# ucsdmanorlab/bootstrapper

Hardware: AMD Instinct MI355X
Metric: Mvoxels/s predict+segment, 1024^3 vol in 128^3 blocks (higher is better)
Workload: dtype bf16x3

## Files before the change

bootstrapper_amd/_lib.py:

```python
import ctypes as C
import os

import torch

_HERE = os.path.dirname(os.path.abspath(__file__))
LIB_PATH = os.environ.get("BSMI_LIB") or os.path.join(_HERE, "libbsmi.so")

MAX_LEVELS, MAX_CONVS, MAX_HEADS, NAME_LEN = 8, 4, 4, 32
PREC_F32, PREC_BF16, PREC_BF16X3 = 0, 1, 2
RAW_U8, RAW_F32, RAW_U8_UNIT = 0, 1, 2
ERR_INVALID, ERR_HIP, ERR_STATE, ERR_MISSING, ERR_OVERFLOW = -1, -2, -3, -4, -5


class UNetConfig(C.Structure):
    _fields_ = [
        ("in_channels", C.c_int32),
        ("num_fmaps", C.c_int32),
        ("fmap_inc_factor", C.c_int32),
        ("num_levels", C.c_int32),
        ("downsample_factors", (C.c_int32 * 3) * MAX_LEVELS),
        ("n_convs_down", C.c_int32 * MAX_LEVELS),
        ("kernel_size_down", ((C.c_int32 * 3) * MAX_CONVS) * MAX_LEVELS),
        ("n_convs_up", C.c_int32 * MAX_LEVELS),
        ("kernel_size_up", ((C.c_int32 * 3) * MAX_CONVS) * MAX_LEVELS),
        ("num_heads", C.c_int32),
        ("head_name", (C.c_char * NAME_LEN) * MAX_HEADS),
        ("head_dims", C.c_int32 * MAX_HEADS),
        ("num_fmaps_out", C.c_int32),
    ]


class StepInfo(C.Structure):
    _fields_ = [("type", C.c_int32), ("materialised", C.c_int32), ("shape", C.c_int32 * 4), ("conv_index", C.c_int32),
                ("form", C.c_int32), ("flags", C.c_int32), ("bn", C.c_int32), ("ksteps", C.c_int32), ("head", C.c_int32),
                ("factor", C.c_int32 * 3), ("offset", C.c_int32 * 3), ("prefix", C.c_char * 64)]


class TrainWgradInfo(C.Structure):
    _fields_ = [(n, C.c_int32) for n in ("family", "residual", "n", "c", "cbase", "kx", "tile_n", "tile_c", "ranges", "lines_per_range",
                                         "det_workspace")]


class TrainStepInfo(C.Structure):
    _fields_ = [("type", C.c_int32), ("n_wgrad", C.c_int32), ("wgrad", TrainWgradInfo * 4), ("dgrad", C.c_int32), ("dgrad_raw", C.c_int32),
                ("dgrad_converted", C.c_int32), ("dgrad_bn", C.c_int32), ("dgrad_ksteps", C.c_int32), ("dgrad_split_k", C.c_int32),
                ("dgrad_scatter", C.c_int32), ("dgrad_residual", C.c_int32), ("border", C.c_int32 * 3), ("has_split", C.c_int32),
                ("bias", C.c_int32), ("up", C.c_int32), ("fwd_split", C.c_int32), ("deterministic", C.c_int32)]


WGRAD_FAMILIES = ("none", "wave-f32", "tiled-f32", "split-bf16")
TRAIN_TENSORS = {"dout": 0, "gmask": 1, "gsplit": 2, "gsplit_hi": 3, "gsplit_lo": 4, "dcat": 5, "head_dp": 6, "pad_count": 7}
STEP_TYPES = ("input", "conv", "pool", "up", "head")
CONV_FORMS = ("gather", "raster-halo", "box-halo", "halo-resident", "first-pass", "winograd F(2x2)", "winograd F(4x4)")
STEP_FLAGS = {1: "fused-up", 2: "res-low", 4: "split-k"}
STEP_BELOW_UP = 8
STEP_WINO_Z = 16


class Codec(C.Structure):
    _fields_ = [("id", C.c_int32), ("level", C.c_int32), ("cname", C.c_int32), ("shuffle", C.c_int32),
                ("typesize", C.c_int32), ("blocksize", C.c_int32)]


class ChunkCopy(C.Structure):
    _fields_ = [("path", C.c_char_p), ("base", C.c_void_p), ("start", C.c_int64 * 4), ("extent", C.c_int64 * 4),
                ("stride", C.c_int64 * 4), ("read_modify_write", C.c_int32), ("reserved", C.c_int32)]


class BatchFragArgs(C.Structure):
    _fields_ = [("affs_dev", C.c_void_p), ("frags_dev", C.c_void_p), ("max_id_dev", C.c_void_p), ("labels_dev", C.c_void_p),
                ("num_labels_dev", C.c_void_p), ("id_offset", C.c_uint64), ("size_dev", C.c_void_p), ("sums_dev", C.c_void_p)]


class BatchGraphArgs(C.Structure):
    _fields_ = [("affs_dev", C.c_void_p), ("frags_dev", C.c_void_p), ("edges_dev", C.c_void_p), ("sums_dev", C.c_void_p),
                ("pair_counts_dev", C.c_void_p), ("counts_dev", C.c_void_p), ("edge_capacity", C.c_uint64)]


class Aug2dDraw(C.Structure):
    _fields_ = [("a", C.c_float * 4), ("src", C.c_float * 2), ("inv_spacing", C.c_float * 2), ("flags", C.c_int32), ("n", C.c_int32 * 2),
                ("lattice_offset", C.c_int32), ("crop", C.c_int32 * 2), ("crop_offset", C.c_int32), ("reserved", C.c_int32)]


class Aug2dIDraw(C.Structure):
    _fields_ = [("seed", C.c_uint64), ("impulse_threshold", C.c_uint64), ("noise_sigma", C.c_float), ("contrast_scale", C.c_float),
                ("nodes", C.c_int32), ("radius", C.c_int32), ("taps_offset", C.c_int32), ("reserved", C.c_int32 * 3)]


CODEC_RAW, CODEC_ZLIB, CODEC_GZIP, CODEC_ZSTD, CODEC_LZ4, CODEC_BLOSC = range(6)
BLOSC_LZ4, BLOSC_ZLIB, BLOSC_ZSTD = 1, 3, 4
CHUNK_MISSING = 1
MORPH_DILATE, MORPH_ERODE = 0, 1
RESCALE_DOWN, RESCALE_UP = 0, 1


class BsmiError(RuntimeError):
    def __init__(self, code, msg):
        super().__init__(f"libbsmi error {code}: {msg}")
        self.code = code
        self.msg = msg


def _load():
    if not os.path.exists(LIB_PATH):
        raise ImportError(
            f"{LIB_PATH} not found: build it with `python -c 'import __graft_entry__ as g; g.build()'` "
            "(or `make -C bootstrapper_amd/csrc`).  There is no CPU fallback.")
    lib = C.CDLL(LIB_PATH)
    p, i32, i64p, vp = C.c_void_p, C.c_int, C.POINTER(C.c_int64), C.c_void_p
# ... 184 lines not shown
```

bootstrapper_amd/csrc/conv_h16.h:

```cpp
#pragma once
#include "conv_igemm.h"

namespace bsmi {

struct H16Phase {
  int32_t tensor;
  int32_t delta;
  int32_t rows;
  int32_t nsteps;
};
static_assert(sizeof(H16Phase) == 16, "H16Phase layout");

struct H16Step {
  int32_t offa, offb, pad0, pad1;
};
static_assert(sizeof(H16Step) == 16, "H16Step layout");

struct H16Args {
  ConvSrc t[kMaxConvTensors];
  const H16Phase* phases;
  const H16Step* steps;
  int nphases, nsteps;
  const void* w;
  const void* w_lo;
  const float* bias;
  void* out;
  int Do, Ho, Wo, Co;
  int Hin, Win;
  int Q;
  int Npad;
  int relu;
  int ntiles, n_big, r_small;
};

constexpr int kH16TileRows = 512;
int h16_halo_rows(int Win, int ky, int kx, int npad, int* max_r);
void h16_tiling(int64_t Q, int npad, int halo_rows, int max_r, int n_cus, int* ntiles, int* n_big, int* r_small);
int launch_conv_h16(const H16Args& a, int halo_rows, hipStream_t stream);

}
```

bootstrapper_amd/csrc/conv_h16.hip:

```cpp
#include "conv_h16.h"

#include <algorithm>

#include "conv_dev.h"

namespace bsmi {

#ifdef BSMI_STAMP
__device__ unsigned long long g_h16_stamp[8];
extern "C" int bsmi_debug_stamps_h16(unsigned long long* out, int reset) {
  if (hipMemcpyFromSymbol(out, HIP_SYMBOL(g_h16_stamp), sizeof(unsigned long long) * 8) != hipSuccess) return -1;
  if (reset) {
    unsigned long long z[8] = {0, 0, 0, 0, 0, 0, 0, 0};
    if (hipMemcpyToSymbol(HIP_SYMBOL(g_h16_stamp), z, sizeof z) != hipSuccess) return -1;
  }
  return 0;
}
#define H16_STAMP(var_) const unsigned long long var_ = wall_clock64()
#else
#define H16_STAMP(var_)
#endif

namespace {

constexpr int kNW = 4;
constexpr int kR = 8;

template <int FNB, int HR>
__global__ __launch_bounds__(64 * kNW, 2) void conv_h16_kernel(const H16Args a) {
  using T = bf16f_elem;
  constexpr int BN = 16 * FNB, BM = kH16TileRows;
  static_assert(BM == kNW * kR * 16, "tile rows");
  constexpr int HALO = HR * 64;
  constexpr int OFF_B = HALO;
  constexpr int EB = BN * 64;
  constexpr int SLOT = 2 * EB;
  constexpr int JW = HR / 16 / kNW;
  static_assert(HR % (16 * kNW) == 0, "the waves share the halo rows evenly");
  constexpr int G = FNB >= 4 ? 1 : (FNB == 2 ? 2 : 8);
  extern __shared__ __attribute__((aligned(16))) char smem[];
  const int tid = threadIdx.x, lane = tid & 63;
  const int wave = __builtin_amdgcn_readfirstlane(tid >> 6);
  const int ntiles = a.ntiles;
  const int qn = ntiles >> 3, rn = ntiles & 7;
  const int xcd = blockIdx.x & 7, jn = blockIdx.x >> 3;
  const int tile = (xcd < rn ? xcd * (qn + 1) : rn * (qn + 1) + (xcd - rn) * qn) + jn;
  const int R = tile < a.n_big ? kR : a.r_small;
  const int q0 = tile < a.n_big ? tile * BM : a.n_big * BM + (tile - a.n_big) * a.r_small * (kNW * 16);
  const int cut = (kR - R) * (kNW * 16);
  H16_STAMP(st_begin);
#ifdef BSMI_STAMP
  unsigned long long acc_halo = 0, acc_k = 0, acc_w = 0;
#endif
  const cint_ptr_t phases = (cint_ptr_t)a.phases;
  const cint_ptr_t steps = (cint_ptr_t)a.steps;
  const int nsteps = a.nsteps, nphases = a.nphases;
// ... 84 lines not shown
      const uint32_t ar = arow0 + (uint32_t)(tap_b ? offb : offa);
      const char* ap = smem + ar * 64 + ((aslot ^ ((ar >> 2) & 1)) << 4);
      const char* apl = smem + ar * 64 + ((aslot ^ ((ar >> 2) & 1) ^ 1) << 4);
#pragma unroll
      for (int i0 = 0; i0 < kR; i0 += G) {
        if (i0 >= R) break;
        u32x4_t AH[G], AL[G];
#pragma unroll
        for (int g = 0; g < G; ++g) {
          AH[g] = *(const u32x4_t*)(ap + (i0 + g) * 1024);
          AL[g] = *(const u32x4_t*)(apl + (i0 + g) * 1024);
        }
#pragma unroll
        for (int g = 0; g < G; ++g)
#pragma unroll
          for (int j = 0; j < FNB; ++j)
            acc[i0 + g][j] = __builtin_amdgcn_mfma_f32_16x16x32_bf16(__builtin_bit_cast(bf16x8_t, AL[g]), __builtin_bit_cast(bf16x8_t, BH[j]), acc[i0 + g][j], 0, 0, 0);
#pragma unroll
        for (int g = 0; g < G; ++g)
#pragma unroll
          for (int j = 0; j < FNB; ++j)
            acc[i0 + g][j] = __builtin_amdgcn_mfma_f32_16x16x32_bf16(__builtin_bit_cast(bf16x8_t, AH[g]), __builtin_bit_cast(bf16x8_t, BH[j]), acc[i0 + g][j], 0, 0, 0);
#pragma unroll
        for (int g = 0; g < G; ++g)
#pragma unroll
          for (int j = 0; j < FNB; ++j)
            acc[i0 + g][j] = __builtin_amdgcn_mfma_f32_16x16x32_bf16(__builtin_bit_cast(bf16x8_t, AH[g]), __builtin_bit_cast(bf16x8_t, BL[j]), acc[i0 + g][j], 0, 0, 0);
      }
      H16_STAMP(st_k1);
      asm volatile("s_waitcnt vmcnt(0) lgkmcnt(0)" ::: "memory");
      __builtin_amdgcn_s_barrier();
#ifdef BSMI_STAMP
      {
        const unsigned long long st_k2 = wall_clock64();
        acc_k += st_k1 - st_k0;
        acc_w += st_k2 - st_k1;
      }
#endif
    }
  }
#undef H16_ISSUE_B
  H16_STAMP(st_epi);

  constexpr int PITCH = BN * 2 + 16;
  constexpr int CPR = BN * 2 / 16;
  constexpr int NCH = 16 * CPR;
  constexpr int LO_STRIPS = kNW * 16 * PITCH;
  static_assert(2 * LO_STRIPS <= HALO, "strips fit in the halo area");
  char* strip = smem + wave * (16 * PITCH);
  T* out = (T*)a.out;
  float bv[FNB];
#pragma unroll
  for (int j = 0; j < FNB; ++j) bv[j] = a.bias[j * 16 + lr];
#pragma unroll
  for (int i = 0; i < kR; ++i) {
    if (i >= R) break;
#pragma unroll
    for (int j = 0; j < FNB; ++j)
#pragma unroll
      for (int r = 0; r < 4; ++r) {
        float v = acc[i][j][r] + bv[j];
        if (a.relu) v = v > 0.f ? v : 0.f;
        Elem<T>::store((T*)(strip + (4 * lq + r) * PITCH) + j * 16 + lr, v);
        Elem<T>::store((T*)(strip + LO_STRIPS + (4 * lq + r) * PITCH) + j * 16 + lr, split_lo(v));
      }
    asm volatile("s_waitcnt lgkmcnt(0)" ::: "memory");
#pragma unroll
    for (int k = 0; k < (NCH + 63) / 64; ++k) {
      const int c = lane + 64 * k;
      if (c >= NCH) break;
      const int row = c / CPR, cc = c - row * CPR;
      const int q = q0 + wave * (R * 16) + i * 16 + row;
      const int n = cc * 8;
      if (q < a.Q && n < a.Co) {
        const int xx = q % a.Win;
        const int zy = q / a.Win;
        const int yy = zy % a.Hin, z = zy / a.Hin;
        if (xx < a.Wo && yy < a.Ho) {
          T* dst = out + act_index<T>(((size_t)(z * a.Ho + yy) * a.Wo + xx) * a.Co, n);
          store_stream16(dst, *(const u32x4_t*)(strip + row * PITCH + cc * 16));
          store_stream16(dst + kSplitLoElems, *(const u32x4_t*)(strip + LO_STRIPS + row * PITCH + cc * 16));
        }
      }
    }
    asm volatile("s_waitcnt lgkmcnt(0)" ::: "memory");
  }
#ifdef BSMI_STAMP
  if (tid == 0) {
    const unsigned long long st_end = wall_clock64();
    atomicAdd(&g_h16_stamp[0], acc_halo);
    atomicAdd(&g_h16_stamp[1], acc_k);
    atomicAdd(&g_h16_stamp[2], acc_w);
    atomicAdd(&g_h16_stamp[3], 1ull);
    atomicAdd(&g_h16_stamp[4], (unsigned long long)nphases);
    atomicAdd(&g_h16_stamp[5], (unsigned long long)nsteps);
    atomicAdd(&g_h16_stamp[6], st_loop - st_begin);
    atomicAdd(&g_h16_stamp[7], st_end - st_epi);
  }
#endif
}

template <int FNB, int HR>
int launch_t(const H16Args& a, hipStream_t stream) {
  constexpr int smem = HR * 64 + 4 * 16 * FNB * 64;
  static_assert(2 * smem <= 160 * 1024, "two workgroups per CU (three at 16 columns and 768 rows)");
  auto kern = conv_h16_kernel<FNB, HR>;
  static DeviceOnce once;
  const int rc_once = once.run([&]() -> int {
    BSMI_HIP(hipFuncSetAttribute((const void*)kern, hipFuncAttributeMaxDynamicSharedMemorySize, smem));
    hipFuncAttributes fa;
    BSMI_HIP(hipFuncGetAttributes(&fa, (const void*)kern));
    if (fa.localSizeBytes != 0) BSMI_FAIL(BSMI_ERR_STATE, "halo conv kernel (%d columns) was compiled with %zu bytes of scratch", 16 * FNB, (size_t)fa.localSizeBytes);
    return BSMI_OK;
  });
  if (rc_once) return rc_once;
  hipLaunchKernelGGL(kern, dim3(a.ntiles), dim3(64 * kNW), smem, stream, a);
  BSMI_HIP(hipGetLastError());
  return BSMI_OK;
}

}

int h16_halo_rows(int Win, int ky, int kx, int npad, int* max_r) {
  if (npad != 16 && npad != 64) return 0;
  const int reach = (ky - 1) * Win + (kx - 1);
  *max_r = kR;
  if (kH16TileRows + reach <= 768) return 768;
  if (npad == 16 && (kR - 1) * kNW * 16 + reach <= 768) {
    *max_r = kR - 1;
    return 768;
  }
  if (kH16TileRows + reach <= 1024 && npad == 16) return 1024;
  return 0;
}

void h16_tiling(int64_t Q, int npad, int halo_rows, int max_r, int n_cus, int* ntiles, int* n_big, int* r_small) {
  const int64_t big = kH16TileRows, unit = kNW * 16;
  if (max_r < kR) {
    *ntiles = (int)((Q + max_r * unit - 1) / (max_r * unit));
    *n_big = 0;
    *r_small = max_r;
    return;
  }
  const int64_t nt = (Q + big - 1) / big;
  *ntiles = (int)nt;
  *n_big = (int)nt;
  *r_small = kR;
  const int64_t lds = (int64_t)halo_rows * 64 + 4 * npad * 64;
  const int64_t per_cu = std::min<int64_t>(npad == 64 ? 2 : 3, (160 * 1024) / lds);
  const int64_t slots = per_cu * n_cus;
  if (slots <= 0 || nt % slots == 0) return;
  const int64_t rounds = (nt + slots - 1) / slots, total = rounds * slots;
  if (rounds > 4) return;
  const int64_t r = (Q + total * unit - 1) / (total * unit);
  if (r < 6 || r > kR) return;
  if (r < kR) {
    const int64_t rows = r * unit;
    *ntiles = (int)((Q + rows - 1) / rows);
    *n_big = 0;
    *r_small = (int)r;
    return;
  }
  const int64_t small = big - unit;
  int64_t nb = (Q - total * small + unit - 1) / unit;
  if (nb < 0) nb = 0;
  *ntiles = (int)total;
  *n_big = (int)nb;
  *r_small = kR - 1;
}

int launch_conv_h16(const H16Args& a, int halo_rows, hipStream_t stream) {
  if (a.Q <= 0 || a.nsteps <= 0 || a.nphases <= 0 || a.Hin <= 0 || a.Win <= 0 || a.Hin > 2047 || a.Win > 2047 || a.Do > 1023)
    BSMI_FAIL(BSMI_ERR_INVALID, "halo conv: bad geometry Q=%d steps=%d phases=%d raster %d x %d", a.Q, a.nsteps, a.nphases, a.Hin, a.Win);
// ... 12 lines not shown
```

bootstrapper_amd/csrc/unet_debug.hip:

```cpp
#include <cstring>

#include "unet_internal.h"

extern "C" {

int bsmi_debug_wino_pack_host(const float* w, int cout, int cin, int wz, uint16_t* out, uint64_t capacity, uint64_t* image_elems, uint64_t* batch_elems,
                              int* npad, int* ksteps) {
  if (!w || cout < 1 || cin < 1) BSMI_FAIL(BSMI_ERR_INVALID, "bad argument");
  std::vector<int> cin_of_v;
  for (int c = 0; c < round_up(cin, kChanPad); ++c) cin_of_v.push_back(c < cin ? c : -1);
  const int Npad = round_up(cout, tile_bn(choose_tile(cout)));
  std::vector<WinoUnit> units;
  wino_units((int)cin_of_v.size(), units, wz ? 1 : 3);
  if (image_elems || batch_elems || out) {
    std::vector<uint16_t> packed;
    size_t ie = 0, be = 0;
    wino_pack_weights(w, cout, cin, cin_of_v, Npad, units, packed, ie, be, 4, wz != 0);
    if (image_elems) *image_elems = ie;
    if (batch_elems) *batch_elems = be;
    if (out) {
      if (capacity < packed.size()) BSMI_FAIL(BSMI_ERR_INVALID, "buffer of %llu values too small", (unsigned long long)capacity);
      memcpy(out, packed.data(), packed.size() * sizeof(uint16_t));
    }
  }
  if (npad) *npad = Npad;
  if (ksteps) *ksteps = (int)(units.size() / kUnitsPerStep);
  return BSMI_OK;
}

int bsmi_unet_debug_activation(bsmi_unet* h, int step, int what, int64_t shape_out[4], float* host_out, uint64_t capacity) {
  if (!h || !shape_out) BSMI_FAIL(BSMI_ERR_INVALID, "null argument");
  Plan* plan = h->last_plan;
  if (!plan) BSMI_FAIL(BSMI_ERR_STATE, "no forward has run");
  if (step < 0 || step >= (int)plan->steps.size()) BSMI_FAIL(BSMI_ERR_INVALID, "step %d out of range (%zu steps)", step, plan->steps.size());
  const PlanStep& st = plan->steps[step];
  if (st.type == PlanStep::HEAD) BSMI_FAIL(BSMI_ERR_INVALID, "head steps write into the caller's buffers");
  if (plan->fused_first && step < 2)
    BSMI_FAIL(BSMI_ERR_STATE, "step %d is not materialised: the first ConvPass ran as one launch (first_pass), which writes step 2 only", step);
  if (st.type == PlanStep::UP && st.skip)
    BSMI_FAIL(BSMI_ERR_STATE, "step %d is not materialised: the upsampling is fused into the Winograd stages that read it", step);
  const TDesc& t = st.out;
  shape_out[0] = t.D; shape_out[1] = t.H; shape_out[2] = t.W; shape_out[3] = t.C;
  if (!host_out) return BSMI_OK;
  const size_t nvox = (size_t)t.D * t.H * t.W;
  if (capacity < nvox * t.C) BSMI_FAIL(BSMI_ERR_INVALID, "buffer of %llu floats too small", (unsigned long long)capacity);
  BSMI_HIP(hipSetDevice(h->device));
  BSMI_HIP(hipDeviceSynchronize());
  const int es = esize(plan->prec);
  const bool split = t.lo_off != 0;
  const size_t bytes = nvox * t.Cpad * es * (split ? 2 : 1);
  std::vector<uint8_t> raw(bytes);
  BSMI_HIP(hipMemcpy(raw.data(), t.ptr, raw.size(), hipMemcpyDeviceToHost));
  for (size_t v = 0; v < nvox; ++v)
    for (int c = 0; c < t.C; ++c) {
      float x;
      if (plan->prec == BSMI_PREC_F32) {
        x = ((const float*)raw.data())[v * t.Cpad + c];
      } else if (!split) {
        x = host_bf16_to_f32(((const uint16_t*)raw.data())[v * t.Cpad + c]);
      } else {
        const size_t i = 2 * v * t.Cpad + (size_t)((c >> 3) << 4) + (c & 7);
        const float hi = host_bf16_to_f32(((const uint16_t*)raw.data())[i]);
        const float lo = host_bf16_to_f32(((const uint16_t*)raw.data())[i + 8]);
        x = what == 1 ? hi : (what == 2 ? lo : hi + lo);
      }
      host_out[v * t.C + c] = x;
    }
  return BSMI_OK;
}

int bsmi_unet_debug_step_info(bsmi_unet* h, int step, bsmi_unet_step_info* info, int* n_steps) {
  if (!h) BSMI_FAIL(BSMI_ERR_INVALID, "null handle");
  Plan* plan = h->last_plan;
  if (!plan) BSMI_FAIL(BSMI_ERR_STATE, "no forward has run");
  if (n_steps) *n_steps = (int)plan->steps.size();
  if (!info) return BSMI_OK;
  if (step < 0 || step >= (int)plan->steps.size()) BSMI_FAIL(BSMI_ERR_INVALID, "step %d out of range (%zu steps)", step, plan->steps.size());
  const PlanStep& st = plan->steps[step];
  memset(info, 0, sizeof *info);
  info->type = (int32_t)st.type;
  const bool in_first = plan->fused_first && step < 3;
  info->materialised = !((plan->fused_first && step < 2) || (st.type == PlanStep::UP && st.skip));
  const TDesc& t = st.type == PlanStep::HEAD ? st.in : st.out;
  info->shape[0] = t.D; info->shape[1] = t.H; info->shape[2] = t.W;
  info->shape[3] = st.type == PlanStep::HEAD ? h->heads[st.head].cout : t.C;
  const std::string* prefix = nullptr;
  if (st.type == PlanStep::HEAD) {
    info->head = st.head;
    prefix = &h->heads[st.head].prefix;
  } else if (st.type == PlanStep::POOL || st.type == PlanStep::UP) {
    for (int d = 0; d < 3; ++d) { info->factor[d] = st.f[d]; info->offset[d] = st.type == PlanStep::UP ? st.o[d] : 0; }
  } else if (st.type == PlanStep::CONV) {
    prefix = &st.site->prefix;
    info->conv_index = st.ci;
    const int sk_grid = h->sk_grid > 0 ? h->sk_grid : 0;
    if (in_first) {
      info->form = BSMI_FORM_FIRST_PASS;
    } else if (st.use_wino) {
      info->form = st.wino_in.m == 4 ? BSMI_FORM_WINO4 : BSMI_FORM_WINO2;
      info->bn = tile_bn(st.tile);
      info->ksteps = st.wino_gemm.nsteps;
      bool up = false;
      for (int q = 0; q < st.wino_in.nsrc; ++q) up = up || st.wino_in.upf[q] > 0;
      if (up || st.wino_out.low || st.wino_has_below) info->flags |= BSMI_STEP_FUSED_UP;
      if (st.wino_has_below) info->flags |= BSMI_STEP_BELOW_UP;
      if (st.wino_has_res_low) info->flags |= BSMI_STEP_RES_LOW;
      if (st.wino_in.wz) info->flags |= BSMI_STEP_WINO_Z;
      if (conv_igemm_split_k(st.wino_gemm, plan->prec, st.tile, sk_grid) ||
          (st.wino_has_res && conv_igemm_split_k(st.wino_res, plan->prec, st.tile, sk_grid)) ||
          (st.wino_has_res_low && conv_igemm_split_k(st.wino_res_low, plan->prec, st.tile, sk_grid)) ||
          (st.wino_has_below && conv_igemm_split_k(st.wino_below, plan->prec, st.below_tile, sk_grid)))
        info->flags |= BSMI_STEP_SPLIT_K;
    } else if (st.use_h16) {
      info->form = BSMI_FORM_HALO_RESIDENT;
      info->bn = st.h16.Npad;
      info->ksteps = st.h16.nsteps;
    } else if (st.use_box) {
      info->form = BSMI_FORM_BOX_HALO;
    } else if (st.use_rh) {
      info->form = BSMI_FORM_RASTER_HALO;
      info->bn = tile_bn(st.tile);
      info->ksteps = st.rh.nsteps;
      if (conv_rh_split_k(st.rh, st.tile, sk_grid)) info->flags |= BSMI_STEP_SPLIT_K;
    } else {
      info->form = BSMI_FORM_GATHER;
      info->bn = tile_bn(st.tile);
      info->ksteps = st.conv.nsteps;
      if (conv_igemm_split_k(st.conv, plan->prec, st.tile, sk_grid)) info->flags |= BSMI_STEP_SPLIT_K;
    }
  }
  if (prefix) snprintf(info->prefix, sizeof info->prefix, "%s", prefix->c_str());
  return BSMI_OK;
}

}
```

bootstrapper_amd/csrc/unet_forward.hip:

```cpp
#include <algorithm>
#include <cstdlib>
#include <mutex>

#include "unet_internal.h"
#include "unet_ops.h"

#include "dev_guard.h"

namespace bsmi {

static int harvest(bsmi_unet* h, Plan* plan) {
  if (!plan || plan->inflight.empty()) return BSMI_OK;
  const size_t n = plan->steps.size();
  for (auto& set : plan->inflight) {
    plan->last_ms.assign(n, 0.f);
    BSMI_HIP(hipEventSynchronize(set[2 * n - 1]));
    for (size_t i = 0; i < n; ++i) {
      float t = 0.f;
      BSMI_HIP(hipEventElapsedTime(&t, set[2 * i], set[2 * i + 1]));
      plan->last_ms[i] = t;
      const int ty = (plan->fused_first && i < 2) ? (int)PlanStep::CONV : (int)plan->steps[i].type;
      h->prof_ms[ty] += t;
      h->prof_flops[ty] += plan->steps[i].flops;
      if (ty == 1) h->prof_exec += plan->steps[i].exec_flops > 0 ? plan->steps[i].exec_flops : plan->steps[i].flops * (plan->prec == BSMI_PREC_BF16X3 ? 3.0 : 1.0);
// ... 71 lines not shown
    } else {
      plan.events.assign(n_ev, nullptr);
      for (auto& e : plan.events) BSMI_HIP(hipEventCreate(&e));
    }
  }
  if (!h->sk_grid) {
    const char* e = getenv("BSMI_STREAMK");
    if ((e && e[0] == '0') || h->sk_request == 0) {
      h->sk_grid = -1;
    } else {
      hipDeviceProp_t prop;
      BSMI_HIP(hipGetDeviceProperties(&prop, h->device));
      h->sk_grid = h->sk_request >= 0 ? h->sk_request : prop.multiProcessorCount / 8 * 8;
      if (const char* g = getenv("BSMI_SK_GRID")) h->sk_grid = std::max(8, atoi(g) / 8 * 8);
      BSMI_HIP(hipMalloc((void**)&h->sk_ws, stream_k_ws_bytes(h->sk_grid)));
      BSMI_HIP(hipMemsetAsync((char*)h->sk_ws + stream_k_ws_bytes(h->sk_grid) - 64, 0, 64, s));
    }
  }
  if (h->train && precision == BSMI_PREC_F32 && !h->train_forward && (rc = train_refresh_f32_images(h, s))) return rc;
  size_t step_idx = 0;
  for (const PlanStep& st : plan.steps) {
    if (prof) BSMI_HIP(hipEventRecord(plan.events[2 * step_idx], s));
    if (plan.fused_first && step_idx < 3) {
      if (step_idx == 2) {
        FirstPassArgs fa;
        fa.raw = raw_dev; fa.raw_dtype = raw_dtype;
        fa.D = plan.steps[0].out.D; fa.H = plan.steps[0].out.H; fa.W = plan.steps[0].out.W;
        fa.out = (uint16_t*)st.out.ptr;
        const FirstPassWeights& fw = precision == BSMI_PREC_BF16X3 ? h->first_pass_x3 : h->first_pass;
        fa.w1a = fw.w1a; fa.w2a = fw.w2a; fa.vec = fw.vec;
        fa.split = fw.split;
        rc = launch_first_pass(fa, h->sk_grid > 0 ? h->sk_grid : 256, s);
        if (rc) return rc;
      }
      if (prof) BSMI_HIP(hipEventRecord(plan.events[2 * step_idx + 1], s));
      ++step_idx;
      continue;
    }
    switch (st.type) {
      case PlanStep::INPUT:
        rc = launch_input_prep(precision, raw_dev, raw_dtype, st.out.ptr, st.out.C, st.out.Cpad,
                               (size_t)st.out.D * st.out.H * st.out.W, s);
        break;
      case PlanStep::CONV:
        if (st.use_wino && !(st.tx3 && h->train_forward)) {
          if ((rc = launch_wino_in(st.wino_in, s))) break;
          if ((rc = launch_conv_igemm(st.wino_gemm, precision, st.tile, s, h->sk_ws, h->sk_grid))) break;
          if (st.wino_has_res && (rc = launch_conv_igemm(st.wino_res, precision, st.tile, s, h->sk_ws, h->sk_grid))) break;
          if (st.wino_has_res_low && (rc = launch_conv_igemm(st.wino_res_low, precision, st.tile, s, h->sk_ws, h->sk_grid))) break;
          if (st.wino_has_below && (rc = launch_conv_igemm(st.wino_below, precision, st.below_tile, s, h->sk_ws, h->sk_grid))) break;
          rc = launch_wino_out(st.wino_out, s);
          break;
        }
        rc = (st.tx3 && h->train_forward) ? train_forward_conv_x3(h, st, s)
             : st.use_h16 ? launch_conv_h16(st.h16, st.h16_rows, s)
             : st.use_box ? launch_conv_box(st.box, s)
             : st.use_rh ? launch_conv_rh(st.rh, precision, st.tile, s, h->sk_ws, h->sk_grid)
                         : launch_conv_igemm(st.conv, precision, st.tile, s, h->sk_ws, h->sk_grid);
        break;
      case PlanStep::POOL:
        if (st.pool_fused) break;
        rc = launch_maxpool(precision, st.in.ptr, st.out.ptr, st.in.D, st.in.H, st.in.W, st.in.Cpad,
                            st.f[0], st.f[1], st.f[2], s);
        break;
      case PlanStep::UP:
        if (st.skip) break;
        rc = launch_upsample_crop(precision, st.in.ptr, st.out.ptr, st.in.D, st.in.H, st.in.W, st.in.Cpad,
                                  st.out.D, st.out.H, st.out.W, st.f[0], st.f[1], st.f[2], st.o[0], st.o[1], st.o[2], s);
        break;
      case PlanStep::HEAD: {
        const HeadSite& hd = h->heads[st.head];
        float* of = out_f32_dev ? out_f32_dev[st.head] : nullptr;
        uint8_t* ou = out_u8_dev ? out_u8_dev[st.head] : nullptr;
        if (of || ou)
          rc = launch_head(precision, st.in.ptr, st.in.Cpad, hd.cin, hd.cout, hd.hw, hd.hb, of, ou,
                           (size_t)st.in.D * st.in.H * st.in.W, s);
        break;
      }
    }
    if (rc) return rc;
    if (prof) BSMI_HIP(hipEventRecord(plan.events[2 * step_idx + 1], s));
    ++step_idx;
  }
  if (prof) plan.inflight.push_back(std::move(plan.events));
  return forward_chain_leave(h->device, s);
}

int bsmi_unet_profile_enable(bsmi_unet* h, int on) {
  if (!h) BSMI_FAIL(BSMI_ERR_INVALID, "null handle");
  h->profile_period = on > 0 ? on : 0;
  h->profile_count = 0;
  return BSMI_OK;
}

int bsmi_unet_profile_read(bsmi_unet* h, int max_n, int* n, int32_t* types, double* ms, double* flops) {
  if (!h || !n) BSMI_FAIL(BSMI_ERR_INVALID, "null argument");
  Plan* plan = h->last_plan;
  if (!plan || !plan->profiled) BSMI_FAIL(BSMI_ERR_STATE, "no profiled forward to read");
  int rc = harvest(h, plan);
  if (rc) return rc;
  const int cnt = (int)plan->steps.size();
  *n = cnt;
  for (int i = 0; i < cnt && i < max_n; ++i) {
    if (types) types[i] = (int32_t)plan->steps[i].type;
    if (ms) ms[i] = plan->last_ms[i];
    if (flops) flops[i] = plan->steps[i].flops;
// ... 27 lines not shown
```

bootstrapper_amd/csrc/unet_internal.h:

```cpp
#pragma once
#include <cstring>
#include <map>
#include <memory>
#include <string>
#include <vector>

#include "conv_igemm.h"
#include "conv_rh.h"
#include "conv_h16.h"
#include "conv_box.h"
#include "first_pass.h"
#include "wino.h"

namespace bsmi {

struct HostWeight {
  std::vector<int64_t> shape;
  std::vector<float> data;
  bool loaded = false;
};

struct PackEntry {
  int slot;
  int dz, dy, dx;
  int c0;
  int wsrc;
  int tap;
  int cin_base;
  int creal;
  bool dummy;
  int phase;
};

struct PackPhase {
  int slot, c0, kind, first_unit, nunits;
};

struct PackedConv {
  bool ready = false;
  std::vector<PackEntry> entries;
  std::vector<PackPhase> phases;
  void* w = nullptr;
  int ks = 1;
  size_t lo_image_bytes = 0;
  float* bias = nullptr;
  int Npad = 0;
  TileCfg tile = TILE_256x32;
};

struct PackedWino {
  bool ready = false;
  int m = 2;
  bool fused_only = false;
  bool wz = false;
  std::vector<WinoUnit> units;
  std::vector<int> cin_of_v;
  int Cv = 0;
  void* w = nullptr;
  size_t lo_image_bytes = 0, batch_bytes = 0;
  int Npad = 0;
  TileCfg tile = TILE_256x32;
  std::vector<PackEntry> res_entries;
  void* res_w = nullptr;
  size_t res_lo_image_bytes = 0;
  std::vector<PackEntry> res_part[2];
  void* res_part_w[2] = {nullptr, nullptr};
  size_t res_part_lo[2] = {0, 0};
  bool below_ready = false;
  std::vector<WinoUnit> skip_units, below_units;
  std::vector<int> skip_cin_of_v;
  int skip_Cv = 0;
  void* skip_w = nullptr;
  size_t skip_lo_image_bytes = 0, skip_batch_bytes = 0;
  void* below_w = nullptr;
  size_t below_lo_image_bytes = 0, below_batch_bytes = 0;
  int below_Npad = 0;
  bool below_dense = false;
  TileCfg below_tile = TILE_256x320;
};

struct H16PhaseHost {
  int slot, c0, dz, kind;
  int first_step, nsteps;
};
struct PackedH16 {
  bool ready = false;
  std::vector<PackEntry> entries;
  std::vector<H16PhaseHost> phases;
  void* w = nullptr;
  size_t lo_image_bytes = 0;
  int Npad = 0;
};

struct PassSite {
  std::string prefix;
  int nslots = 1;
  int cin[2] = {0, 0};
  int cout = 0;
  int nconv = 0;
  int k[BSMI_MAX_CONVS][3];
  PackedConv packed[BSMI_NUM_PREC][BSMI_MAX_CONVS];
  PackedWino wino[BSMI_MAX_CONVS];
  PackedH16 h16[BSMI_MAX_CONVS];
};

struct HeadSite {
  std::string prefix;
  int cin = 0, cout = 0;
  float* hw = nullptr;
  float* hb = nullptr;
};

struct TDesc {
  void* ptr = nullptr;
  int C = 0, Cpad = 0, D = 0, H = 0, W = 0;
  size_t lo_off = 0;
};

struct PlanStep {
  enum Type { INPUT, CONV, POOL, UP, HEAD } type;
  ConvArgs conv;
  RhArgs rh;
  bool use_rh = false;
  H16Args h16;
  bool use_h16 = false;
  int h16_rows = 0;
  BoxArgs box;
  bool use_box = false;
  bool use_wino = false;
  WinoInArgs wino_in;
  ConvArgs wino_gemm, wino_res, wino_res_low;
  bool wino_has_res = false, wino_has_res_low = false;
  ConvArgs wino_below;
  bool wino_has_below = false;
  TileCfg below_tile = TILE_256x320;
  WinoOutArgs wino_out;
  TileCfg tile;
  TDesc in, out;
  int f[3], o[3];
  bool skip = false;
  bool pool_fused = false;
  int head = 0;
  double flops = 0;
  double exec_flops = 0;
  struct PassSite* site = nullptr;
  int ci = 0;
  TDesc slots[kMaxConvTensors];
  int so[kMaxConvTensors][3] = {{0, 0, 0}, {0, 0, 0}, {0, 0, 0}};
  int nsl = 0;
  struct TrainFwdX3* tx3 = nullptr;
};

struct Plan {
  std::vector<float> last_ms;
  bool pending = false;
  std::vector<void*> allocs;
  std::vector<PlanStep> steps;
  int64_t out_shape[3] = {0, 0, 0};
  double flops = 0;
  size_t bytes = 0;
  std::vector<hipEvent_t> events;
  std::vector<std::vector<hipEvent_t>> inflight, spare;
  bool profiled = false;
  bool fused_first = false;
  int prec = 0;
};

struct TrainState;

static inline uint16_t host_f32_to_bf16(float f) {
  uint32_t u;
  memcpy(&u, &f, 4);
  if ((u & 0x7fffffffu) > 0x7f800000u) return (uint16_t)((u >> 16) | 0x40);
  u += 0x7fffu + ((u >> 16) & 1u);
  return (uint16_t)(u >> 16);
}
static inline float host_bf16_to_f32(uint16_t b) {
  const uint32_t u = (uint32_t)b << 16;
  float f;
// ... 4 lines not shown
int esize(int prec);
int ksplit(int prec);
int bke(int prec);
int sube(int prec);
void build_entries(const PassSite& p, int ci, int prec, std::vector<PackEntry>& out, std::vector<PackPhase>* phases_out = nullptr);

}

using namespace bsmi;

struct bsmi_unet {
  bsmi_unet_config cfg;
  int device = 0;
  int nl = 0;
  std::vector<PassSite> l_conv, r_conv;
  std::vector<HeadSite> heads;
  int crop_factor[BSMI_MAX_LEVELS][3];
  std::map<std::string, HostWeight> weights;
  bool finalized[BSMI_NUM_PREC] = {false, false, false};
  int profile_period = 0;
  uint64_t profile_count = 0;
  Plan* last_plan = nullptr;
  double prof_ms[5] = {0, 0, 0, 0, 0}, prof_flops[5] = {0, 0, 0, 0, 0};
  double prof_exec = 0;
  int64_t prof_launches[5] = {0, 0, 0, 0, 0};
  std::map<std::vector<int64_t>, std::unique_ptr<Plan>> plans;
  float* sk_ws = nullptr;
  int sk_grid = 0;
  int sk_request = -1;
  bsmi::TrainState* train = nullptr;
  bool train_forward = false;
  int train_split = 1;
  int train_det = 0;
  bsmi::FirstPassWeights first_pass;
  bsmi::FirstPassWeights first_pass_x3;
};

namespace bsmi {
int pack_conv(bsmi_unet* h, PassSite& p, int ci, int prec);
int pack_wino(bsmi_unet* h, PassSite& p, int ci);
int pack_h16(bsmi_unet* h, PassSite& p, int ci);
void release(PackedConv& pc);
void release(PackedWino& pw);
void release(PackedH16& ph);

bool x3_fused_for(TileCfg tile);
bool wino_eligible(const PassSite& p, int ci);
int wino_tile_edge();
bool wino_narrow_last(const bsmi_unet* h, const PassSite& p, int ci);
bool below_up_site(const bsmi_unet* h, const PassSite& p, int ci);
bool wino_z_site(const bsmi_unet* h, const PassSite& p, int ci);
bool fuse_up_enabled();
bool pool_fuse_enabled();
int h16_mode();
int h16_only_npad();
bool h16_balanced();
bool rh_enabled(int prec, TileCfg tile, size_t nsteps);
bool box_enabled();
bool first_pass_eligible(const bsmi_unet* h);

int check_shape_arg(const int64_t s[3]);
int get_plan(bsmi_unet* h, int precision, const int64_t in_shape[3], Plan** out);
int dry_plan(bsmi_unet* h, const int64_t in_shape[3], Plan& plan);
void free_plan(Plan* p);
void free_train_state(bsmi_unet* h);
int train_forward_conv_x3(bsmi_unet* h, const PlanStep& st, hipStream_t s);
int train_refresh_f32_images(bsmi_unet* h, hipStream_t s);
}
```

bootstrapper_amd/csrc/unet_pack.hip:

```cpp
#include <cstdlib>
#include <cstring>

#include "unet_internal.h"

#include "dev_guard.h"

namespace bsmi {

int esize(int prec) { return prec == BSMI_PREC_F32 ? 4 : 2; }
int ksplit(int prec) { return prec == BSMI_PREC_BF16X3 ? 3 : 1; }
int bke(int prec) { return kStepRowBytes / esize(prec); }
int sube(int prec) { return 32 / esize(prec); }

static inline void split_bf16(float v, uint16_t& hi, uint16_t& lo) {
  hi = host_f32_to_bf16(v);
  lo = host_f32_to_bf16(v - host_bf16_to_f32(hi));
}

template <class T>
static void release_image(T*& w) {
  if (w) (void)hipFree(w);
  w = nullptr;
}
void release(PackedConv& pc) {
  release_image(pc.w);
  release_image(pc.bias);
  pc.ready = false;
}
void release(PackedWino& pw) {
  release_image(pw.w);
  release_image(pw.res_w);
  for (int part = 0; part < 2; ++part) release_image(pw.res_part_w[part]);
  release_image(pw.skip_w);
  release_image(pw.below_w);
  pw.below_ready = false;
  pw.ready = false;
}
void release(PackedH16& ph) {
  release_image(ph.w);
  ph.ready = false;
}

void build_entries(const PassSite& p, int ci, int prec, std::vector<PackEntry>& out, std::vector<PackPhase>* phases_out) {
  const int SUB = sube(prec);
  const bool last = ci == p.nconv - 1;
  std::vector<PackPhase> phases;
  auto close_phase = [&](PackPhase ph) {
    while ((out.size() - ph.first_unit) % kUnitsPerStep) out.push_back(PackEntry{ph.slot, 0, 0, 0, 0, 0, 0, 0, 0, true, (int)phases.size()});
    ph.nunits = (int)out.size() - ph.first_unit;
    phases.push_back(ph);
  };
  auto add_taps = [&](int slot, const int* k, int cin_base, int creal) {
    const int cpad = round_up(creal, kChanPad);
    if (cpad == SUB) {
      PackPhase ph{slot, 0, 0, (int)out.size(), 0};
      for (int z = 0; z < k[0]; ++z)
        for (int y = 0; y < k[1]; ++y)
          for (int x = 0; x < k[2]; x += kUnitsPerStep)
            for (int j = 0; j < kUnitsPerStep; ++j) {
              if (x + j < k[2])
                out.push_back(PackEntry{slot, z, y, x + j, 0, 0, (z * k[1] + y) * k[2] + x + j, cin_base, creal, false, (int)phases.size()});
              else
                out.push_back(PackEntry{slot, 0, 0, 0, 0, 0, 0, 0, 0, true, (int)phases.size()});
            }
      close_phase(ph);
      return;
    }
    for (int c32 = 0; c32 < cpad; c32 += kUnitsPerStep * SUB) {
      PackPhase ph{slot, c32, 0, (int)out.size(), 0};
      for (int z = 0; z < k[0]; ++z)
        for (int y = 0; y < k[1]; ++y)
          for (int x = 0; x < k[2]; ++x) {
            for (int c0 = c32; c0 < std::min(cpad, c32 + kUnitsPerStep * SUB); c0 += SUB)
              out.push_back(PackEntry{slot, z, y, x, c0, 0, (z * k[1] + y) * k[2] + x, cin_base, creal, false, (int)phases.size()});
            while ((out.size() - ph.first_unit) % kUnitsPerStep)
              out.push_back(PackEntry{slot, 0, 0, 0, 0, 0, 0, 0, 0, true, (int)phases.size()});
          }
      close_phase(ph);
    }
  };
  auto add_residual = [&](int slot, const int* crop, int cin_base, int creal) {
    const int cpad = round_up(creal, kChanPad);
    for (int c32 = 0; c32 < cpad; c32 += kUnitsPerStep * SUB) {
      PackPhase ph{slot, c32, 1, (int)out.size(), 0};
      for (int c0 = c32; c0 < std::min(cpad, c32 + kUnitsPerStep * SUB); c0 += SUB)
        out.push_back(PackEntry{slot, crop[0] / 2, crop[1] / 2, crop[2] / 2, c0, 1, 0, cin_base, creal, false, (int)phases.size()});
      close_phase(ph);
    }
  };
  const int* k = p.k[ci];
  if (ci == 0) {
    int base = 0;
// ... 37 lines not shown
  const int64_t cin_r = wr.shape[1];
  const int SUB = sube(prec);
  const bool fused = prec == BSMI_PREC_BF16X3 && x3_fused_for(pc.tile);
  const int KS = pc.ks = fused ? 1 : ksplit(prec);
  const size_t nsteps = pc.entries.size() / kUnitsPerStep * KS;
  const size_t nelem = (nsteps * (size_t)pc.Npad + kWeightRowSlack) * BKE;
  std::vector<float> bias(pc.Npad, 0.f);
  for (int n = 0; n < p.cout; ++n) bias[n] = bm.data[n] + (last ? br.data[n] : 0.f);

  pc.lo_image_bytes = fused ? nelem * esize(prec) : 0;
  std::vector<uint8_t> packed(nelem * esize(prec) * (fused ? 2 : 1), 0);
  host_parallel_for((size_t)p.cout, [&](size_t n_) {
    const int n = (int)n_;
    for (size_t u = 0; u < pc.entries.size(); ++u) {
      const PackEntry& e = pc.entries[u];
      if (e.dummy) continue;
      const size_t s = u / kUnitsPerStep, j = u % kUnitsPerStep;
      for (int kk = 0; kk < SUB; ++kk) {
        const int c = e.c0 + kk;
        if (c >= e.creal) break;
        float v;
        if (e.wsrc == 0) v = wm.data[((size_t)n * cin_m + (e.cin_base + c)) * ntap_m + e.tap];
        else v = wr.data[(size_t)n * cin_r + (e.cin_base + c)];
        const size_t idx = (s * KS * pc.Npad + n) * BKE + j * SUB + kk;
        if (prec == BSMI_PREC_F32) {
          ((float*)packed.data())[idx] = v;
        } else if (prec == BSMI_PREC_BF16) {
          ((uint16_t*)packed.data())[idx] = host_f32_to_bf16(v);
        } else {
          uint16_t hi, lo;
          split_bf16(v, hi, lo);
          uint16_t* w16 = (uint16_t*)packed.data();
          if (fused) {
            w16[idx] = hi;
            w16[idx + nelem] = lo;
          } else {
            const size_t blk = (size_t)pc.Npad * BKE;
            w16[idx] = hi;
            w16[idx + blk] = hi;
            w16[idx + 2 * blk] = lo;
          }
        }
      }
    }
  });
  BSMI_HIP(hipMalloc(&pc.w, packed.size()));
  BSMI_HIP(hipMemcpy(pc.w, packed.data(), packed.size(), hipMemcpyHostToDevice));
  BSMI_HIP(hipMalloc((void**)&pc.bias, bias.size() * sizeof(float)));
  BSMI_HIP(hipMemcpy(pc.bias, bias.data(), bias.size() * sizeof(float), hipMemcpyHostToDevice));
  pc.ready = true;
  return BSMI_OK;
}

int pack_wino(bsmi_unet* h, PassSite& p, int ci) {
  PackedWino& pw = p.wino[ci];
  release(pw);
  pw.fused_only = wino_narrow_last(h, p, ci);
  if (!wino_eligible(p, ci) && !pw.fused_only) return BSMI_OK;
  const HostWeight& wm = h->weights[p.prefix + ".conv_pass." + std::to_string(2 * ci) + ".weight"];
  const HostWeight& wr = h->weights[p.prefix + ".residual.0.weight"];
  const int cin_m = (int)wm.shape[1];
  pw.cin_of_v.clear();
  if (ci == 0) {
    int base = 0;
    for (int s = 0; s < p.nslots; ++s) {
      for (int c = 0; c < round_up(p.cin[s], kChanPad); ++c) pw.cin_of_v.push_back(c < p.cin[s] ? base + c : -1);
      base += p.cin[s];
    }
  } else {
    for (int c = 0; c < round_up(p.cout, kChanPad); ++c) pw.cin_of_v.push_back(c < p.cout ? c : -1);
  }
  pw.Cv = (int)pw.cin_of_v.size();
  pw.m = wino_tile_edge();
  pw.tile = choose_tile(p.cout);
  pw.Npad = round_up(p.cout, tile_bn(pw.tile));
  pw.wz = !pw.fused_only && pw.m == 4 && wino_z_site(h, p, ci);
  wino_units(pw.Cv, pw.units, pw.wz ? 1 : 3);
  {
    size_t image_elems = 0, batch_elems = 0;
    static const bool on_host = [] { const char* e = getenv("BSMI_WINO_PACK_HOST"); return e && e[0] == '1'; }();
    if (on_host) {
      std::vector<uint16_t> packed;
      wino_pack_weights(wm.data.data(), p.cout, cin_m, pw.cin_of_v, pw.Npad, pw.units, packed, image_elems, batch_elems, pw.m, pw.wz);
      BSMI_HIP(hipMalloc(&pw.w, packed.size() * 2));
      BSMI_HIP(hipMemcpy(pw.w, packed.data(), packed.size() * 2, hipMemcpyHostToDevice));
    } else {
      const int rc = wino_pack_weights_dev(wm.data.data(), p.cout, cin_m, pw.cin_of_v, pw.Npad, pw.units, pw.m, &pw.w, image_elems, batch_elems, pw.wz);
      if (rc) return rc;
    }
    pw.lo_image_bytes = image_elems * 2;
    pw.batch_bytes = batch_elems * 2;
  }
  pw.res_entries.clear();
  if (ci == p.nconv - 1) {
    std::vector<PackEntry> all;
    build_entries(p, ci, BSMI_PREC_BF16X3, all);
    for (size_t u = 0; u + 1 < all.size(); u += kUnitsPerStep) {
      bool res = false;
      for (int j = 0; j < kUnitsPerStep; ++j) res |= !all[u + j].dummy && all[u + j].wsrc == 1;
      if (res)
        for (int j = 0; j < kUnitsPerStep; ++j) pw.res_entries.push_back(all[u + j]);
    }
    if ((pw.res_entries.size() / kUnitsPerStep) % 2)
      for (int j = 0; j < kUnitsPerStep; ++j) pw.res_entries.push_back(PackEntry{0, 0, 0, 0, 0, 0, 0, 0, 0, true, 0});
    const int64_t cin_r = wr.shape[1];
    auto pack_res = [&](const std::vector<PackEntry>& ents, void** w_out, size_t* lo_out) -> int {
      const size_t nsteps = ents.size() / kUnitsPerStep;
      const size_t nelem = (nsteps * (size_t)pw.Npad + kWeightRowSlack) * 32;
      std::vector<uint16_t> packed(2 * nelem, 0);
      for (size_t u = 0; u < ents.size(); ++u) {
        const PackEntry& e = ents[u];
        if (e.dummy) continue;
        const size_t s = u / kUnitsPerStep, j = u % kUnitsPerStep;
        for (int n = 0; n < p.cout; ++n)
          for (int kk = 0; kk < 16; ++kk) {
            const int c = e.c0 + kk;
            if (c >= e.creal) break;
            const float v = wr.data[(size_t)n * cin_r + (e.cin_base + c)];
            const size_t idx = (s * pw.Npad + n) * 32 + j * 16 + kk;
            split_bf16(v, packed[idx], packed[nelem + idx]);
          }
      }
      *lo_out = nelem * 2;
      BSMI_HIP(hipMalloc(w_out, packed.size() * 2));
      BSMI_HIP(hipMemcpy(*w_out, packed.data(), packed.size() * 2, hipMemcpyHostToDevice));
      return BSMI_OK;
    };
    int rc = pack_res(pw.res_entries, &pw.res_w, &pw.res_lo_image_bytes);
    if (rc) return rc;
    for (int part = 0; part < 2; ++part) pw.res_part[part].clear();
    if (p.nslots == 2) {
      const int up_slot = (ci == 0 ? 0 : 1) + 1;
      for (size_t u = 0; u + 1 < pw.res_entries.size(); u += kUnitsPerStep) {
        int slot = -1;
        for (int j = 0; j < kUnitsPerStep; ++j)
          if (!pw.res_entries[u + j].dummy) slot = pw.res_entries[u + j].slot;
        if (slot < 0) continue;
        for (int j = 0; j < kUnitsPerStep; ++j) pw.res_part[slot == up_slot ? 1 : 0].push_back(pw.res_entries[u + j]);
      }
      for (int part = 0; part < 2; ++part) {
        if ((pw.res_part[part].size() / kUnitsPerStep) % 2)
          for (int j = 0; j < kUnitsPerStep; ++j) pw.res_part[part].push_back(PackEntry{0, 0, 0, 0, 0, 0, 0, 0, 0, true, 0});
        if ((rc = pack_res(pw.res_part[part], &pw.res_part_w[part], &pw.res_part_lo[part]))) return rc;
      }
    }
  }
  if (below_up_site(h, p, ci) && pw.m == 4) {
    pw.skip_cin_of_v.assign(pw.cin_of_v.begin(), pw.cin_of_v.begin() + round_up(p.cin[0], kChanPad));
    pw.skip_Cv = (int)pw.skip_cin_of_v.size();
    wino_units(pw.skip_Cv, pw.skip_units);
    size_t image_elems = 0, batch_elems = 0;
    int rc = wino_pack_weights_dev(wm.data.data(), p.cout, cin_m, pw.skip_cin_of_v, pw.Npad, pw.skip_units, pw.m, &pw.skip_w, image_elems, batch_elems);
    if (rc) return rc;
    pw.skip_lo_image_bytes = image_elems * 2;
    pw.skip_batch_bytes = batch_elems * 2;
    const int cpad_low = round_up(p.cin[1], kChanPad), cpad_out = round_up(p.cout, kChanPad);
    wino_units(cpad_low, pw.below_units);
    pw.below_dense = p.cout <= 64;
    pw.below_tile = pw.below_dense ? TILE_256x320 : pw.tile;
    pw.below_Npad = pw.below_dense ? round_up(9 * cpad_out, tile_bn(pw.below_tile)) : pw.Npad;
    const size_t nsteps = pw.below_units.size() / kUnitsPerStep;
    const size_t tap_elems = nsteps * (size_t)pw.below_Npad * 32;
    const size_t nelem = (pw.below_dense ? 1 : 9) * tap_elems + (size_t)kWeightRowSlack * 32;
    std::vector<uint16_t> packed(2 * nelem, 0);
    const bool dense = pw.below_dense;
    const int cin1 = p.cin[1], cbase = p.cin[0];
    host_parallel_for((size_t)p.cout, [&](size_t n_) {
      const int n = (int)n_;
      for (size_t u = 0; u < pw.below_units.size(); ++u) {
        const WinoUnit& un = pw.below_units[u];
        if (un.dummy) continue;
        const size_t s = u / kUnitsPerStep, j = u % kUnitsPerStep;
        for (int kk = 0; kk < 16; ++kk) {
          const int c = un.vc0 + kk;
          if (c >= cin1) break;
          const float* g = wm.data.data() + (((size_t)n * cin_m + (cbase + c)) * 3 + un.kz) * 9;
          for (int tap = 0; tap < 9; ++tap) {
            const size_t idx = dense ? (s * pw.below_Npad + (size_t)tap * cpad_out + n) * 32 + j * 16 + kk
                                     : (size_t)tap * tap_elems + (s * pw.below_Npad + n) * 32 + j * 16 + kk;
            split_bf16(g[tap], packed[idx], packed[nelem + idx]);
          }
        }
      }
    });
    pw.below_lo_image_bytes = nelem * 2;
    pw.below_batch_bytes = dense ? 0 : tap_elems * 2;
    BSMI_HIP(hipMalloc(&pw.below_w, packed.size() * 2));
    BSMI_HIP(hipMemcpy(pw.below_w, packed.data(), packed.size() * 2, hipMemcpyHostToDevice));
    pw.below_ready = true;
  }
  pw.ready = true;
  return BSMI_OK;
}

static void build_entries_h16(const PassSite& p, int ci, std::vector<PackEntry>& out, std::vector<H16PhaseHost>& phases) {
  const bool last = ci == p.nconv - 1;
  const int* k = p.k[ci];
  const PackEntry dummy{0, 0, 0, 0, 0, 0, 0, 0, 0, true, 0};
  auto add_taps = [&](int slot, int cin_base, int creal) {
    const int cpad = round_up(creal, kChanPad);
    for (int z = 0; z < k[0]; ++z)
      for (int c0 = 0; c0 < cpad; c0 += 16) {
        H16PhaseHost ph{slot, c0, z, 0, (int)(out.size() / kUnitsPerStep), 0};
        const int ntap = k[1] * k[2];
        for (int i = 0; i < ntap; i += 2) {
          for (int j = 0; j < 2; ++j) {
            if (i + j < ntap) {
              const int y = (i + j) / k[2], x = (i + j) % k[2];
              out.push_back(PackEntry{slot, z, y, x, c0, 0, (z * k[1] + y) * k[2] + x, cin_base, creal, false, (int)phases.size()});
            } else {
              out.push_back(dummy);
            }
          }
          ++ph.nsteps;
        }
        phases.push_back(ph);
      }
  };
  if (ci == 0) {
    int base = 0;
    for (int s = 0; s < p.nslots; ++s) {
      add_taps(s, base, p.cin[s]);
      base += p.cin[s];
    }
  } else {
    add_taps(0, 0, p.cout);
  }
  if (last) {
    int crop[3] = {0, 0, 0};
    for (int i = 0; i < p.nconv; ++i)
      for (int d = 0; d < 3; ++d) crop[d] += p.k[i][d] - 1;
    const int first_slot = ci == 0 ? 0 : 1;
    int base = 0;
    for (int s = 0; s < p.nslots; ++s) {
      const int cpad = round_up(p.cin[s], kChanPad);
      for (int c0 = 0; c0 < cpad; c0 += 16) {
        phases.push_back(H16PhaseHost{first_slot + s, c0, crop[0] / 2, 1, (int)(out.size() / kUnitsPerStep), 1});
        out.push_back(PackEntry{first_slot + s, crop[0] / 2, crop[1] / 2, crop[2] / 2, c0, 1, 0, base, p.cin[s], false, (int)phases.size() - 1});
        out.push_back(dummy);
      }
      base += p.cin[s];
    }
  }
}

int pack_h16(bsmi_unet* h, PassSite& p, int ci) {
  PackedH16& ph = p.h16[ci];
  release(ph);
  if (h16_mode() == 0 || p.cout > 64) return BSMI_OK;
  ph.entries.clear();
  ph.phases.clear();
  build_entries_h16(p, ci, ph.entries, ph.phases);
  ph.Npad = p.cout <= 16 ? 16 : 64;
  const HostWeight& wm = h->weights[p.prefix + ".conv_pass." + std::to_string(2 * ci) + ".weight"];
  const HostWeight& wr = h->weights[p.prefix + ".residual.0.weight"];
  const int64_t cin_m = wm.shape[1], ntap_m = wm.shape[2] * wm.shape[3] * wm.shape[4], cin_r = wr.shape[1];
  const size_t nsteps = ph.entries.size() / kUnitsPerStep;
  const size_t nelem = (nsteps * (size_t)ph.Npad + kWeightRowSlack) * 32;
  std::vector<uint16_t> packed(2 * nelem, 0);
  host_parallel_for((size_t)p.cout, [&](size_t n_) {
    const int n = (int)n_;
    for (size_t u = 0; u < ph.entries.size(); ++u) {
      const PackEntry& e = ph.entries[u];
      if (e.dummy) continue;
      const size_t s = u / kUnitsPerStep, j = u % kUnitsPerStep;
      for (int kk = 0; kk < 16; ++kk) {
        const int c = e.c0 + kk;
        if (c >= e.creal) break;
        const float v = e.wsrc == 0 ? wm.data[((size_t)n * cin_m + (e.cin_base + c)) * ntap_m + e.tap] : wr.data[(size_t)n * cin_r + (e.cin_base + c)];
        const size_t idx = (s * ph.Npad + n) * 32 + j * 16 + kk;
        split_bf16(v, packed[idx], packed[nelem + idx]);
      }
    }
  });
  ph.lo_image_bytes = nelem * 2;
  BSMI_HIP(hipMalloc(&ph.w, packed.size() * 2));
  BSMI_HIP(hipMemcpy(ph.w, packed.data(), packed.size() * 2, hipMemcpyHostToDevice));
  ph.ready = true;
  return BSMI_OK;
}

}
```

bootstrapper_amd/csrc/unet_plan.h:

```cpp
#pragma once
#include "unet_internal.h"

namespace bsmi {

struct UpFuse {
  TDesc low;
  int f[3];
  int o[3];
};

struct Planner {
  bsmi_unet* h;
  int prec;
  Plan* plan;
  bool dry;
  const UpFuse* fuse_up = nullptr;

  int alloc(TDesc& t);
  int plan_rh(const PassSite& p, int ci, const PackedConv& pc, const TDesc* slots, const int (*so)[3], const TDesc& o, PlanStep& st);
  int plan_h16(PassSite& p, int ci, const PackedConv& pc, const TDesc* slots, const int (*so)[3], const TDesc& o, PlanStep& st);
  int plan_box(const PassSite& p, int ci, const TDesc* slots, const int (*so)[3], const TDesc& o, PlanStep& st);
  int plan_wino(PassSite& p, int ci, const PackedConv& pc, const TDesc* slots, const int (*so)[3], int nsl, const TDesc& o, PlanStep& st);
  int pass(PassSite& p, const TDesc* in, const int (*org)[3], const int sp_in[3], TDesc& out);
  int rec(int level, const TDesc& f_in, TDesc& f_out);
  int run(const int64_t in_shape[3]);
};

int upload_ksteps(Plan* plan, const std::vector<KStep>& ks, ConvArgs& a);
void set_strides(ConvArgs& a, const void* base, int H, int W, int C, int bytes_per_channel);

}
```

bootstrapper_amd/csrc/unet_plan.hip:

```cpp
#include <algorithm>
#include <cmath>
#include <cstdlib>
#include <cstring>
#include <memory>

#include "unet_plan.h"

#include "dev_guard.h"

namespace bsmi {

int upload_ksteps(Plan* plan, const std::vector<KStep>& ks, ConvArgs& a) {
  KStep* dks = nullptr;
  BSMI_HIP(hipMalloc((void**)&dks, ks.size() * sizeof(KStep)));
  plan->allocs.push_back(dks);
  BSMI_HIP(hipMemcpy(dks, ks.data(), ks.size() * sizeof(KStep), hipMemcpyHostToDevice));
  a.steps = dks;
  a.nsteps = (int)ks.size();
  return BSMI_OK;
}

void set_strides(ConvArgs& a, const void* base, int H, int W, int C, int bytes_per_channel) {
  for (int sl = 0; sl < kMaxConvTensors; ++sl) {
    a.t[sl].base = (uint64_t)(uintptr_t)base;
// ... 74 lines not shown
  for (int q = 2; q < np; ++q) {
    const int is = first_step[q - 1] - 1;
    phases[q].issue_step = is;
    if (steps[is].issue >= 0) BSMI_FAIL(BSMI_ERR_STATE, "raster-halo plan: two halos on one staging slot");
    steps[is].issue = q;
  }
  std::vector<int> posW(nlisted + 8, 0), posH(np, 0);
  std::vector<char> isH;
  auto push = [&](bool halo) { isH.push_back(halo ? 1 : 0); return (int)isH.size() - 1; };
  posH[0] = push(true);
  if (np > 1) posH[1] = push(true);
  for (int w = 0; w < 4; ++w) posW[w] = push(false);
  for (size_t hh = 0; hh < nlisted; ++hh) {
    if (steps[hh].issue >= 0) posH[steps[hh].issue] = push(true);
    posW[hh + 4] = push(false);
  }
  for (size_t hh = 0; hh < nlisted; ++hh) {
    const int upto = posW[hh + 3];
    int need = posW[hh + 1];
    if (hh + 1 < nlisted) need = std::max(need, posH[steps[hh + 1].buf_phase >> 8]);
    if (need > upto) BSMI_FAIL(BSMI_ERR_STATE, "raster-halo plan: halo of K-step %zu staged too late", hh + 1);
    int aw = 0, bh = 0;
    for (int q = need + 1; q <= upto; ++q) (isH[q] ? bh : aw)++;
    if (aw > 2 || bh > 2) BSMI_FAIL(BSMI_ERR_STATE, "raster-halo plan: wait code out of range");
    steps[hh].wait = aw * 3 + bh;
  }
  RhArgs& a = st.rh;
  memset(&a, 0, sizeof a);
  for (int sl = 0; sl < kMaxConvTensors; ++sl) a.t[sl] = st.conv.t[sl];
  RhStep* dsteps = nullptr;
  RhPhase* dphases = nullptr;
  BSMI_HIP(hipMalloc((void**)&dsteps, steps.size() * sizeof(RhStep)));
  plan->allocs.push_back(dsteps);
  BSMI_HIP(hipMalloc((void**)&dphases, phases.size() * sizeof(RhPhase)));
  plan->allocs.push_back(dphases);
  BSMI_HIP(hipMemcpy(dsteps, steps.data(), steps.size() * sizeof(RhStep), hipMemcpyHostToDevice));
  BSMI_HIP(hipMemcpy(dphases, phases.data(), phases.size() * sizeof(RhPhase), hipMemcpyHostToDevice));
  a.steps = dsteps;
  a.phases = dphases;
  a.nsteps = (int)nlisted;
  a.nphases = np;
  a.w = pc.w;
  a.bias = pc.bias;
  a.out = o.ptr;
  a.Do = o.D; a.Ho = o.H; a.Wo = o.W; a.Co = o.Cpad;
  a.Hin = Hin; a.Win = Win;
  a.Q = o.D * Hin * Win;
  a.Npad = pc.Npad;
  a.relu = 1;
  st.use_rh = true;
  return BSMI_OK;
}

int Planner::plan_h16(PassSite& p, int ci, const PackedConv& pc, const TDesc* slots, const int (*so)[3], const TDesc& o, PlanStep& st) {
  st.use_h16 = false;
  const PackedH16& ph = p.h16[ci];
  const int* k = p.k[ci];
  const int Hin = o.H + k[1] - 1, Win = o.W + k[2] - 1;
  if (prec != BSMI_PREC_BF16X3 || !ph.ready || h16_mode() == 0 || pc.bias == nullptr) return BSMI_OK;
  if (h16_only_npad() && h16_only_npad() != ph.Npad) return BSMI_OK;
  int max_r = 0;
  const int rows = h16_halo_rows(Win, k[1], k[2], ph.Npad, &max_r);
  if (!rows || Hin > 2047 || Win > 2047 || o.D > 1023) return BSMI_OK;
  const int64_t Q = (int64_t)o.D * Hin * Win;
  if (Q >= ((int64_t)1 << 31)) return BSMI_OK;
  if (h16_mode() == 1 && Q < (int64_t)2 * 256 * kH16TileRows) return BSMI_OK;
  if (h16_mode() == 1 && ph.Npad == 64) {
    int main_steps = 0, res_steps = 0;
    for (const H16PhaseHost& hp : ph.phases) (hp.kind ? res_steps : main_steps) += hp.nsteps;
    if (3 * res_steps > main_steps) return BSMI_OK;
  }
  const int64_t es = 4;
  std::vector<H16Phase> phases(ph.phases.size());
  std::vector<H16Step> steps(ph.entries.size() / kUnitsPerStep);
  for (size_t q = 0; q < ph.phases.size(); ++q) {
    const H16PhaseHost& hp = ph.phases[q];
    const TDesc& t = slots[hp.slot];
    const PackEntry& e0 = ph.entries[(size_t)kUnitsPerStep * hp.first_step];
    const int oz = so[hp.slot][0] + hp.dz;
    const int oy = so[hp.slot][1] + (hp.kind ? e0.dy : 0);
    const int ox = so[hp.slot][2] + (hp.kind ? e0.dx : 0);
    const int64_t delta = ((((int64_t)oz * t.H + oy) * t.W + ox) * t.Cpad + hp.c0) * es;
    if (delta >= ((int64_t)1 << 31)) return BSMI_OK;
    phases[q] = H16Phase{hp.slot, (int32_t)delta, hp.kind ? kH16TileRows : kH16TileRows + (k[1] - 1) * Win + (k[2] - 1), hp.nsteps};
    for (int s = hp.first_step; s < hp.first_step + hp.nsteps; ++s) {
      const PackEntry& ea = ph.entries[(size_t)kUnitsPerStep * s];
      const PackEntry& eb = ph.entries[(size_t)kUnitsPerStep * s + 1];
      const int offa = hp.kind ? 0 : ea.dy * Win + ea.dx;
      const int offb = (hp.kind || eb.dummy) ? offa : eb.dy * Win + eb.dx;
      steps[s] = H16Step{offa, offb, 0, 0};
    }
  }
  H16Args& a = st.h16;
  memset(&a, 0, sizeof a);
  for (int sl = 0; sl < kMaxConvTensors; ++sl) a.t[sl] = st.conv.t[sl];
  H16Phase* dphases = nullptr;
  H16Step* dsteps = nullptr;
  BSMI_HIP(hipMalloc((void**)&dphases, phases.size() * sizeof(H16Phase)));
  plan->allocs.push_back(dphases);
  BSMI_HIP(hipMalloc((void**)&dsteps, steps.size() * sizeof(H16Step)));
  plan->allocs.push_back(dsteps);
  BSMI_HIP(hipMemcpy(dphases, phases.data(), phases.size() * sizeof(H16Phase), hipMemcpyHostToDevice));
  BSMI_HIP(hipMemcpy(dsteps, steps.data(), steps.size() * sizeof(H16Step), hipMemcpyHostToDevice));
  a.phases = dphases;
  a.steps = dsteps;
  a.nphases = (int)phases.size();
  a.nsteps = (int)steps.size();
  a.w = ph.w;
  a.w_lo = (const char*)ph.w + ph.lo_image_bytes;
  a.bias = pc.bias;
  a.out = o.ptr;
  a.Do = o.D; a.Ho = o.H; a.Wo = o.W; a.Co = o.Cpad;
  a.Hin = Hin; a.Win = Win;
  a.Q = (int)Q;
  a.Npad = ph.Npad;
  a.relu = 1;
  {
    int n_cus = 256;
    hipDeviceProp_t prop;
    if (hipGetDeviceProperties(&prop, h->device) == hipSuccess && prop.multiProcessorCount > 0) n_cus = prop.multiProcessorCount;
    h16_tiling(Q, ph.Npad, rows, max_r, h16_balanced() ? n_cus : 0, &a.ntiles, &a.n_big, &a.r_small);
  }
  st.h16_rows = rows;
  st.use_h16 = true;
  return BSMI_OK;
}

int Planner::plan_box(const PassSite& p, int ci, const TDesc* slots, const int (*so)[3], const TDesc& o, PlanStep& st) {
  st.use_box = false;
  const int* k = p.k[ci];
  if (!box_enabled() || prec != BSMI_PREC_BF16 || k[0] != 3 || k[1] != 3 || k[2] != 3 || !box_supported(p.cout)) return BSMI_OK;
  const bool last = ci == p.nconv - 1;
  const int NB = 1;
  const HostWeight& wm = h->weights[p.prefix + ".conv_pass." + std::to_string(2 * ci) + ".weight"];
  const HostWeight& bm = h->weights[p.prefix + ".conv_pass." + std::to_string(2 * ci) + ".bias"];
  const HostWeight& wr = h->weights[p.prefix + ".residual.0.weight"];
  const HostWeight& br = h->weights[p.prefix + ".residual.0.bias"];
  const int64_t cin_m = wm.shape[1], cin_r = wr.shape[1];
  int crop[3] = {0, 0, 0};
  for (int i = 0; i < p.nconv; ++i)
    for (int d = 0; d < 3; ++d) crop[d] += p.k[i][d] - 1;

  struct Src { int slot, cin_base, creal; };
  std::vector<Src> full, center;
  if (ci == 0) {
    int base = 0;
    for (int s = 0; s < p.nslots; ++s) { full.push_back({s, base, p.cin[s]}); base += p.cin[s]; }
  } else {
    full.push_back({0, 0, p.cout});
  }
  if (last) {
    const int first_slot = ci == 0 ? 0 : 1;
    int base = 0;
    for (int s = 0; s < p.nslots; ++s) { center.push_back({first_slot + s, base, p.cin[s]}); base += p.cin[s]; }
  }
  std::vector<BoxChunk> chunks;
  std::vector<uint32_t> wimg;
  auto chunk_of = [&](const TDesc& t, const int* org, int c0) {
    BoxChunk ck;
    ck.sx = t.Cpad * 2; ck.sy = t.W * ck.sx; ck.sz = t.H * ck.sy;
    ck.base = (uint64_t)(uintptr_t)t.ptr + (uint64_t)org[0] * ck.sz + (uint64_t)org[1] * ck.sy + (uint64_t)org[2] * ck.sx + (uint64_t)c0 * 2;
    ck.D = t.D - org[0]; ck.H = t.H - org[1]; ck.W = t.W - org[2];
    return ck;
  };
  auto put = [&](size_t lane_base, int j, float v) { wimg[lane_base + j / 2] |= (uint32_t)host_f32_to_bf16(v) << (16 * (j & 1)); };
  for (const Src& sr : full) {
    const TDesc& t = slots[sr.slot];
    for (int c0 = 0; c0 < t.Cpad; c0 += 16) {
      chunks.push_back(chunk_of(t, so[sr.slot], c0));
      const size_t w0 = wimg.size();
      wimg.resize(w0 + (size_t)14 * NB * 64 * 4, 0u);
      for (int s = 0; s < 14; ++s)
        for (int b = 0; b < NB; ++b)
          for (int l = 0; l < 64; ++l) {
// ... 210 lines not shown
    for (int d = 0; d < 3; ++d) st.f[d] = f[d];
    PlanStep& prod = plan->steps.back();
    if (pool_fuse_enabled() && prec == BSMI_PREC_BF16X3 && f[0] == 1 && f[1] == 2 && f[2] == 2 && prod.type == PlanStep::CONV && prod.use_wino &&
        prod.wino_out.m == 4 && !prod.wino_out.low && !prod.wino_out.wz && prod.wino_out.out == f_left.ptr && !(f_left.H & 1) && !(f_left.W & 1)) {
      prod.wino_out.pool = g_in.ptr;
      st.pool_fused = true;
    }
    plan->steps.push_back(st);
  }
  TDesc g_out;
  rc = rec(level - 1, g_in, g_out);
  if (rc) return rc;

  PassSite& rp = h->r_conv[i];
  const int up[3] = {g_out.D * f[0], g_out.H * f[1], g_out.W * f[2]};
  int conv_crop[3] = {0, 0, 0};
  for (int c = 0; c < rp.nconv; ++c)
    for (int d = 0; d < 3; ++d) conv_crop[d] += rp.k[c][d] - 1;
  int target[3];
  for (int d = 0; d < 3; ++d) {
    const int cf = h->crop_factor[i][d];
    const int n = (int)std::floor((double)(up[d] - conv_crop[d]) / cf);
    target[d] = n * cf + conv_crop[d];
    if (target[d] != up[d] && target[d] <= conv_crop[d])
      BSMI_FAIL(BSMI_ERR_INVALID,
                "Feature map with shape (%d, %d, %d) is too small to ensure translation equivariance",
                up[0], up[1], up[2]);
  }
  TDesc g_c;
  g_c.C = g_out.C; g_c.D = target[0]; g_c.H = target[1]; g_c.W = target[2];
  rc = alloc(g_c);
  if (rc) return rc;
  int so[2][3];
  for (int d = 0; d < 3; ++d) {
    so[0][d] = (dims[d] - target[d]) / 2;
    so[1][d] = 0;
    if (dims[d] < target[d])
      BSMI_FAIL(BSMI_ERR_INVALID, "skip connection (%d,%d,%d) smaller than upsampled map (%d,%d,%d)",
                dims[0], dims[1], dims[2], target[0], target[1], target[2]);
  }
  UpFuse uf;
  bool fuse = false;
  if (!dry && prec == BSMI_PREC_BF16X3 && f[0] == 1 && f[1] == 2 && f[2] == 2 && rp.nslots == 2 && rp.wino[0].ready &&
      rp.wino[rp.nconv - 1].ready && !rp.wino[rp.nconv - 1].res_part[1].empty() && g_out.ptr) {
    fuse = fuse_up_enabled();
    int sp[3] = {target[0], target[1], target[2]};
    for (int c = 0; c < rp.nconv && fuse; ++c) {
      for (int d = 0; d < 3; ++d) sp[d] -= rp.k[c][d] - 1;
      const int wm = rp.wino[c].m;
      if ((c == 0 || c == rp.nconv - 1) && ((wm == 2 && ((sp[1] & 1) || (sp[2] & 1))) || sp[0] <= 0 || sp[1] <= 0 || sp[2] <= 0)) fuse = false;
      if ((c == 0 || c == rp.nconv - 1) && (size_t)(sp[0] + 2) * ((sp[1] + wm - 1) / wm) * ((sp[2] + wm - 1) / wm) * rp.wino[c].Cv * 4 >= ((size_t)1 << 31)) fuse = false;
    }
  }
  if (!dry) {
    PlanStep st;
    st.type = PlanStep::UP;
    st.in = g_out; st.out = g_c;
    for (int d = 0; d < 3; ++d) { st.f[d] = f[d]; st.o[d] = (up[d] - target[d]) / 2; }
    st.skip = fuse;
    plan->steps.push_back(st);
  }
  if (fuse) {
    uf.low = g_out;
    for (int d = 0; d < 3; ++d) { uf.f[d] = f[d]; uf.o[d] = (up[d] - target[d]) / 2; }
    fuse_up = &uf;
    if (getenv("BSMI_PLAN_DEBUG")) fprintf(stderr, "[bsmi plan] %s: upsampling fused into the Winograd stages\n", rp.prefix.c_str());
  }
  const TDesc ins[2] = {f_left, g_c};
  rc = pass(rp, ins, so, target, f_out);
  fuse_up = nullptr;
  return rc;
}

int Planner::run(const int64_t in_shape[3]) {
  TDesc x;
  x.C = h->cfg.in_channels; x.D = (int)in_shape[0]; x.H = (int)in_shape[1]; x.W = (int)in_shape[2];
  int rc = alloc(x);
  if (rc) return rc;
  if (!dry) {
    PlanStep st;
    st.type = PlanStep::INPUT;
    st.out = x;
    plan->steps.push_back(st);
  }
  TDesc z;
  rc = rec(h->nl - 1, x, z);
  if (rc) return rc;
  plan->out_shape[0] = z.D; plan->out_shape[1] = z.H; plan->out_shape[2] = z.W;
  for (size_t hd = 0; hd < h->heads.size(); ++hd) {
    plan->flops += 2.0 * 2.0 * (double)z.D * z.H * z.W * h->heads[hd].cin * h->heads[hd].cout;
    if (!dry) {
      PlanStep st;
      st.type = PlanStep::HEAD;
      st.in = z;
      st.head = (int)hd;
      st.flops = 2.0 * 2.0 * (double)z.D * z.H * z.W * h->heads[hd].cin * h->heads[hd].cout;
      plan->steps.push_back(st);
    }
  }
  return BSMI_OK;
}

void free_plan(Plan* p) {
for (void* a : p->allocs) (void)hipFree(a);
p->allocs.clear();
for (auto* sets : {&p->inflight, &p->spare})
  for (auto& set : *sets)
    for (hipEvent_t e : set) (void)hipEventDestroy(e);
p->inflight.clear();
p->spare.clear();
p->events.clear();
}

int get_plan(bsmi_unet* h, int precision, const int64_t in_shape[3], Plan** out) {
  const std::vector<int64_t> key = {precision, in_shape[0], in_shape[1], in_shape[2]};
  auto it = h->plans.find(key);
  if (it == h->plans.end()) {
    std::unique_ptr<Plan> plan(new Plan);
    plan->prec = precision;
// ... 37 lines not shown
```

bootstrapper_amd/csrc/unet_plan_wino.hip:

```cpp
#include <cstring>

#include "unet_plan.h"

#include "dev_guard.h"

namespace bsmi {

namespace {

void raw_gemm(ConvArgs& a, const void* w, size_t lo_image_bytes, int Npad) {
  a.w = w;
  a.w_lo = (const char*)w + lo_image_bytes;
  a.Npad = Npad;
  a.relu = 0;
  a.raw = 1;
  a.nbatch = 0;
  a.a_batch = a.w_batch = 0;
}

struct WinoStage {
  Plan* plan;
  const UpFuse* fuse_up;
  const PassSite& p;
  int ci;
  const PackedConv& pc;
  const PackedWino& pw;
  const TDesc* slots;
  const int (*so)[3];
  const TDesc& o;
  PlanStep& st;
  bool below;
  bool cut;
  bool wz;
  int wm, nbatch, Dv, Ty, Tx, Cv;
  size_t vbatch, Mrows;
  void *V = nullptr, *Mbuf = nullptr, *addend = nullptr, *low = nullptr, *Ybuf = nullptr;
  size_t Mbelow = 0;
  int low_off[3] = {0, 0, 0}, below_off[3] = {0, 0, 0};

  int input_transform() {
    WinoInArgs& wi = st.wino_in;
    memset(&wi, 0, sizeof wi);
    const int nsrc = below ? 1 : ci == 0 ? p.nslots : 1;
    int cv0 = 0;
    for (int q = 0; q < nsrc; ++q) {
      const TDesc& t = slots[q];
      wi.src[q] = t.ptr;
      wi.H[q] = t.H; wi.W[q] = t.W; wi.Cpad[q] = t.Cpad;
      wi.oz[q] = so[q][0]; wi.oy[q] = so[q][1]; wi.ox[q] = so[q][2];
      wi.cv0[q] = cv0;
      cv0 += t.Cpad;
      if (fuse_up && ci == 0 && q == 1) {
        if (fuse_up->low.Cpad != t.Cpad) BSMI_FAIL(BSMI_ERR_STATE, "%s: fused upsampling with a different channel padding", p.prefix.c_str());
        wi.src[q] = fuse_up->low.ptr;
        wi.H[q] = fuse_up->low.H; wi.W[q] = fuse_up->low.W;
        wi.oz[q] += fuse_up->o[0]; wi.oy[q] += fuse_up->o[1]; wi.ox[q] += fuse_up->o[2];
        wi.upf[q] = fuse_up->f[1];
      }
    }
    if (cv0 != Cv) BSMI_FAIL(BSMI_ERR_STATE, "%s conv %d: winograd channel layout %d != %d", p.prefix.c_str(), ci, cv0, Cv);
    wi.nsrc = nsrc;
    wi.V = V;
    wi.Dv = Dv; wi.Ty = Ty; wi.Tx = Tx; wi.Cv = Cv;
    wi.m = wm;
    wi.wz = wz ? 1 : 0;
    wi.Dz = o.D + 2;
    return BSMI_OK;
  }

  int batched_gemm() {
    const std::vector<WinoUnit>& units = below ? pw.skip_units : pw.units;
    ConvArgs& g = st.wino_gemm;
    memset(&g, 0, sizeof g);
    set_strides(g, V, Ty, Tx, Cv, 4);
    std::vector<KStep> ks(units.size() / kUnitsPerStep);
    for (size_t s = 0; s < ks.size(); ++s) {
      KStep k;
      memset(&k, 0, sizeof k);
      for (int j = 0; j < kUnitsPerStep; ++j) {
        const WinoUnit& u = units[kUnitsPerStep * s + j];
        if (!u.dummy) k.delta[j] = (int32_t)(((int64_t)u.kz * Ty * Tx * Cv + u.vc0) * 4);
      }
      ks[s] = k;
    }
    const int rc = upload_ksteps(plan, ks, g);
    if (rc) return rc;
    raw_gemm(g, below ? pw.skip_w : pw.w, below ? pw.skip_lo_image_bytes : pw.lo_image_bytes, pw.Npad);
    g.bias = pc.bias;
    g.out = Mbuf;
    g.Do = wz ? Dv : o.D; g.Ho = Ty; g.Wo = Tx; g.Co = o.Cpad;
    g.M = (int)Mrows;
    g.nbatch = nbatch;
    g.a_batch = (int64_t)vbatch;
    g.w_batch = (int64_t)(below ? pw.skip_batch_bytes : pw.batch_bytes);
    return BSMI_OK;
  }

  int below_up() {
    const TDesc& lt = fuse_up->low;
    for (int d = 0; d < 3; ++d) below_off[d] = so[1][d] + fuse_up->o[d];
    if (fuse_up->f[1] != 2 || fuse_up->f[2] != 2 || lt.Cpad != slots[1].Cpad || below_off[0] < 0 || below_off[0] + o.D + 2 > lt.D || below_off[1] < 0 ||
        below_off[2] < 0 || below_off[1] + o.H + 2 > 2 * lt.H || below_off[2] + o.W + 2 > 2 * lt.W)
      BSMI_FAIL(BSMI_ERR_STATE, "%s: the low-resolution tensor does not cover the stage's input", p.prefix.c_str());
    Mbelow = (size_t)o.D * lt.H * lt.W;
    const size_t ybytes = 9 * Mbelow * o.Cpad * sizeof(float);
    if (Mbelow * 9 >= ((size_t)1 << 31)) BSMI_FAIL(BSMI_ERR_STATE, "%s: too many rows of sums below the upsampling", p.prefix.c_str());
    BSMI_HIP(hipMalloc(&Ybuf, ybytes));
    plan->allocs.push_back(Ybuf);
    plan->bytes += ybytes;
    ConvArgs& r = st.wino_below;
    memset(&r, 0, sizeof r);
    set_strides(r, lt.ptr, lt.H, lt.W, lt.Cpad, 4);
    std::vector<KStep> ks(pw.below_units.size() / kUnitsPerStep);
    for (size_t s = 0; s < ks.size(); ++s) {
      KStep k;
      memset(&k, 0, sizeof k);
      for (int j = 0; j < kUnitsPerStep; ++j) {
        const WinoUnit& u = pw.below_units[kUnitsPerStep * s + j];
        if (!u.dummy) k.delta[j] = (int32_t)(((int64_t)(u.kz + below_off[0]) * lt.H * lt.W * lt.Cpad + u.vc0) * 4);
      }
      ks[s] = k;
    }
    const int rc = upload_ksteps(plan, ks, r);
    if (rc) return rc;
    raw_gemm(r, pw.below_w, pw.below_lo_image_bytes, pw.below_Npad);
    r.bias = pc.bias;
    r.out = Ybuf;
    r.Do = o.D; r.Ho = lt.H; r.Wo = lt.W;
    r.Co = pw.below_dense ? 9 * o.Cpad : o.Cpad;
    r.M = (int)Mbelow;
    r.nbatch = pw.below_dense ? 0 : 9;
    r.w_batch = (int64_t)pw.below_batch_bytes;
    st.below_tile = pw.below_tile;
    st.wino_has_below = true;
    return BSMI_OK;
  }

  int residual_low() {
    const TDesc& g = fuse_up->low;
    const size_t Mlow = (size_t)g.D * g.H * g.W;
    BSMI_HIP(hipMalloc(&low, Mlow * o.Cpad * sizeof(float)));
    plan->allocs.push_back(low);
    plan->bytes += Mlow * o.Cpad * sizeof(float);
    ConvArgs& r = st.wino_res_low;
    memset(&r, 0, sizeof r);
    set_strides(r, g.ptr, g.H, g.W, g.Cpad, 4);
    const std::vector<PackEntry>& ents = pw.res_part[1];
    std::vector<KStep> ks(ents.size() / kUnitsPerStep);
    int up_slot = -1;
    for (size_t s = 0; s < ks.size(); ++s) {
      KStep k;
      memset(&k, 0, sizeof k);
      for (int j = 0; j < kUnitsPerStep; ++j) {
        const PackEntry& e = ents[kUnitsPerStep * s + j];
        if (e.dummy) continue;
        k.delta[j] = (int32_t)((int64_t)e.c0 * 4);
        up_slot = e.slot;
        low_off[0] = e.dz; low_off[1] = e.dy; low_off[2] = e.dx;
      }
      ks[s] = k;
    }
    if (up_slot < 0) BSMI_FAIL(BSMI_ERR_STATE, "%s: empty low-resolution residual", p.prefix.c_str());
    for (int d = 0; d < 3; ++d) low_off[d] += so[up_slot][d] + fuse_up->o[d];
    const int rc = upload_ksteps(plan, ks, r);
    if (rc) return rc;
    raw_gemm(r, pw.res_part_w[1], pw.res_part_lo[1], pw.Npad);
    r.bias = pc.bias;
    r.out = low;
    r.Do = g.D; r.Ho = g.H; r.Wo = g.W; r.Co = o.Cpad;
    r.M = (int)Mlow;
    st.wino_has_res_low = true;
    return BSMI_OK;
  }

  int residual() {
    const std::vector<PackEntry>& res_entries = cut ? pw.res_part[0] : pw.res_entries;
    BSMI_HIP(hipMalloc(&addend, (size_t)o.D * o.H * o.W * o.Cpad * sizeof(float)));
    plan->allocs.push_back(addend);
    plan->bytes += (size_t)o.D * o.H * o.W * o.Cpad * sizeof(float);
    ConvArgs& r = st.wino_res;
    r = st.conv;
    std::vector<KStep> ks(res_entries.size() / kUnitsPerStep);
    for (size_t s = 0; s < ks.size(); ++s) {
      KStep k;
      memset(&k, 0, sizeof k);
      const PackEntry& e0 = res_entries[kUnitsPerStep * s];
      k.tensor = e0.dummy ? 0 : e0.slot;
      for (int j = 0; j < kUnitsPerStep; ++j) {
        const PackEntry& e = res_entries[kUnitsPerStep * s + j];
        if (e.dummy) continue;
        const TDesc& t = slots[e.slot];
        const int64_t off = ((((int64_t)(e.dz + so[e.slot][0]) * t.H) + (e.dy + so[e.slot][1])) * t.W + (e.dx + so[e.slot][2])) * t.Cpad + e.c0;
        k.delta[j] = (int32_t)(off * 4);
      }
      ks[s] = k;
    }
    const int rc = upload_ksteps(plan, ks, r);
    if (rc) return rc;
    raw_gemm(r, cut ? pw.res_part_w[0] : pw.res_w, cut ? pw.res_part_lo[0] : pw.res_lo_image_bytes, pw.Npad);
    r.out = addend;
    return BSMI_OK;
  }

  void output_transform(int prec) {
    WinoOutArgs& wo = st.wino_out;
    memset(&wo, 0, sizeof wo);
    wo.M = (const float*)Mbuf;
    wo.addend = (const float*)addend;
    if (cut) {
      wo.low = (const float*)low;
      wo.lD = fuse_up->low.D; wo.lH = fuse_up->low.H; wo.lW = fuse_up->low.W;
      wo.lf = fuse_up->f[1];
      wo.loz = low_off[0]; wo.loy = low_off[1]; wo.lox = low_off[2];
    }
    if (below) {
      wo.below = (const float*)Ybuf;
      wo.btap = pw.below_dense ? (int64_t)o.Cpad : (int64_t)Mbelow * o.Cpad;
      wo.brow = pw.below_dense ? 9 * o.Cpad : o.Cpad;
      wo.boy = below_off[1]; wo.box = below_off[2];
      wo.lD = fuse_up->low.D; wo.lH = fuse_up->low.H; wo.lW = fuse_up->low.W;
      wo.lf = fuse_up->f[1];
    }
    wo.bias = pc.bias;
    wo.out = o.ptr;
    wo.Do = o.D; wo.Ty = Ty; wo.Tx = Tx; wo.Co = o.Cpad;
    wo.m = wm; wo.Ho = o.H; wo.Wo = o.W;
    wo.relu = 1;
    wo.wz = wz ? 1 : 0;
    const double kstep = (double)kUnitsPerStep * sube(prec);
    st.exec_flops = 2.0 * (double)round_up((int)Mrows, 256) * pw.Npad * ((double)st.wino_gemm.nsteps * kstep) * nbatch * 3.0;
    if (st.wino_has_res) st.exec_flops += 2.0 * (double)round_up(st.wino_res.M, 256) * pw.Npad * ((double)st.wino_res.nsteps * kstep) * 3.0;
    if (st.wino_has_res_low) st.exec_flops += 2.0 * (double)round_up(st.wino_res_low.M, 256) * pw.Npad * ((double)st.wino_res_low.nsteps * kstep) * 3.0;
    if (st.wino_has_below)
      st.exec_flops += 2.0 * (double)round_up(st.wino_below.M, 256) * pw.below_Npad * (pw.below_dense ? 1 : 9) * ((double)st.wino_below.nsteps * kstep) * 3.0;
  }
};

}

int Planner::plan_wino(PassSite& p, int ci, const PackedConv& pc, const TDesc* slots, const int (*so)[3], int nsl, const TDesc& o, PlanStep& st) {
  st.use_wino = false;
  const PackedWino& pw = p.wino[ci];
  const bool wants_fused = fuse_up && (ci == 0 || ci == p.nconv - 1);
  if (pw.fused_only && !fuse_up) return BSMI_OK;
  const bool wz = pw.wz;
  const int wm = pw.m, nbatch = wino_batches(wm) * (wz ? kWinoZ : 1);
  if (wz && (wm != 4 || wants_fused)) BSMI_FAIL(BSMI_ERR_STATE, "%s conv %d: packed for the z transform, but planned behind a fused upsampling", p.prefix.c_str(), ci);
  if (prec != BSMI_PREC_BF16X3 || !pw.ready || (wm == 2 && ((o.H & 1) || (o.W & 1))) || st.use_box || st.use_rh) {
    if (wants_fused) BSMI_FAIL(BSMI_ERR_STATE, "%s conv %d: the upsampling was fused into this stage, which cannot take the Winograd form", p.prefix.c_str(), ci);
    return BSMI_OK;
  }
  const bool below = fuse_up && ci == 0 && pw.below_ready && wm == 4 && nsl == 2;
  const int Dv = wz ? (o.D + 1) / 2 : o.D + 2, Ty = (o.H + wm - 1) / wm, Tx = (o.W + wm - 1) / wm, Cv = below ? pw.skip_Cv : pw.Cv;
  const size_t vbatch = (size_t)Dv * Ty * Tx * Cv * 4;
  if (vbatch >= ((size_t)1 << 31)) {
    if (wants_fused) BSMI_FAIL(BSMI_ERR_STATE, "%s conv %d: fused upsampling, but the transformed input is too large", p.prefix.c_str(), ci);
    return BSMI_OK;
  }
  const size_t Mrows = (size_t)(wz ? Dv : o.D) * Ty * Tx;
  if (Mrows >= ((size_t)1 << 31)) BSMI_FAIL(BSMI_ERR_STATE, "%s conv %d: too many rows in a batch of the transform-domain GEMM", p.prefix.c_str(), ci);
  const bool cut = fuse_up && ci == p.nconv - 1;
  WinoStage w{plan, fuse_up, p, ci, pc, pw, slots, so, o, st, below, cut, wz, wm, nbatch, Dv, Ty, Tx, Cv, vbatch, Mrows};
  BSMI_HIP(hipMalloc(&w.V, (size_t)nbatch * vbatch + 4096));
  plan->allocs.push_back(w.V);
  BSMI_HIP(hipMalloc(&w.Mbuf, (size_t)nbatch * Mrows * o.Cpad * sizeof(float)));
  plan->allocs.push_back(w.Mbuf);
  plan->bytes += nbatch * (vbatch + Mrows * o.Cpad * sizeof(float));
  int rc = w.input_transform();
  if (rc || (rc = w.batched_gemm())) return rc;
  st.wino_has_below = false;
  if (below && (rc = w.below_up())) return rc;
  if (cut && (pw.res_part[0].empty() || pw.res_part[1].empty())) BSMI_FAIL(BSMI_ERR_STATE, "%s: fused upsampling without a cut residual branch", p.prefix.c_str());
  st.wino_has_res = !(cut ? pw.res_part[0] : pw.res_entries).empty();
  st.wino_has_res_low = false;
  if (cut && (rc = w.residual_low())) return rc;
  if (st.wino_has_res && (rc = w.residual())) return rc;
  w.output_transform(prec);
  st.tile = pw.tile;
  st.use_wino = true;
  return BSMI_OK;
}

}
```

bootstrapper_amd/csrc/unet_rules.hip:

```cpp
#include <cstdlib>

#include "unet_internal.h"

namespace bsmi {

static int x3_fused_mode() {
  static const int m = [] { const char* e = getenv("BSMI_X3_FUSED"); return e ? atoi(e) : 1; }();
  return m;
}
bool x3_fused_for(TileCfg tile) {
  if (!two_waves_per_simd()) return false;
  return x3_fused_mode() == 1 || x3_fused_mode() == 2 || (x3_fused_mode() == 3 && tile != TILE_256x320);
}

static int wino_mode() {
  static const int m = [] { const char* e = getenv("BSMI_WINO"); return e ? atoi(e) : 1; }();
  return m;
}

static int wino4_mode() {
  static const int m = [] { const char* e = getenv("BSMI_WINO4"); return e ? atoi(e) : 1; }();
  return m;
}
int wino_tile_edge() { return wino4_mode() == 0 ? 2 : 4; }
// ... 33 lines not shown
  if (conv_below_up_mode() == 0 || ci != 0 || p.nslots != 2 || p.nconv < 2 || !wino_eligible(p, 0)) return false;
  if (&p < h->r_conv.data() || &p >= h->r_conv.data() + h->r_conv.size()) return false;
  const int* f = h->cfg.downsample_factors[&p - h->r_conv.data()];
  if (f[0] != 1 || f[1] != 2 || f[2] != 2) return false;
  if (p.cout <= 64 && !x3_fused_for(TILE_256x320)) return false;
  return true;
}

bool fuse_up_enabled() {
  static const bool on = [] { const char* e = getenv("BSMI_FUSE_UP"); return !(e && e[0] == '0'); }();
  return on;
}
bool pool_fuse_enabled() {
  static const bool pool_fuse = [] { const char* e = getenv("BSMI_POOL_FUSE"); return !(e && e[0] == '0'); }();
  return pool_fuse;
}

static int wino_z_mode() {
  static const int m = [] { const char* e = getenv("BSMI_WINO_Z"); return e ? atoi(e) : -1; }();
  return m;
}
bool wino_z_site(const bsmi_unet* h, const PassSite& p, int ci) {
  if (wino_z_mode() == 0 || wino_tile_edge() != 4 || !wino_eligible(p, ci)) return false;
  int cin = p.cout;
  if (ci == 0) {
    cin = 0;
    for (int s = 0; s < p.nslots; ++s) cin += p.cin[s];
  }
  if (&p >= h->r_conv.data() && &p < h->r_conv.data() + h->r_conv.size()) {
    const int* f = h->cfg.downsample_factors[&p - h->r_conv.data()];
    const bool fusable = fuse_up_enabled() && p.nslots == 2 && f[0] == 1 && f[1] == 2 && f[2] == 2;
    if (fusable && (ci == 0 || ci == p.nconv - 1)) return false;
  } else if (&p >= h->l_conv.data() && &p < h->l_conv.data() + h->l_conv.size()) {
    const size_t i = &p - h->l_conv.data();
    if (i + 1 < h->l_conv.size() && ci == p.nconv - 1) {
      const int* f = h->cfg.downsample_factors[i];
      if (pool_fuse_enabled() && f[0] == 1 && f[1] == 2 && f[2] == 2) return false;
    }
  } else {
    return false;
  }
  if (wino_z_mode() >= 1) return true;
  return cin >= 1024 && p.cout >= 1024;
}

int h16_mode() {
  static const int m = [] { const char* e = getenv("BSMI_H16"); return e ? atoi(e) : 1; }();
  return m;
}
int h16_only_npad() {
  static const int only_npad = [] { const char* e = getenv("BSMI_H16_NPAD"); return e ? atoi(e) : 0; }();
  return only_npad;
}
bool h16_balanced() {
  static const bool balanced = [] { const char* e = getenv("BSMI_H16_BALANCE"); return !(e && e[0] == '0'); }();
  return balanced;
}

bool rh_enabled(int prec, TileCfg tile, size_t nsteps) {
  static const int mode = [] { const char* e = getenv("BSMI_USE_RH"); return !e ? 2 : (e[0] == '1' ? 1 : 0); }();
  return prec != BSMI_PREC_BF16X3 && (mode == 1 || (mode == 2 && tile_bn(tile) <= 64 && nsteps >= 200));
}

bool box_enabled() {
  static const bool enabled = [] { const char* e = getenv("BSMI_USE_BOX"); return !(e && e[0] == '0'); }();
  return enabled;
}

bool first_pass_eligible(const bsmi_unet* h) {
  if (h->cfg.in_channels != 1 || h->l_conv.empty()) return false;
  const PassSite& p = h->l_conv[0];
  if (p.nconv != 2 || p.cout > 16) return false;
  for (int c = 0; c < 2; ++c)
    for (int d = 0; d < 3; ++d)
      if (p.k[c][d] != 3) return false;
  const char* e = getenv("BSMI_FUSED_FIRST");
  return !(e && e[0] == '0');
}

}
```

bootstrapper_amd/csrc/wino.hip:

```cpp
#include "wino.h"

#include <cstdlib>
#include <cstring>

#include "dev_guard.h"

namespace bsmi {

typedef uint32_t u32x4_t __attribute__((ext_vector_type(4)));
typedef float f32x4_t __attribute__((ext_vector_type(4)));

namespace {

__device__ __forceinline__ uint16_t to_bf16(float f) {
  __bf16 h = (__bf16)f;
  return __builtin_bit_cast(uint16_t, h);
}
__device__ __forceinline__ void unpack8(u32x4_t v, float* f) {
  const uint32_t w[4] = {v.x, v.y, v.z, v.w};
#pragma unroll
  for (int i = 0; i < 4; ++i) {
    f[2 * i] = __uint_as_float(w[i] << 16);
    f[2 * i + 1] = __uint_as_float(w[i] & 0xffff0000u);
  }
}
__device__ __forceinline__ u32x4_t pack8(const float* f) {
  uint32_t w[4];
#pragma unroll
  for (int i = 0; i < 4; ++i) w[i] = (uint32_t)to_bf16(f[2 * i]) | ((uint32_t)to_bf16(f[2 * i + 1]) << 16);
  u32x4_t v = {w[0], w[1], w[2], w[3]};
  return v;
}
__device__ __forceinline__ void load_split8(const uint16_t* base, size_t e, float* f) {
  const uint16_t* p = base + 2 * e;
  float g[8];
  unpack8(*(const u32x4_t*)p, f);
  unpack8(*(const u32x4_t*)(p + 8), g);
#pragma unroll
  for (int k = 0; k < 8; ++k) f[k] += g[k];
}
template <bool NT>
__device__ __forceinline__ void store_split8(uint16_t* base, size_t e, const float* f) {
  uint16_t* p = base + 2 * e;
  const u32x4_t hv = pack8(f);
  float h[8], r[8];
  unpack8(hv, h);
#pragma unroll
  for (int k = 0; k < 8; ++k) r[k] = f[k] - h[k];
  const u32x4_t lv = pack8(r);
  if constexpr (NT) {
    __builtin_nontemporal_store(hv, (u32x4_t*)p);
    __builtin_nontemporal_store(lv, (u32x4_t*)(p + 8));
  } else {
    *(u32x4_t*)p = hv;
    *(u32x4_t*)(p + 8) = lv;
  }
}

__device__ __forceinline__ void lin_src(int dst, int f, int n, int& i0, int& i1, float& w0, float& w1) {
  float src = ((float)dst + 0.5f) * (1.0f / (float)f) - 0.5f;
  src = src < 0.f ? 0.f : src;
  i0 = (int)src;
  i0 = i0 < n - 1 ? i0 : n - 1;
  i1 = i0 + 1 < n ? i0 + 1 : n - 1;
  w1 = src - (float)i0;
  w1 = w1 < 0.f ? 0.f : (w1 > 1.f ? 1.f : w1);
  w0 = 1.f - w1;
}

__global__ __launch_bounds__(256) void wino_in_kernel(const WinoInArgs a, int src, size_t total) {
  const unsigned nb = gridDim.x, q = nb >> 3, r = nb & 7, xcd = blockIdx.x & 7, j = blockIdx.x >> 3;
  const unsigned blk = (xcd < r ? xcd * (q + 1) : r * (q + 1) + (xcd - r) * q) + j;
  const size_t i = (size_t)blk * blockDim.x + threadIdx.x;
  if (i >= total) return;
  const int ncv = a.Cpad[src] >> 3;
  const int cv = (int)(i % ncv);
  const size_t t = i / ncv;
  const int ty = (int)(t % a.Ty);
  const int z = (int)(t / a.Ty);
  const uint16_t* sp = (const uint16_t*)a.src[src];
  const int H = a.H[src], W = a.W[src], C = a.Cpad[src];
  const size_t e_in = (((size_t)(z + a.oz[src]) * H + (2 * ty + a.oy[src])) * W + a.ox[src]) * C + 8 * cv;
  const size_t rstride = (size_t)W * C;
  uint16_t* V = (uint16_t*)a.V;
  const size_t plane = (size_t)a.Dv * a.Ty * a.Tx * a.Cv;
  const size_t e_out = (((size_t)z * a.Ty + ty) * a.Tx) * a.Cv + a.cv0[src] + 8 * cv;
  float col[4][4][8];
  auto load_col = [&](int c, int x) __attribute__((always_inline)) {
    float d[4][8];
#pragma unroll
    for (int rr = 0; rr < 4; ++rr) load_split8(sp, e_in + rr * rstride + (size_t)x * C, d[rr]);
#pragma unroll
    for (int k = 0; k < 8; ++k) {
      col[c][0][k] = d[0][k] - d[2][k];
      col[c][1][k] = d[1][k] + d[2][k];
      col[c][2][k] = d[2][k] - d[1][k];
      col[c][3][k] = d[1][k] - d[3][k];
    }
  };
  load_col(0, 0);
  load_col(1, 1);
  for (int tx = 0; tx < a.Tx; ++tx) {
    load_col(2, 2 * tx + 2);
    load_col(3, 2 * tx + 3);
    const size_t e0 = e_out + (size_t)tx * a.Cv;
#pragma unroll
    for (int xi = 0; xi < 4; ++xi) {
      float v[4][8];
#pragma unroll
      for (int k = 0; k < 8; ++k) {
        v[0][k] = col[0][xi][k] - col[2][xi][k];
        v[1][k] = col[1][xi][k] + col[2][xi][k];
        v[2][k] = col[2][xi][k] - col[1][xi][k];
        v[3][k] = col[1][xi][k] - col[3][xi][k];
      }
#pragma unroll
      for (int nu = 0; nu < 4; ++nu) store_split8<false>(V, (size_t)(4 * xi + nu) * plane + e0, v[nu]);
    }
#pragma unroll
    for (int xi = 0; xi < 4; ++xi)
#pragma unroll
// ... 381 lines not shown
  const size_t e_out = (((size_t)z * a.Ty + ty) * a.Tx) * a.Cv + a.cv0[src] + 8 * cv;
  float ct[5][6][4];
  auto load_ct = [&](int c, int xlow) __attribute__((always_inline)) {
    const int x = xlow < 0 ? 0 : (xlow > W - 1 ? W - 1 : xlow);
    float L[5][4];
#pragma unroll
    for (int k = 0; k < 5; ++k) load_split4(sp, e_low + ((size_t)wy[k] * W + x) * C, hf, L[k]);
#pragma unroll
    for (int xi = 0; xi < 6; ++xi)
#pragma unroll
      for (int ch = 0; ch < 4; ++ch) {
        float acc = 0.f;
#pragma unroll
        for (int k = 0; k < 5; ++k)
          if (tu4(PY, xi, k) != 0.f) acc += tu4(PY, xi, k) * L[k][ch];
        ct[c][xi][ch] = acc;
      }
  };
  load_ct(0, bx + 2 * tx0);
  load_ct(1, bx + 2 * tx0 + 1);
  load_ct(2, bx + 2 * tx0 + 2);
  uint16_t* vt = (uint16_t*)a.V + 2 * (e_out + (size_t)tx0 * a.Cv) + 8 * hf;
  for (int tx = tx0; tx < tx1; ++tx) {
    load_ct(3, bx + 2 * tx + 3);
    load_ct(4, bx + 2 * tx + 4);
    uint16_t* vp = vt;
#pragma unroll
    for (int xi = 0; xi < 6; ++xi) {
#pragma unroll
      for (int nu = 0; nu < 6; ++nu) {
        float v[4];
#pragma unroll
        for (int ch = 0; ch < 4; ++ch) {
          float acc = 0.f;
#pragma unroll
          for (int c = 0; c < 5; ++c)
            if (tu4(PX, nu, c) != 0.f) acc += tu4(PX, nu, c) * ct[c][xi][ch];
          v[ch] = acc;
        }
        store_split4_pair(vp, hf, v);
        vp += 2 * plane;
      }
    }
    vt += 2 * a.Cv;
#pragma unroll
    for (int c = 0; c < 3; ++c)
#pragma unroll
      for (int xi = 0; xi < 6; ++xi)
#pragma unroll
        for (int ch = 0; ch < 4; ++ch) ct[c][xi][ch] = ct[c + 2][xi][ch];
  }
}

__device__ __forceinline__ constexpr int up2_rel(int e) { return (e >> 1) + (e & 1); }
template <bool LOW, bool POOL = false, int BELOW = -1>
__global__ __launch_bounds__(256) void wino4_out_kernel(const WinoOutArgs a, size_t total) {
  const size_t i = (size_t)blockIdx.x * blockDim.x + threadIdx.x;
  if (i >= total) return;
  const int ncg = a.Co >> 2;
  const int cg = (int)(i % ncg), cv = cg >> 1, hf = cg & 1;
  size_t t = i / ncg;
  const int tx = (int)(t % a.Tx);
  t /= a.Tx;
  const int ty = (int)(t % a.Ty);
  const int z = (int)(t / a.Ty);
  const size_t Mrows = (size_t)a.Do * a.Ty * a.Tx;
  const size_t m = ((size_t)z * a.Ty + ty) * a.Tx + tx;
  [[maybe_unused]] float bacc[4][4][4];
  if constexpr (BELOW >= 0) {
    constexpr int PY = BELOW >> 1, PX = BELOW & 1;
    const int uy = 4 * ty + a.boy, ux = 4 * tx + a.box;
    const int wy_0 = (uy >> 1) - 1, wx_0 = (ux >> 1) - 1;
    float wy0[6], wy1[6], wx0[6], wx1[6];
#pragma unroll
    for (int s = 0; s < 6; ++s) {
      int i0, i1;
      lin_src(uy + s, 2, a.lH, i0, i1, wy0[s], wy1[s]);
      lin_src(ux + s, 2, a.lW, i0, i1, wx0[s], wx1[s]);
    }
    uint32_t roff[5], coff[5];
#pragma unroll
    for (int r = 0; r < 5; ++r) {
      const int y = wy_0 + r, x = wx_0 + r;
      roff[r] = (uint32_t)(y < 0 ? 0 : (y > a.lH - 1 ? a.lH - 1 : y)) * (uint32_t)(a.lW * a.brow);
      coff[r] = (uint32_t)(x < 0 ? 0 : (x > a.lW - 1 ? a.lW - 1 : x)) * (uint32_t)a.brow;
    }
#pragma unroll
    for (int p = 0; p < 4; ++p)
#pragma unroll
      for (int q = 0; q < 4; ++q)
#pragma unroll
        for (int k = 0; k < 4; ++k) bacc[p][q][k] = 0.f;
    const float* yb = a.below + (size_t)z * a.lH * a.lW * a.brow + 4 * cg;
#pragma unroll
    for (int ky = 0; ky < 3; ++ky)
#pragma unroll
      for (int kx = 0; kx < 3; ++kx) {
        const float* yt = yb + (size_t)(3 * ky + kx) * a.btap;
        const int r_lo = up2_rel(PY + ky), nr = up2_rel(PY + ky + 3) + 2 - r_lo;
        const int c_lo = up2_rel(PX + kx), nc = up2_rel(PX + kx + 3) + 2 - c_lo;
        f32x4_t win[4][4];
#pragma unroll
        for (int r = 0; r < 4; ++r)
#pragma unroll
          for (int c = 0; c < 4; ++c)
            if (r < nr && c < nc) win[r][c] = *(const f32x4_t*)(yt + (roff[r_lo + r] + coff[c_lo + c]));
#pragma unroll
        for (int p = 0; p < 4; ++p) {
          const int ra = up2_rel(PY + ky + p) - r_lo;
          float rowb[4][4];
#pragma unroll
          for (int c = 0; c < 4; ++c)
            if (c < nc) {
#pragma unroll
              for (int k = 0; k < 4; ++k) rowb[c][k] = wy0[ky + p] * win[ra][c][k] + wy1[ky + p] * win[ra + 1][c][k];
            }
#pragma unroll
          for (int q = 0; q < 4; ++q) {
            const int ca = up2_rel(PX + kx + q) - c_lo;
#pragma unroll
            for (int k = 0; k < 4; ++k) bacc[p][q][k] += wx0[kx + q] * rowb[ca][k] + wx1[kx + q] * rowb[ca + 1][k];
          }
        }
#pragma unroll
        for (int p = 0; p < 4; ++p)
#pragma unroll
          for (int q = 0; q < 4; ++q)
#pragma unroll
            for (int k = 0; k < 4; ++k) asm volatile("" : "+v"(bacc[p][q][k]) : : "memory");
      }
  }
  float tp[6][4][4];
#pragma unroll
  for (int nu = 0; nu < 6; ++nu) {
    float mm[6][4];
#pragma unroll
    for (int xi = 0; xi < 6; ++xi) {
      const f32x4_t v = __builtin_nontemporal_load((const f32x4_t*)(a.M + ((size_t)(6 * xi + nu) * Mrows + m) * a.Co + 4 * cg));
#pragma unroll
      for (int k = 0; k < 4; ++k) mm[xi][k] = v[k];
    }
    at4_apply(mm, tp[nu]);
  }
  float bv[4];
#pragma unroll
  for (int k = 0; k < 4; ++k) bv[k] = a.bias[4 * cg + k];
  uint16_t* out = (uint16_t*)a.out;
  [[maybe_unused]] float even[4][4];
#pragma unroll
  for (int p = 0; p < 4; ++p) {
    float in[6][4], y[4][4];
#pragma unroll
    for (int nu = 0; nu < 6; ++nu)
#pragma unroll
      for (int k = 0; k < 4; ++k) in[nu][k] = tp[nu][p][k];
    at4_apply(in, y);
    const int oy = 4 * ty + p;
    if (oy >= a.Ho) continue;
    [[maybe_unused]] float left[4];
#pragma unroll
    for (int q = 0; q < 4; ++q) {
      const int ox = 4 * tx + q;
      if (ox >= a.Wo) continue;
      const size_t e8 = (((size_t)z * a.Ho + oy) * a.Wo + ox) * a.Co + 8 * cv;
      const size_t e = e8 + 4 * hf;
      float v[4];
#pragma unroll
      for (int k = 0; k < 4; ++k) v[k] = y[q][k] + bv[k];
      if constexpr (BELOW >= 0) {
#pragma unroll
        for (int k = 0; k < 4; ++k) v[k] += bacc[p][q][k];
      }
      if (a.addend) {
        const f32x4_t r0 = __builtin_nontemporal_load((const f32x4_t*)(a.addend + e));
#pragma unroll
        for (int k = 0; k < 4; ++k) v[k] += r0[k];
      }
      if constexpr (LOW) {
        int y0, y1, x0, x1;
        float wy0, wy1, wx0, wx1;
        lin_src(oy + a.loy, a.lf, a.lH, y0, y1, wy0, wy1);
        lin_src(ox + a.lox, a.lf, a.lW, x0, x1, wx0, wx1);
        const float* base = a.low + ((size_t)(z + a.loz) * a.lH * a.lW) * a.Co + 4 * cg;
        const f32x4_t r00 = *(const f32x4_t*)(base + ((size_t)y0 * a.lW + x0) * a.Co), r01 = *(const f32x4_t*)(base + ((size_t)y0 * a.lW + x1) * a.Co);
        const f32x4_t r10 = *(const f32x4_t*)(base + ((size_t)y1 * a.lW + x0) * a.Co), r11 = *(const f32x4_t*)(base + ((size_t)y1 * a.lW + x1) * a.Co);
#pragma unroll
        for (int k = 0; k < 4; ++k) {
          const float pa = wx0 * r00[k] + wx1 * r01[k];
          const float pb = wx0 * r10[k] + wx1 * r11[k];
          v[k] += wy0 * pa + wy1 * pb;
        }
      }
      if (a.relu) {
#pragma unroll
        for (int k = 0; k < 4; ++k) v[k] = v[k] > 0.f ? v[k] : 0.f;
      }
      store_split4(out, e8, hf, v);
      if constexpr (POOL) {
        float sv[4];
#pragma unroll
        for (int k = 0; k < 4; ++k) {
          const float h = __uint_as_float((uint32_t)to_bf16(v[k]) << 16);
          sv[k] = h + __uint_as_float((uint32_t)to_bf16(v[k] - h) << 16);
        }
        if ((p & 1) == 0) {
#pragma unroll
          for (int k = 0; k < 4; ++k) even[q][k] = sv[k];
        } else if ((q & 1) == 0) {
#pragma unroll
          for (int k = 0; k < 4; ++k) left[k] = sv[k];
        } else {
          float mx[4];
#pragma unroll
          for (int k = 0; k < 4; ++k) mx[k] = fmaxf(fmaxf(fmaxf(fmaxf(-INFINITY, even[q > 0 ? q - 1 : 0][k]), even[q][k]), left[k]), sv[k]);
          const size_t pe = (((size_t)z * (a.Ho >> 1) + (oy >> 1)) * (a.Wo >> 1) + (ox >> 1)) * a.Co + 8 * cv;
          store_split4((uint16_t*)a.pool, pe, hf, mx);
        }
      }
    }
  }
}

__global__ __launch_bounds__(256) void wino4z_out_kernel(const WinoOutArgs a, size_t total) {
  const size_t i = (size_t)blockIdx.x * blockDim.x + threadIdx.x;
  if (i >= total) return;
  const int ncg = a.Co >> 2;
  const int cg = (int)(i % ncg), cv = cg >> 1, hf = cg & 1;
  size_t t = i / ncg;
  const int tx = (int)(t % a.Tx);
  t /= a.Tx;
  const int ty = (int)(t % a.Ty);
  const int r = (int)(t / a.Ty);
  const size_t Mrows = (size_t)((a.Do + 1) >> 1) * a.Ty * a.Tx;
  const size_t m = ((size_t)r * a.Ty + ty) * a.Tx + tx;
  const float* mp = a.M + m * a.Co + 4 * cg;
  const size_t bstride = Mrows * a.Co;
  float o0[4][4][4], o1[4][4][4];
#pragma unroll
  for (int e = 0; e < kWinoZ; ++e) {
    float tp[6][4][4];
#pragma unroll
    for (int nu = 0; nu < 6; ++nu) {
      float mm[6][4];
#pragma unroll
// ... 338 lines not shown
```

bootstrapper_amd/unet.py:

```python
import ctypes as C
import json
import os

import numpy as np
import torch

from . import _lib
from ._lib import lib, check

HEAD_OF_OUTPUT = {"3d_affs": "affs_head", "3d_lsds": "lsds_head", "2d_affs": "aff_head", "2d_lsds": "lsd_head"}

PRECISIONS = {"f32": _lib.PREC_F32, "fp32": _lib.PREC_F32, "float32": _lib.PREC_F32,
              "bf16": _lib.PREC_BF16, "bfloat16": _lib.PREC_BF16,
              "bf16x3": _lib.PREC_BF16X3}


def _tuplify(x):
    return [[int(v) for v in ks] for ks in x]


def _lift(k):
    k = [int(v) for v in k]
    if len(k) == 2:
        return [1] + k
# ... 132 lines not shown
        out = (C.c_int64 * 3)()
        check(lib.bsmi_unet_output_shape(self._h, _lib.i64x3(in_shape), out))
        return tuple(out)

    def flops(self, in_shape):
        f = C.c_double()
        check(lib.bsmi_unet_flops(self._h, _lib.i64x3(in_shape), C.byref(f)))
        return f.value

    def profile(self, on=True):
        check(lib.bsmi_unet_profile_enable(self._h, int(on)))
        return self

    def read_profile(self):
        n = C.c_int()
        cap = 256
        types = (C.c_int32 * cap)()
        ms = (C.c_double * cap)()
        fl = (C.c_double * cap)()
        check(lib.bsmi_unet_profile_read(self._h, cap, C.byref(n), types, ms, fl))
        return [(types[i], ms[i], fl[i]) for i in range(min(n.value, cap))]

    def profile_totals(self, reset=False):
        ms = (C.c_double * 5)()
        fl = (C.c_double * 5)()
        cnt = (C.c_int64 * 5)()
        check(lib.bsmi_unet_profile_totals(self._h, ms, fl, cnt, 1 if reset else 0))
        names = ["input", "conv", "pool", "upsample", "head"]
        return {names[i]: (ms[i], fl[i], cnt[i]) for i in range(5)}

    def profile_executed(self, reset=False):
        v = C.c_double()
        check(lib.bsmi_unet_profile_executed(self._h, C.byref(v), 1 if reset else 0))
        return v.value

    def debug_activation(self, step, what=0):
        shape = (C.c_int64 * 4)()
        check(lib.bsmi_unet_debug_activation(self._h, int(step), int(what), shape, None, 0))
        out = np.empty(tuple(shape), dtype=np.float32)
        check(lib.bsmi_unet_debug_activation(self._h, int(step), int(what), shape, out.ctypes.data_as(C.c_void_p), out.size))
        return out

    def plan_steps(self):
        n = C.c_int()
        check(lib.bsmi_unet_debug_step_info(self._h, 0, None, C.byref(n)))
        out = []
        for i in range(n.value):
            si = _lib.StepInfo()
            check(lib.bsmi_unet_debug_step_info(self._h, i, C.byref(si), None))
            d = {"step": i, "type": _lib.STEP_TYPES[si.type], "materialised": bool(si.materialised), "shape": tuple(si.shape)}
            if d["type"] == "conv":
                d.update(prefix=si.prefix.decode(), conv=si.conv_index, form=_lib.CONV_FORMS[si.form],
                         flags=tuple(name for bit, name in _lib.STEP_FLAGS.items() if si.flags & bit), bn=si.bn, ksteps=si.ksteps,
                         below_up=bool(si.flags & _lib.STEP_BELOW_UP), wino_z=bool(si.flags & _lib.STEP_WINO_Z))
            elif d["type"] == "head":
                d.update(prefix=si.prefix.decode(), head=si.head)
            elif d["type"] in ("pool", "up"):
                d.update(factor=tuple(si.factor))
                if d["type"] == "up":
                    d.update(offset=tuple(si.offset))
            out.append(d)
        return out

    def _run(self, raw, raw_dtype, in_shape, want_f32, want_u8):
        dev = torch.device("cuda", self.device)
        osz = self.output_shape(in_shape)
        nh = len(self.heads)
        f32 = [torch.empty((d,) + osz, dtype=torch.float32, device=dev) if want_f32 else None
               for _, d in self.heads]
        u8 = [torch.empty((d,) + osz, dtype=torch.uint8, device=dev) if want_u8 else None
              for _, d in self.heads]
        pf = (C.c_void_p * nh)(*[t.data_ptr() if t is not None else None for t in f32])
        pu = (C.c_void_p * nh)(*[t.data_ptr() if t is not None else None for t in u8])
        stream = torch.cuda.current_stream(dev).cuda_stream
        check(lib.bsmi_unet_forward(self._h, self.precision, C.c_void_p(raw.data_ptr()), raw_dtype,
                                    _lib.i64x3(in_shape), pf, pu, C.c_void_p(stream)))
        return f32, u8

    def forward(self, *inputs):
        if not all(t.is_cuda for t in inputs):
            raise RuntimeError("bootstrapper_amd.Model runs on the GPU only; move the input to cuda")
        input = inputs[0] if len(inputs) == 1 else torch.cat(inputs, dim=1)
        if self.two_d:
            if input.dim() == 5:
                n, c, d, hh, ww = input.shape
                input = input.reshape(n, c * d, hh, ww)
            if input.dim() != 4 or input.shape[0] != 1:
                raise ValueError("expected input of shape (1, C, H, W)")
            input = input[:, :, None]
        if input.dim() != 5 or input.shape[0] != 1:
            raise ValueError("expected input of shape (1, C, D, H, W)")
        if input.shape[1] != self._cfg.in_channels:
            raise ValueError(f"expected {self._cfg.in_channels} input channels, got {input.shape[1]}")
        x = input.to(torch.float32).contiguous()
        f32, _ = self._run(x, _lib.RAW_F32, x.shape[2:], True, False)
        outs = [t[None] for t in f32]
        if self.two_d and not self.stack_infer:
            outs = [t[:, :, 0] for t in outs]
        return outs[0] if len(outs) == 1 else tuple(outs)

    __call__ = forward

    def predict_u8(self, raw_u8, want_f32=False):
        if raw_u8.dtype != torch.uint8 or not raw_u8.is_cuda:
            raise ValueError("raw_u8 must be a uint8 CUDA tensor")
        x = raw_u8.contiguous()
        shape = x.shape[-3:]
# ... 15 lines not shown
```

include/bsmi.h:

```cpp
#ifndef BSMI_H
#define BSMI_H

#include <stddef.h>
#include <stdint.h>
#include <sys/types.h>

#ifdef __cplusplus
extern "C" {
#endif

#define BSMI_MAX_LEVELS 8
#define BSMI_MAX_CONVS 4
#define BSMI_MAX_HEADS 4
#define BSMI_NAME_LEN 32

#define BSMI_OK 0
#define BSMI_ERR_INVALID (-1)
#define BSMI_ERR_HIP (-2)
#define BSMI_ERR_STATE (-3)
#define BSMI_ERR_MISSING (-4)
#define BSMI_ERR_OVERFLOW (-5)

#define BSMI_PREC_F32 0
#define BSMI_PREC_BF16 1
// ... 106 lines not shown

int bsmi_train_lsd_targets(int device, const int64_t *labels_dev, const uint8_t *unlabelled_dev, const int64_t shape[3],
                           const int64_t roi_offset[3], const int64_t roi_shape[3], const float sigma[3],
                           const float voxel_size[3], int downsample, float *lsds_dev, float *weights_dev, void *stream);

int bsmi_train_lsd2d_targets(int device, const int64_t *labels_dev, const uint8_t *unlabelled_dev, int n_sections,
                             const int64_t shape[2], const int64_t roi_offset[2], const int64_t roi_shape[2], const float sigma[2],
                             const float voxel_size[2], int downsample, float *lsds_dev, float *weights_dev, void *stream);

int bsmi_train_affinity_targets_roi(int device, int64_t *labels_dev, const uint8_t *unlabelled_dev, int n_samples,
                                    const int64_t shape[3], const int64_t roi_offset[3], const int64_t roi_shape[3],
                                    const int32_t *neighborhood, int n, int grow_steps, int only_xy, float clip_min,
                                    float clip_max, float *affs_dev, float *weights_dev, void *stream);

int bsmi_train_mask_sat(int device, const uint8_t *mask_dev, int n_sections, int height, int width, uint32_t *sat_dev,
                        void *stream);

int bsmi_unet_set_persistent_grid(bsmi_unet *h, int n_cus);

int bsmi_stream_create_cu_mask(int device, const uint32_t *cu_mask, int n_words, void **stream_out);
int bsmi_stream_destroy(int device, void *stream);

int bsmi_unet_profile_enable(bsmi_unet *h, int on);
int bsmi_unet_profile_read(bsmi_unet *h, int max_n, int *n, int32_t *types, double *ms,
                           double *flops);
int bsmi_unet_profile_totals(bsmi_unet *h, double ms_by_type[5], double flops_by_type[5],
                             int64_t launches_by_type[5], int reset);
int bsmi_unet_profile_executed(bsmi_unet *h, double *executed_flops, int reset);
int bsmi_debug_lds_canary(int lds_bytes, int blocks, int spins, unsigned long long *mismatches_dev, void *stream);
int bsmi_debug_check_guards(void);
void *bsmi_debug_torch_malloc(ssize_t size, int device, void *stream);
void bsmi_debug_torch_free(void *ptr, ssize_t size, void *stream);
int bsmi_debug_guard_selftest(void);

int bsmi_unet_debug_activation(bsmi_unet *h, int step, int what, int64_t shape_out[4], float *host_out,
                               uint64_t capacity);

enum { BSMI_STEP_INPUT = 0, BSMI_STEP_CONV = 1, BSMI_STEP_POOL = 2, BSMI_STEP_UP = 3, BSMI_STEP_HEAD = 4 };
enum {
  BSMI_FORM_GATHER = 0,
  BSMI_FORM_RASTER_HALO = 1,
  BSMI_FORM_BOX_HALO = 2,
  BSMI_FORM_HALO_RESIDENT = 3,
  BSMI_FORM_FIRST_PASS = 4,
  BSMI_FORM_WINO2 = 5,
  BSMI_FORM_WINO4 = 6,
  BSMI_FORM_COUNT = 7
};
enum {
  BSMI_STEP_FUSED_UP = 1,
  BSMI_STEP_RES_LOW = 2,
  BSMI_STEP_SPLIT_K = 4,
  BSMI_STEP_BELOW_UP = 8,
  BSMI_STEP_WINO_Z = 16
};
typedef struct {
  int32_t type;
  int32_t materialised;
  int32_t shape[4];
  int32_t conv_index;
  int32_t form;
  int32_t flags;
  int32_t bn;
  int32_t ksteps;
  int32_t head;
  int32_t factor[3];
  int32_t offset[3];
  char prefix[64];
} bsmi_unet_step_info;
int bsmi_unet_debug_step_info(bsmi_unet *h, int step, bsmi_unet_step_info *info, int *n_steps);

int bsmi_debug_wino_pack_host(const float *w, int cout, int cin, int wz, uint16_t *out, uint64_t capacity,
                              uint64_t *image_elems, uint64_t *batch_elems, int *npad, int *ksteps);

int bsmi_extract_block_reflect_u8(const uint8_t *vol_dev, const int64_t vol_shape[3],
                                  const int64_t offset[3], const int64_t block_shape[3],
                                  uint8_t *block_dev, void *stream);

typedef struct bsmi_seg bsmi_seg;
int bsmi_seg_create(int device, const int64_t max_shape[3], bsmi_seg **out);
int bsmi_seg_destroy(bsmi_seg *h);

int bsmi_ws_fragments_u8(bsmi_seg *h, const uint8_t *affs_dev, const int64_t shape[3],
                         int fragments_in_xy, int min_seed_distance, uint64_t *frags_dev,
                         uint64_t *max_id_dev, void *stream);

int bsmi_ws_fragments_seeds_u8(bsmi_seg *h, const uint8_t *affs_dev, const int64_t shape[3],
                               int fragments_in_xy, int min_seed_distance, uint64_t *frags_dev,
                               uint64_t *max_id_dev, uint64_t *seeds_dev, void *stream);

int bsmi_agglomerate_mean_u8(bsmi_seg *h, const uint8_t *affs_dev, const uint64_t *frags_dev,
                             const int64_t shape[3], const float *thresholds_host,
                             int n_thresholds, uint64_t *segs_dev, void *stream);

int bsmi_agglomerate_hist_u8(bsmi_seg *h, const uint8_t *affs_dev, const uint64_t *frags_dev,
                             const int64_t shape[3], const float *thresholds_host, int n_thresholds,
                             int quantile, int init_with_max, uint64_t *segs_dev, void *stream);

int bsmi_agglomerate_hist_graph(uint32_t n_nodes, uint32_t n_edges, const uint32_t *edge_u, const uint32_t *edge_v,
                                uint32_t *hist, int quantile, int init_with_max, const float *thresholds,
                                int n_thresholds, uint32_t *roots_out);

int bsmi_frag_postprocess_u8(bsmi_seg *h, const uint8_t *affs_dev, uint64_t *frags_dev,
                             const int64_t shape[3], double filter_value, int64_t min_size,
                             const int64_t crop_offset[3], const int64_t crop_shape[3],
                             uint64_t id_offset, uint64_t *out_dev, uint64_t *num_labels_dev,
                             void *stream);
// ... 269 lines not shown
```

Baseline: 116.2.

## Fuse upsampling into halo-resident conv stages via below-upsample sums and blend addend

Extends the below-upsample trick, previously limited to Winograd stages, to the halo-resident (h16) convolution. The conv over the upsampled input is computed at low resolution as per-tap sums through an implicit GEMM, then blended up by a new kernel into an addend buffer. The h16 epilogue adds that buffer, so the upsampled tensor is never materialised. The cost is extra launches, an fp32 addend round trip and more packing state. The shared blend helpers move into a common header.

```diff
diff --git a/bootstrapper_amd/_lib.py b/bootstrapper_amd/_lib.py
--- a/bootstrapper_amd/_lib.py
+++ b/bootstrapper_amd/_lib.py
@@ -55,6 +55,7 @@
 STEP_FLAGS = {1: "fused-up", 2: "res-low", 4: "split-k"}
 STEP_BELOW_UP = 8
 STEP_WINO_Z = 16
+STEP_BELOW_UP_H16 = 32
 
 
 class Codec(C.Structure):
diff --git a/bootstrapper_amd/csrc/below_blend.h b/bootstrapper_amd/csrc/below_blend.h
--- /dev/null
+++ b/bootstrapper_amd/csrc/below_blend.h
@@ -0,0 +1,103 @@
+#pragma once
+#include <cstdint>
+
+#include <hip/hip_runtime.h>
+
+namespace bsmi {
+
+typedef float f32x4_t __attribute__((ext_vector_type(4)));
+
+__device__ __forceinline__ void lin_src(int dst, int f, int n, int& i0, int& i1, float& w0, float& w1) {
+  float src = ((float)dst + 0.5f) * (1.0f / (float)f) - 0.5f;
+  src = src < 0.f ? 0.f : src;
+  i0 = (int)src;
+  i0 = i0 < n - 1 ? i0 : n - 1;
+  i1 = i0 + 1 < n ? i0 + 1 : n - 1;
+  w1 = src - (float)i0;
+  w1 = w1 < 0.f ? 0.f : (w1 > 1.f ? 1.f : w1);
+  w0 = 1.f - w1;
+}
+
+__device__ __forceinline__ constexpr int up2_rel(int e) { return (e >> 1) + (e & 1); }
+
+template <int PY, int PX>
+__device__ __forceinline__ void below_blend_tile(const float* below, int64_t btap, int brow, int lH, int lW, int boy, int box, int z, int ty, int tx,
+                                                 int cg, float (&bacc)[4][4][4]) {
+  const int uy = 4 * ty + boy, ux = 4 * tx + box;
+  const int wy_0 = (uy >> 1) - 1, wx_0 = (ux >> 1) - 1;
+  float wy0[6], wy1[6], wx0[6], wx1[6];
+#pragma unroll
+  for (int s = 0; s < 6; ++s) {
+    int i0, i1;
+    lin_src(uy + s, 2, lH, i0, i1, wy0[s], wy1[s]);
+    lin_src(ux + s, 2, lW, i0, i1, wx0[s], wx1[s]);
+  }
+  uint32_t roff[5], coff[5];
+#pragma unroll
+  for (int r = 0; r < 5; ++r) {
+    const int y = wy_0 + r, x = wx_0 + r;
+    roff[r] = (uint32_t)(y < 0 ? 0 : (y > lH - 1 ? lH - 1 : y)) * (uint32_t)(lW * brow);
+    coff[r] = (uint32_t)(x < 0 ? 0 : (x > lW - 1 ? lW - 1 : x)) * (uint32_t)brow;
+  }
+#pragma unroll
+  for (int p = 0; p < 4; ++p)
+#pragma unroll
+    for (int q = 0; q < 4; ++q)
+#pragma unroll
+      for (int k = 0; k < 4; ++k) bacc[p][q][k] = 0.f;
+  const float* yb = below + (size_t)z * lH * lW * brow + 4 * cg;
+#pragma unroll
+  for (int ky = 0; ky < 3; ++ky)
+#pragma unroll
+    for (int kx = 0; kx < 3; ++kx) {
+      const float* yt = yb + (size_t)(3 * ky + kx) * btap;
+      const int r_lo = up2_rel(PY + ky), nr = up2_rel(PY + ky + 3) + 2 - r_lo;
+      const int c_lo = up2_rel(PX + kx), nc = up2_rel(PX + kx + 3) + 2 - c_lo;
+      f32x4_t win[4][4];
+#pragma unroll
+      for (int r = 0; r < 4; ++r)
+#pragma unroll
+        for (int c = 0; c < 4; ++c)
+          if (r < nr && c < nc) win[r][c] = *(const f32x4_t*)(yt + (roff[r_lo + r] + coff[c_lo + c]));
+#pragma unroll
+      for (int p = 0; p < 4; ++p) {
+        const int ra = up2_rel(PY + ky + p) - r_lo;
+        float rowb[4][4];
+#pragma unroll
+        for (int c = 0; c < 4; ++c)
+          if (c < nc) {
+#pragma unroll
+            for (int k = 0; k < 4; ++k) rowb[c][k] = wy0[ky + p] * win[ra][c][k] + wy1[ky + p] * win[ra + 1][c][k];
+          }
+#pragma unroll
+        for (int q = 0; q < 4; ++q) {
+          const int ca = up2_rel(PX + kx + q) - c_lo;
+#pragma unroll
+          for (int k = 0; k < 4; ++k) bacc[p][q][k] += wx0[kx + q] * rowb[ca][k] + wx1[kx + q] * rowb[ca + 1][k];
+        }
+      }
+#pragma unroll
+      for (int p = 0; p < 4; ++p)
+#pragma unroll
+        for (int q = 0; q < 4; ++q)
+#pragma unroll
+          for (int k = 0; k < 4; ++k) asm volatile("" : "+v"(bacc[p][q][k]) : : "memory");
+    }
+}
+
+__device__ __forceinline__ void low_blend4(const float* plane, int stride, int lH, int lW, int f, int y, int x, float (&v)[4]) {
+  int y0, y1, x0, x1;
+  float wy0, wy1, wx0, wx1;
+  lin_src(y, f, lH, y0, y1, wy0, wy1);
+  lin_src(x, f, lW, x0, x1, wx0, wx1);
+  const f32x4_t r00 = *(const f32x4_t*)(plane + ((size_t)y0 * lW + x0) * stride), r01 = *(const f32x4_t*)(plane + ((size_t)y0 * lW + x1) * stride);
+  const f32x4_t r10 = *(const f32x4_t*)(plane + ((size_t)y1 * lW + x0) * stride), r11 = *(const f32x4_t*)(plane + ((size_t)y1 * lW + x1) * stride);
+#pragma unroll
+  for (int k = 0; k < 4; ++k) {
+    const float pa = wx0 * r00[k] + wx1 * r01[k];
+    const float pb = wx0 * r10[k] + wx1 * r11[k];
+    v[k] += wy0 * pa + wy1 * pb;
+  }
+}
+
+}
diff --git a/bootstrapper_amd/csrc/conv_h16.h b/bootstrapper_amd/csrc/conv_h16.h
--- a/bootstrapper_amd/csrc/conv_h16.h
+++ b/bootstrapper_amd/csrc/conv_h16.h
@@ -31,7 +31,21 @@
   int Npad;
   int relu;
   int ntiles, n_big, r_small;
+  const float* addend;
 };
+
+struct H16BlendArgs {
+  const float* y;
+  float* addend;
+  int astride;
+  int ntaps;
+  int64_t btap;
+  int brow;
+  int lD, lH, lW;
+  int oz, oy, ox;
+  int Do, Ho, Wo, Co;
+};
+int launch_h16_blend(const H16BlendArgs& a, hipStream_t stream);
 
 constexpr int kH16TileRows = 512;
 int h16_halo_rows(int Win, int ky, int kx, int npad, int* max_r);
diff --git a/bootstrapper_amd/csrc/conv_h16.hip b/bootstrapper_amd/csrc/conv_h16.hip
--- a/bootstrapper_amd/csrc/conv_h16.hip
+++ b/bootstrapper_amd/csrc/conv_h16.hip
@@ -2,6 +2,7 @@
 
 #include <algorithm>
 
+#include "below_blend.h"
 #include "conv_dev.h"
 
 namespace bsmi {
@@ -192,9 +193,31 @@
   float bv[FNB];
 #pragma unroll
   for (int j = 0; j < FNB; ++j) bv[j] = a.bias[j * 16 + lr];
+  const float* const addend = a.addend;
 #pragma unroll
   for (int i = 0; i < kR; ++i) {
     if (i >= R) break;
+    if (addend) {
+      const int qb = q0 + wave * (R * 16) + i * 16 + 4 * lq;
+      int xx = qb % a.Win;
+      const int zy = qb / a.Win;
+      int yy = zy % a.Hin, z = zy / a.Hin;
+#pragma unroll
+      for (int r = 0; r < 4; ++r) {
+        if (qb + r < a.Q && xx < a.Wo && yy < a.Ho) {
+          const float* ar = addend + ((size_t)(z * a.Ho + yy) * a.Wo + xx) * BN + lr;
+#pragma unroll
+          for (int j = 0; j < FNB; ++j) acc[i][j][r] += ar[j * 16];
+        }
+        if (++xx == a.Win) {
+          xx = 0;
+          if (++yy == a.Hin) {
+            yy = 0;
+            ++z;
+          }
+        }
+      }
+    }
 #pragma unroll
     for (int j = 0; j < FNB; ++j)
 #pragma unroll
@@ -259,6 +282,76 @@
   return BSMI_OK;
 }
 
+template <int PAR>
+__global__ __launch_bounds__(256) void h16_blend9_kernel(const H16BlendArgs a, int Ty, int Tx, size_t total) {
+  const size_t i = (size_t)blockIdx.x * blockDim.x + threadIdx.x;
+  if (i >= total) return;
+  const int ncg = a.Co >> 2;
+  const int cg = (int)(i % ncg);
+  size_t t = i / ncg;
+  const int tx = (int)(t % Tx);
+  t /= Tx;
+  const int ty = (int)(t % Ty);
+  const int z = (int)(t / Ty);
+  float bacc[4][4][4];
+  below_blend_tile<(PAR >> 1), (PAR & 1)>(a.y, a.btap, a.brow, a.lH, a.lW, a.oy, a.ox, z, ty, tx, cg, bacc);
+#pragma unroll
+  for (int p = 0; p < 4; ++p) {
+    const int oy = 4 * ty + p;
+    if (oy >= a.Ho) continue;
+#pragma unroll
+    for (int q = 0; q < 4; ++q) {
+      const int ox = 4 * tx + q;
+      if (ox >= a.Wo) continue;
+      const f32x4_t v = {bacc[p][q][0], bacc[p][q][1], bacc[p][q][2], bacc[p][q][3]};
+      *(f32x4_t*)(a.addend + (((size_t)z * a.Ho + oy) * a.Wo + ox) * a.astride + 4 * cg) = v;
+    }
+  }
+}
+
+__global__ __launch_bounds__(256) void h16_blend1_kernel(const H16BlendArgs a, size_t total) {
+  const size_t i = (size_t)blockIdx.x * blockDim.x + threadIdx.x;
+  if (i >= total) return;
+  const int ncg = a.Co >> 2;
+  const int cg = (int)(i % ncg);
+  size_t t = i / ncg;
+  const int x = (int)(t % a.Wo);
+  t /= a.Wo;
+  const int y = (int)(t % a.Ho);
+  const int z = (int)(t / a.Ho);
+  float v[4] = {0.f, 0.f, 0.f, 0.f};
+  low_blend4(a.y + ((size_t)(z + a.oz) * a.lH * a.lW) * a.brow + 4 * cg, a.brow, a.lH, a.lW, 2, y + a.oy, x + a.ox, v);
+  const f32x4_t o = {v[0], v[1], v[2], v[3]};
+  *(f32x4_t*)(a.addend + (((size_t)z * a.Ho + y) * a.Wo + x) * a.astride + 4 * cg) = o;
+}
+
+}
+
+int launch_h16_blend(const H16BlendArgs& a, hipStream_t stream) {
+  if (!a.y || !a.addend || a.Do < 1 || a.Ho < 1 || a.Wo < 1 || a.Co < 4 || a.Co % 4 || a.astride < a.Co || a.astride % 4 || a.brow < a.Co || a.lH < 1 || a.lW < 1 || a.oy < 0 || a.ox < 0 ||
+      (int64_t)a.lH * a.lW * a.brow >= ((int64_t)1 << 31))
+    BSMI_FAIL(BSMI_ERR_INVALID, "halo conv blend: bad geometry");
+  if (a.ntaps == 9) {
+    if (a.btap < a.Co || a.oy + a.Ho + 2 > 2 * a.lH || a.ox + a.Wo + 2 > 2 * a.lW)
+      BSMI_FAIL(BSMI_ERR_INVALID, "halo conv blend: the sums below the upsampling do not cover the stage's input");
+    const int Ty = (a.Ho + 3) / 4, Tx = (a.Wo + 3) / 4;
+    const size_t total = (size_t)a.Do * Ty * Tx * (a.Co / 4);
+    const dim3 grid((unsigned)((total + 255) / 256));
+    const int par = 2 * (a.oy & 1) + (a.ox & 1);
+    if (par == 0) hipLaunchKernelGGL(h16_blend9_kernel<0>, grid, dim3(256), 0, stream, a, Ty, Tx, total);
+    else if (par == 1) hipLaunchKernelGGL(h16_blend9_kernel<1>, grid, dim3(256), 0, stream, a, Ty, Tx, total);
+    else if (par == 2) hipLaunchKernelGGL(h16_blend9_kernel<2>, grid, dim3(256), 0, stream, a, Ty, Tx, total);
+    else hipLaunchKernelGGL(h16_blend9_kernel<3>, grid, dim3(256), 0, stream, a, Ty, Tx, total);
+  } else if (a.ntaps == 1) {
+    if (a.oz < 0 || a.oz + a.Do > a.lD || a.oy + a.Ho > 2 * a.lH || a.ox + a.Wo > 2 * a.lW)
+      BSMI_FAIL(BSMI_ERR_INVALID, "halo conv blend: the low-resolution residual does not cover the output");
+    const size_t total = (size_t)a.Do * a.Ho * a.Wo * (a.Co / 4);
+    hipLaunchKernelGGL(h16_blend1_kernel, dim3((unsigned)((total + 255) / 256)), dim3(256), 0, stream, a, total);
+  } else {
+    BSMI_FAIL(BSMI_ERR_INVALID, "halo conv blend: %d taps (1 or 9)", a.ntaps);
+  }
+  BSMI_HIP(hipGetLastError());
+  return BSMI_OK;
 }
 
 int h16_halo_rows(int Win, int ky, int kx, int npad, int* max_r) {
diff --git a/bootstrapper_amd/csrc/unet_debug.hip b/bootstrapper_amd/csrc/unet_debug.hip
--- a/bootstrapper_amd/csrc/unet_debug.hip
+++ b/bootstrapper_amd/csrc/unet_debug.hip
@@ -38,7 +38,7 @@
   if (plan->fused_first && step < 2)
     BSMI_FAIL(BSMI_ERR_STATE, "step %d is not materialised: the first ConvPass ran as one launch (first_pass), which writes step 2 only", step);
   if (st.type == PlanStep::UP && st.skip)
-    BSMI_FAIL(BSMI_ERR_STATE, "step %d is not materialised: the upsampling is fused into the Winograd stages that read it", step);
+    BSMI_FAIL(BSMI_ERR_STATE, "step %d is not materialised: the upsampling is fused into the stages that read it", step);
   const TDesc& t = st.out;
   shape_out[0] = t.D; shape_out[1] = t.H; shape_out[2] = t.W; shape_out[3] = t.C;
   if (!host_out) return BSMI_OK;
@@ -115,6 +115,14 @@
       info->form = BSMI_FORM_HALO_RESIDENT;
       info->bn = st.h16.Npad;
       info->ksteps = st.h16.nsteps;
+      if (st.h16_has_blend) {
+        info->flags |= BSMI_STEP_FUSED_UP;
+        if (st.wino_has_below) info->flags |= BSMI_STEP_BELOW_UP_H16;
+        if (st.wino_has_res_low) info->flags |= BSMI_STEP_RES_LOW;
+        if ((st.wino_has_below && conv_igemm_split_k(st.wino_below, plan->prec, st.below_tile, sk_grid)) ||
+            (st.wino_has_res_low && conv_igemm_split_k(st.wino_res_low, plan->prec, st.tile, sk_grid)))
+          info->flags |= BSMI_STEP_SPLIT_K;
+      }
     } else if (st.use_box) {
       info->form = BSMI_FORM_BOX_HALO;
     } else if (st.use_rh) {
diff --git a/bootstrapper_amd/csrc/unet_forward.hip b/bootstrapper_amd/csrc/unet_forward.hip
--- a/bootstrapper_amd/csrc/unet_forward.hip
+++ b/bootstrapper_amd/csrc/unet_forward.hip
@@ -147,6 +147,11 @@
           rc = launch_wino_out(st.wino_out, s);
           break;
         }
+        if (st.use_h16 && st.h16_has_blend && !(st.tx3 && h->train_forward)) {
+          if (st.wino_has_below && (rc = launch_conv_igemm(st.wino_below, precision, st.below_tile, s, h->sk_ws, h->sk_grid))) break;
+          if (st.wino_has_res_low && (rc = launch_conv_igemm(st.wino_res_low, precision, st.tile, s, h->sk_ws, h->sk_grid))) break;
+          if ((rc = launch_h16_blend(st.h16_blend, s))) break;
+        }
         rc = (st.tx3 && h->train_forward) ? train_forward_conv_x3(h, st, s)
              : st.use_h16 ? launch_conv_h16(st.h16, st.h16_rows, s)
              : st.use_box ? launch_conv_box(st.box, s)
diff --git a/bootstrapper_amd/csrc/unet_internal.h b/bootstrapper_amd/csrc/unet_internal.h
--- a/bootstrapper_amd/csrc/unet_internal.h
+++ b/bootstrapper_amd/csrc/unet_internal.h
@@ -48,6 +48,15 @@
   TileCfg tile = TILE_256x32;
 };
 
+struct BelowImage {
+  std::vector<WinoUnit> units;
+  void* w = nullptr;
+  size_t lo_image_bytes = 0, batch_bytes = 0;
+  int Npad = 0;
+  bool dense = false;
+  TileCfg tile = TILE_256x320;
+};
+
 struct PackedWino {
   bool ready = false;
   int m = 2;
@@ -67,16 +76,12 @@
   void* res_part_w[2] = {nullptr, nullptr};
   size_t res_part_lo[2] = {0, 0};
   bool below_ready = false;
-  std::vector<WinoUnit> skip_units, below_units;
+  std::vector<WinoUnit> skip_units;
   std::vector<int> skip_cin_of_v;
   int skip_Cv = 0;
   void* skip_w = nullptr;
   size_t skip_lo_image_bytes = 0, skip_batch_bytes = 0;
-  void* below_w = nullptr;
-  size_t below_lo_image_bytes = 0, below_batch_bytes = 0;
-  int below_Npad = 0;
-  bool below_dense = false;
-  TileCfg below_tile = TILE_256x320;
+  BelowImage below;
 };
 
 struct H16PhaseHost {
@@ -90,6 +95,17 @@
   void* w = nullptr;
   size_t lo_image_bytes = 0;
   int Npad = 0;
+  bool below_ready = false;
+  std::vector<PackEntry> skip_entries;
+  std::vector<H16PhaseHost> skip_phases;
+  void* skip_w = nullptr;
+  size_t skip_lo_image_bytes = 0;
+  BelowImage below;
+  std::vector<PackEntry> res_low;
+  void* res_low_w = nullptr;
+  size_t res_low_lo = 0;
+  int res_low_Npad = 0;
+  TileCfg res_low_tile = TILE_256x32;
 };
 
 struct PassSite {
@@ -125,6 +141,8 @@
   H16Args h16;
   bool use_h16 = false;
   int h16_rows = 0;
+  H16BlendArgs h16_blend;
+  bool h16_has_blend = false;
   BoxArgs box;
   bool use_box = false;
   bool use_wino = false;
@@ -235,6 +253,8 @@
 bool wino_z_site(const bsmi_unet* h, const PassSite& p, int ci);
 bool fuse_up_enabled();
 bool pool_fuse_enabled();
+bool below_up_h16_site(const bsmi_unet* h, const PassSite& p);
+int below_up_h16_mode();
 int h16_mode();
 int h16_only_npad();
 bool h16_balanced();
diff --git a/bootstrapper_amd/csrc/unet_pack.hip b/bootstrapper_amd/csrc/unet_pack.hip
--- a/bootstrapper_amd/csrc/unet_pack.hip
+++ b/bootstrapper_amd/csrc/unet_pack.hip
@@ -32,12 +32,16 @@
   release_image(pw.res_w);
   for (int part = 0; part < 2; ++part) release_image(pw.res_part_w[part]);
   release_image(pw.skip_w);
-  release_image(pw.below_w);
+  release_image(pw.below.w);
   pw.below_ready = false;
   pw.ready = false;
 }
 void release(PackedH16& ph) {
   release_image(ph.w);
+  release_image(ph.skip_w);
+  release_image(ph.below.w);
+  release_image(ph.res_low_w);
+  ph.below_ready = false;
   ph.ready = false;
 }
 
@@ -181,6 +185,97 @@
   return BSMI_OK;
 }
 
+
+static void residual_entries(const PassSite& p, int ci, std::vector<PackEntry>& res) {
+  res.clear();
+  std::vector<PackEntry> all;
+  build_entries(p, ci, BSMI_PREC_BF16X3, all);
+  for (size_t u = 0; u + 1 < all.size(); u += kUnitsPerStep) {
+    bool is_res = false;
+    for (int j = 0; j < kUnitsPerStep; ++j) is_res |= !all[u + j].dummy && all[u + j].wsrc == 1;
+    if (is_res)
+      for (int j = 0; j < kUnitsPerStep; ++j) res.push_back(all[u + j]);
+  }
+  if ((res.size() / kUnitsPerStep) % 2)
+    for (int j = 0; j < kUnitsPerStep; ++j) res.push_back(PackEntry{0, 0, 0, 0, 0, 0, 0, 0, 0, true, 0});
+}
+
+static void cut_residual(int ci, const std::vector<PackEntry>& res, std::vector<PackEntry> part[2]) {
+  for (int q = 0; q < 2; ++q) part[q].clear();
+  const int up_slot = (ci == 0 ? 0 : 1) + 1;
+  for (size_t u = 0; u + 1 < res.size(); u += kUnitsPerStep) {
+    int slot = -1;
+    for (int j = 0; j < kUnitsPerStep; ++j)
+      if (!res[u + j].dummy) slot = res[u + j].slot;
+    if (slot < 0) continue;
+    for (int j = 0; j < kUnitsPerStep; ++j) part[slot == up_slot ? 1 : 0].push_back(res[u + j]);
+  }
+  for (int q = 0; q < 2; ++q)
+    if ((part[q].size() / kUnitsPerStep) % 2)
+      for (int j = 0; j < kUnitsPerStep; ++j) part[q].push_back(PackEntry{0, 0, 0, 0, 0, 0, 0, 0, 0, true, 0});
+}
+
+static int pack_res_image(const PassSite& p, const HostWeight& wr, const std::vector<PackEntry>& ents, int Npad, void** w_out, size_t* lo_out) {
+  const int64_t cin_r = wr.shape[1];
+  const size_t nsteps = ents.size() / kUnitsPerStep;
+  const size_t nelem = (nsteps * (size_t)Npad + kWeightRowSlack) * 32;
+  std::vector<uint16_t> packed(2 * nelem, 0);
+  for (size_t u = 0; u < ents.size(); ++u) {
+    const PackEntry& e = ents[u];
+    if (e.dummy) continue;
+    const size_t s = u / kUnitsPerStep, j = u % kUnitsPerStep;
+    for (int n = 0; n < p.cout; ++n)
+      for (int kk = 0; kk < 16; ++kk) {
+        const int c = e.c0 + kk;
+        if (c >= e.creal) break;
+        const float v = wr.data[(size_t)n * cin_r + (e.cin_base + c)];
+        const size_t idx = (s * Npad + n) * 32 + j * 16 + kk;
+        split_bf16(v, packed[idx], packed[nelem + idx]);
+      }
+  }
+  *lo_out = nelem * 2;
+  BSMI_HIP(hipMalloc(w_out, packed.size() * 2));
+  BSMI_HIP(hipMemcpy(*w_out, packed.data(), packed.size() * 2, hipMemcpyHostToDevice));
+  return BSMI_OK;
+}
+
+static int pack_below_taps(const PassSite& p, const HostWeight& wm, bool dense, TileCfg tile, int stage_npad, BelowImage& b) {
+  const int cin_m = (int)wm.shape[1];
+  const int cpad_low = round_up(p.cin[1], kChanPad), cpad_out = round_up(p.cout, kChanPad);
+  wino_units(cpad_low, b.units);
+  b.dense = dense;
+  b.tile = tile;
+  b.Npad = dense ? round_up(9 * cpad_out, tile_bn(tile)) : stage_npad;
+  const size_t nsteps = b.units.size() / kUnitsPerStep;
+  const size_t tap_elems = nsteps * (size_t)b.Npad * 32;
+  const size_t nelem = (dense ? 1 : 9) * tap_elems + (size_t)kWeightRowSlack * 32;
+  std::vector<uint16_t> packed(2 * nelem, 0);
+  const int cin1 = p.cin[1], cbase = p.cin[0];
+  host_parallel_for((size_t)p.cout, [&](size_t n_) {
+    const int n = (int)n_;
+    for (size_t u = 0; u < b.units.size(); ++u) {
+      const WinoUnit& un = b.units[u];
+      if (un.dummy) continue;
+      const size_t s = u / kUnitsPerStep, j = u % kUnitsPerStep;
+      for (int kk = 0; kk < 16; ++kk) {
+        const int c = un.vc0 + kk;
+        if (c >= cin1) break;
+        const float* g = wm.data.data() + (((size_t)n * cin_m + (cbase + c)) * 3 + un.kz) * 9;
+        for (int tap = 0; tap < 9; ++tap) {
+          const size_t idx = dense ? (s * b.Npad + (size_t)tap * cpad_out + n) * 32 + j * 16 + kk
+                                   : (size_t)tap * tap_elems + (s * b.Npad + n) * 32 + j * 16 + kk;
+          split_bf16(g[tap], packed[idx], packed[nelem + idx]);
+        }
+      }
+    }
+  });
+  b.lo_image_bytes = nelem * 2;
+  b.batch_bytes = dense ? 0 : tap_elems * 2;
+  BSMI_HIP(hipMalloc(&b.w, packed.size() * 2));
+  BSMI_HIP(hipMemcpy(b.w, packed.data(), packed.size() * 2, hipMemcpyHostToDevice));
+  return BSMI_OK;
+}
+
 int pack_wino(bsmi_unet* h, PassSite& p, int ci) {
   PackedWino& pw = p.wino[ci];
   release(pw);
@@ -222,56 +317,14 @@
   }
   pw.res_entries.clear();
   if (ci == p.nconv - 1) {
-    std::vector<PackEntry> all;
-    build_entries(p, ci, BSMI_PREC_BF16X3, all);
-    for (size_t u = 0; u + 1 < all.size(); u += kUnitsPerStep) {
-      bool res = false;
-      for (int j = 0; j < kUnitsPerStep; ++j) res |= !all[u + j].dummy && all[u + j].wsrc == 1;
-      if (res)
-        for (int j = 0; j < kUnitsPerStep; ++j) pw.res_entries.push_back(all[u + j]);
-    }
-    if ((pw.res_entries.size() / kUnitsPerStep) % 2)
-      for (int j = 0; j < kUnitsPerStep; ++j) pw.res_entries.push_back(PackEntry{0, 0, 0, 0, 0, 0, 0, 0, 0, true, 0});
-    const int64_t cin_r = wr.shape[1];
-    auto pack_res = [&](const std::vector<PackEntry>& ents, void** w_out, size_t* lo_out) -> int {
-      const size_t nsteps = ents.size() / kUnitsPerStep;
-      const size_t nelem = (nsteps * (size_t)pw.Npad + kWeightRowSlack) * 32;
-      std::vector<uint16_t> packed(2 * nelem, 0);
-      for (size_t u = 0; u < ents.size(); ++u) {
-        const PackEntry& e = ents[u];
-        if (e.dummy) continue;
-        const size_t s = u / kUnitsPerStep, j = u % kUnitsPerStep;
-        for (int n = 0; n < p.cout; ++n)
-          for (int kk = 0; kk < 16; ++kk) {
-            const int c = e.c0 + kk;
-            if (c >= e.creal) break;
-            const float v = wr.data[(size_t)n * cin_r + (e.cin_base + c)];
-            const size_t idx = (s * pw.Npad + n) * 32 + j * 16 + kk;
-            split_bf16(v, packed[idx], packed[nelem + idx]);
-          }
-      }
-      *lo_out = nelem * 2;
-      BSMI_HIP(hipMalloc(w_out, packed.size() * 2));
-      BSMI_HIP(hipMemcpy(*w_out, packed.data(), packed.size() * 2, hipMemcpyHostToDevice));
-      return BSMI_OK;
-    };
-    int rc = pack_res(pw.res_entries, &pw.res_w, &pw.res_lo_image_bytes);
+    residual_entries(p, ci, pw.res_entries);
+    int rc = pack_res_image(p, wr, pw.res_entries, pw.Npad, &pw.res_w, &pw.res_lo_image_bytes);
     if (rc) return rc;
     for (int part = 0; part < 2; ++part) pw.res_part[part].clear();
     if (p.nslots == 2) {
-      const int up_slot = (ci == 0 ? 0 : 1) + 1;
-      for (size_t u = 0; u + 1 < pw.res_entries.size(); u += kUnitsPerStep) {
-        int slot = -1;
-        for (int j = 0; j < kUnitsPerStep; ++j)
-          if (!pw.res_entries[u + j].dummy) slot = pw.res_entries[u + j].slot;
-        if (slot < 0) continue;
-        for (int j = 0; j < kUnitsPerStep; ++j) pw.res_part[slot == up_slot ? 1 : 0].push_back(pw.res_entries[u + j]);
-      }
-      for (int part = 0; part < 2; ++part) {
-        if ((pw.res_part[part].size() / kUnitsPerStep) % 2)
-          for (int j = 0; j < kUnitsPerStep; ++j) pw.res_part[part].push_back(PackEntry{0, 0, 0, 0, 0, 0, 0, 0, 0, true, 0});
-        if ((rc = pack_res(pw.res_part[part], &pw.res_part_w[part], &pw.res_part_lo[part]))) return rc;
-      }
+      cut_residual(ci, pw.res_entries, pw.res_part);
+      for (int part = 0; part < 2; ++part)
+        if ((rc = pack_res_image(p, wr, pw.res_part[part], pw.Npad, &pw.res_part_w[part], &pw.res_part_lo[part]))) return rc;
     }
   }
   if (below_up_site(h, p, ci) && pw.m == 4) {
@@ -283,50 +336,20 @@
     if (rc) return rc;
     pw.skip_lo_image_bytes = image_elems * 2;
     pw.skip_batch_bytes = batch_elems * 2;
-    const int cpad_low = round_up(p.cin[1], kChanPad), cpad_out = round_up(p.cout, kChanPad);
-    wino_units(cpad_low, pw.below_units);
-    pw.below_dense = p.cout <= 64;
-    pw.below_tile = pw.below_dense ? TILE_256x320 : pw.tile;
-    pw.below_Npad = pw.below_dense ? round_up(9 * cpad_out, tile_bn(pw.below_tile)) : pw.Npad;
-    const size_t nsteps = pw.below_units.size() / kUnitsPerStep;
-    const size_t tap_elems = nsteps * (size_t)pw.below_Npad * 32;
-    const size_t nelem = (pw.below_dense ? 1 : 9) * tap_elems + (size_t)kWeightRowSlack * 32;
-    std::vector<uint16_t> packed(2 * nelem, 0);
-    const bool dense = pw.below_dense;
-    const int cin1 = p.cin[1], cbase = p.cin[0];
-    host_parallel_for((size_t)p.cout, [&](size_t n_) {
-      const int n = (int)n_;
-      for (size_t u = 0; u < pw.below_units.size(); ++u) {
-        const WinoUnit& un = pw.below_units[u];
-        if (un.dummy) continue;
-        const size_t s = u / kUnitsPerStep, j = u % kUnitsPerStep;
-        for (int kk = 0; kk < 16; ++kk) {
-          const int c = un.vc0 + kk;
-          if (c >= cin1) break;
-          const float* g = wm.data.data() + (((size_t)n * cin_m + (cbase + c)) * 3 + un.kz) * 9;
-          for (int tap = 0; tap < 9; ++tap) {
-            const size_t idx = dense ? (s * pw.below_Npad + (size_t)tap * cpad_out + n) * 32 + j * 16 + kk
-                                     : (size_t)tap * tap_elems + (s * pw.below_Npad + n) * 32 + j * 16 + kk;
-            split_bf16(g[tap], packed[idx], packed[nelem + idx]);
-          }
-        }
-      }
-    });
-    pw.below_lo_image_bytes = nelem * 2;
-    pw.below_batch_bytes = dense ? 0 : tap_elems * 2;
-    BSMI_HIP(hipMalloc(&pw.below_w, packed.size() * 2));
-    BSMI_HIP(hipMemcpy(pw.below_w, packed.data(), packed.size() * 2, hipMemcpyHostToDevice));
+    const bool dense = p.cout <= 64;
+    if ((rc = pack_below_taps(p, wm, dense, dense ? TILE_256x320 : pw.tile, pw.Npad, pw.below))) return rc;
     pw.below_ready = true;
   }
   pw.ready = true;
   return BSMI_OK;
 }
 
-static void build_entries_h16(const PassSite& p, int ci, std::vector<PackEntry>& out, std::vector<H16PhaseHost>& phases) {
+static void build_entries_h16(const PassSite& p, int ci, std::vector<PackEntry>& out, std::vector<H16PhaseHost>& phases, int without_slot = -1) {
   const bool last = ci == p.nconv - 1;
   const int* k = p.k[ci];
   const PackEntry dummy{0, 0, 0, 0, 0, 0, 0, 0, 0, true, 0};
   auto add_taps = [&](int slot, int cin_base, int creal) {
+    if (slot == without_slot) return;
     const int cpad = round_up(creal, kChanPad);
     for (int z = 0; z < k[0]; ++z)
       for (int c0 = 0; c0 < cpad; c0 += 16) {
@@ -362,7 +385,7 @@
     const int first_slot = ci == 0 ? 0 : 1;
     int base = 0;
     for (int s = 0; s < p.nslots; ++s) {
-      const int cpad = round_up(p.cin[s], kChanPad);
+      const int cpad = first_slot + s == without_slot ? 0 : round_up(p.cin[s], kChanPad);
       for (int c0 = 0; c0 < cpad; c0 += 16) {
         phases.push_back(H16PhaseHost{first_slot + s, c0, crop[0] / 2, 1, (int)(out.size() / kUnitsPerStep), 1});
         out.push_back(PackEntry{first_slot + s, crop[0] / 2, crop[1] / 2, crop[2] / 2, c0, 1, 0, base, p.cin[s], false, (int)phases.size() - 1});
@@ -384,27 +407,52 @@
   const HostWeight& wm = h->weights[p.prefix + ".conv_pass." + std::to_string(2 * ci) + ".weight"];
   const HostWeight& wr = h->weights[p.prefix + ".residual.0.weight"];
   const int64_t cin_m = wm.shape[1], ntap_m = wm.shape[2] * wm.shape[3] * wm.shape[4], cin_r = wr.shape[1];
-  const size_t nsteps = ph.entries.size() / kUnitsPerStep;
-  const size_t nelem = (nsteps * (size_t)ph.Npad + kWeightRowSlack) * 32;
-  std::vector<uint16_t> packed(2 * nelem, 0);
-  host_parallel_for((size_t)p.cout, [&](size_t n_) {
-    const int n = (int)n_;
-    for (size_t u = 0; u < ph.entries.size(); ++u) {
-      const PackEntry& e = ph.entries[u];
-      if (e.dummy) continue;
-      const size_t s = u / kUnitsPerStep, j = u % kUnitsPerStep;
-      for (int kk = 0; kk < 16; ++kk) {
-        const int c = e.c0 + kk;
-        if (c >= e.creal) break;
-        const float v = e.wsrc == 0 ? wm.data[((size_t)n * cin_m + (e.cin_base + c)) * ntap_m + e.tap] : wr.data[(size_t)n * cin_r + (e.cin_base + c)];
-        const size_t idx = (s * ph.Npad + n) * 32 + j * 16 + kk;
-        split_bf16(v, packed[idx], packed[nelem + idx]);
-      }
-    }
-  });
-  ph.lo_image_bytes = nelem * 2;
-  BSMI_HIP(hipMalloc(&ph.w, packed.size() * 2));
-  BSMI_HIP(hipMemcpy(ph.w, packed.data(), packed.size() * 2, hipMemcpyHostToDevice));
+  auto pack_image = [&](const std::vector<PackEntry>& ents, void** w_out, size_t* lo_out) -> int {
+    const size_t nsteps = ents.size() / kUnitsPerStep;
+    const size_t nelem = (nsteps * (size_t)ph.Npad + kWeightRowSlack) * 32;
+    std::vector<uint16_t> packed(2 * nelem, 0);
+    host_parallel_for((size_t)p.cout, [&](size_t n_) {
+      const int n = (int)n_;
+      for (size_t u = 0; u < ents.size(); ++u) {
+        const PackEntry& e = ents[u];
+        if (e.dummy) continue;
+        const size_t s = u / kUnitsPerStep, j = u % kUnitsPerStep;
+        for (int kk = 0; kk < 16; ++kk) {
+          const int c = e.c0 + kk;
+          if (c >= e.creal) break;
+          const float v = e.wsrc == 0 ? wm.data[((size_t)n * cin_m + (e.cin_base + c)) * ntap_m + e.tap] : wr.data[(size_t)n * cin_r + (e.cin_base + c)];
+          const size_t idx = (s * ph.Npad + n) * 32 + j * 16 + kk;
+          split_bf16(v, packed[idx], packed[nelem + idx]);
+        }
+      }
+    });
+    *lo_out = nelem * 2;
+    BSMI_HIP(hipMalloc(w_out, packed.size() * 2));
+    BSMI_HIP(hipMemcpy(*w_out, packed.data(), packed.size() * 2, hipMemcpyHostToDevice));
+    return BSMI_OK;
+  };
+  int rc = pack_image(ph.entries, &ph.w, &ph.lo_image_bytes);
+  if (rc) return rc;
+  const bool last = ci == p.nconv - 1;
+  if (below_up_h16_site(h, p) && (ci == 0 || last)) {
+    ph.skip_entries.clear();
+    ph.skip_phases.clear();
+    build_entries_h16(p, ci, ph.skip_entries, ph.skip_phases, (ci == 0 ? 0 : 1) + 1);
+    if ((rc = pack_image(ph.skip_entries, &ph.skip_w, &ph.skip_lo_image_bytes))) return rc;
+    if (ci == 0) {
+      const int ncol = 9 * round_up(p.cout, kChanPad);
+      if ((rc = pack_below_taps(p, wm, true, ncol <= 160 ? TILE_256x160 : TILE_256x320, 0, ph.below))) return rc;
+    } else {
+      std::vector<PackEntry> res, part[2];
+      residual_entries(p, ci, res);
+      cut_residual(ci, res, part);
+      ph.res_low = part[1];
+      ph.res_low_tile = choose_tile(p.cout);
+      ph.res_low_Npad = round_up(p.cout, tile_bn(ph.res_low_tile));
+      if ((rc = pack_res_image(p, wr, ph.res_low, ph.res_low_Npad, &ph.res_low_w, &ph.res_low_lo))) return rc;
+    }
+    ph.below_ready = true;
+  }
   ph.ready = true;
   return BSMI_OK;
 }
diff --git a/bootstrapper_amd/csrc/unet_plan.h b/bootstrapper_amd/csrc/unet_plan.h
--- a/bootstrapper_amd/csrc/unet_plan.h
+++ b/bootstrapper_amd/csrc/unet_plan.h
@@ -7,6 +7,7 @@
   TDesc low;
   int f[3];
   int o[3];
+  bool h16 = false;
 };
 
 struct Planner {
@@ -29,4 +30,9 @@
 int upload_ksteps(Plan* plan, const std::vector<KStep>& ks, ConvArgs& a);
 void set_strides(ConvArgs& a, const void* base, int H, int W, int C, int bytes_per_channel);
 
+int plan_below_gemm(Plan* plan, const std::string& who, const BelowImage& b, const UpFuse& fu, const int so_up[3], int up_cpad, const TDesc& o,
+                    const float* bias, ConvArgs& r, void** Ybuf, size_t* Mbelow, int below_off[3]);
+int plan_residual_low_gemm(Plan* plan, const std::string& who, const std::vector<PackEntry>& ents, const void* w, size_t lo_image_bytes, int Npad,
+                           const UpFuse& fu, const int (*so)[3], const TDesc& o, const float* bias, ConvArgs& r, void** low, int low_off[3]);
+
 }
diff --git a/bootstrapper_amd/csrc/unet_plan.hip b/bootstrapper_amd/csrc/unet_plan.hip
--- a/bootstrapper_amd/csrc/unet_plan.hip
+++ b/bootstrapper_amd/csrc/unet_plan.hip
@@ -150,40 +150,81 @@
   return BSMI_OK;
 }
 
+static int h16_geometry(int npad, const int* k, const TDesc& o, int* max_r) {
+  const int Hin = o.H + k[1] - 1, Win = o.W + k[2] - 1;
+  const int rows = h16_halo_rows(Win, k[1], k[2], npad, max_r);
+  if (!rows || Hin > 2047 || Win > 2047 || o.D > 1023) return 0;
+  if ((int64_t)o.D * Hin * Win >= ((int64_t)1 << 31)) return 0;
+  return rows;
+}
+
+static bool h16_rule_selects(const PackedH16& ph, const int* k, const TDesc& o) {
+  const int64_t Q = (int64_t)o.D * (o.H + k[1] - 1) * (o.W + k[2] - 1);
+  if (Q < (int64_t)2 * 256 * kH16TileRows) return false;
+  if (ph.Npad == 64) {
+    int main_steps = 0, res_steps = 0;
+    for (const H16PhaseHost& hp : ph.phases) (hp.kind ? res_steps : main_steps) += hp.nsteps;
+    if (3 * res_steps > main_steps) return false;
+  }
+  return true;
+}
+
+static bool below_up_h16_takes(const bsmi_unet* h, const PassSite& rp, const int target[3]) {
+  const int last = rp.nconv - 1;
+  if (!below_up_h16_site(h, rp) || !rp.h16[0].below_ready || !rp.h16[last].below_ready) return false;
+  if (h16_only_npad() && h16_only_npad() != rp.h16[0].Npad) return false;
+  TDesc o;
+  o.D = target[0]; o.H = target[1]; o.W = target[2];
+  for (int c = 0; c < rp.nconv; ++c) {
+    o.D -= rp.k[c][0] - 1; o.H -= rp.k[c][1] - 1; o.W -= rp.k[c][2] - 1;
+    if (o.D <= 0 || o.H <= 0 || o.W <= 0) return false;
+    if (c != 0 && c != last) continue;
+    int max_r = 0;
+    if (!h16_geometry(rp.h16[c].Npad, rp.k[c], o, &max_r)) return false;
+    if (below_up_h16_mode() != 1 && !h16_rule_selects(rp.h16[c], rp.k[c], o)) return false;
+  }
+  return true;
+}
+
 int Planner::plan_h16(PassSite& p, int ci, const PackedConv& pc, const TDesc* slots, const int (*so)[3], const TDesc& o, PlanStep& st) {
   st.use_h16 = false;
   const PackedH16& ph = p.h16[ci];
   const int* k = p.k[ci];
   const int Hin = o.H + k[1] - 1, Win = o.W + k[2] - 1;
-  if (prec != BSMI_PREC_BF16X3 || !ph.ready || h16_mode() == 0 || pc.bias == nullptr) return BSMI_OK;
-  if (h16_only_npad() && h16_only_npad() != ph.Npad) return BSMI_OK;
+  const bool below = fuse_up && fuse_up->h16 && (ci == 0 || ci == p.nconv - 1);
   int max_r = 0;
-  const int rows = h16_halo_rows(Win, k[1], k[2], ph.Npad, &max_r);
-  if (!rows || Hin > 2047 || Win > 2047 || o.D > 1023) return BSMI_OK;
+  const int rows = h16_geometry(ph.Npad, k, o, &max_r);
+  if (below) {
+    if (prec != BSMI_PREC_BF16X3 || !ph.below_ready || pc.bias == nullptr || !rows)
+      BSMI_FAIL(BSMI_ERR_STATE, "%s conv %d: the upsampling was fused into this stage, which cannot take the halo-resident form", p.prefix.c_str(), ci);
+  } else {
+    if (prec != BSMI_PREC_BF16X3 || !ph.ready || h16_mode() == 0 || pc.bias == nullptr) return BSMI_OK;
+    if (h16_only_npad() && h16_only_npad() != ph.Npad) return BSMI_OK;
+    if (!rows) return BSMI_OK;
+    if (h16_mode() == 1 && !h16_rule_selects(ph, k, o)) return BSMI_OK;
+  }
   const int64_t Q = (int64_t)o.D * Hin * Win;
-  if (Q >= ((int64_t)1 << 31)) return BSMI_OK;
-  if (h16_mode() == 1 && Q < (int64_t)2 * 256 * kH16TileRows) return BSMI_OK;
-  if (h16_mode() == 1 && ph.Npad == 64) {
-    int main_steps = 0, res_steps = 0;
-    for (const H16PhaseHost& hp : ph.phases) (hp.kind ? res_steps : main_steps) += hp.nsteps;
-    if (3 * res_steps > main_steps) return BSMI_OK;
-  }
+  const std::vector<H16PhaseHost>& ph_phases = below ? ph.skip_phases : ph.phases;
+  const std::vector<PackEntry>& ph_entries = below ? ph.skip_entries : ph.entries;
   const int64_t es = 4;
-  std::vector<H16Phase> phases(ph.phases.size());
-  std::vector<H16Step> steps(ph.entries.size() / kUnitsPerStep);
-  for (size_t q = 0; q < ph.phases.size(); ++q) {
-    const H16PhaseHost& hp = ph.phases[q];
+  std::vector<H16Phase> phases(ph_phases.size());
+  std::vector<H16Step> steps(ph_entries.size() / kUnitsPerStep);
+  for (size_t q = 0; q < ph_phases.size(); ++q) {
+    const H16PhaseHost& hp = ph_phases[q];
     const TDesc& t = slots[hp.slot];
-    const PackEntry& e0 = ph.entries[(size_t)kUnitsPerStep * hp.first_step];
+    const PackEntry& e0 = ph_entries[(size_t)kUnitsPerStep * hp.first_step];
     const int oz = so[hp.slot][0] + hp.dz;
     const int oy = so[hp.slot][1] + (hp.kind ? e0.dy : 0);
     const int ox = so[hp.slot][2] + (hp.kind ? e0.dx : 0);
     const int64_t delta = ((((int64_t)oz * t.H + oy) * t.W + ox) * t.Cpad + hp.c0) * es;
-    if (delta >= ((int64_t)1 << 31)) return BSMI_OK;
+    if (delta >= ((int64_t)1 << 31)) {
+      if (below) BSMI_FAIL(BSMI_ERR_STATE, "%s conv %d: fused upsampling, but a source is too large for the halo-resident form", p.prefix.c_str(), ci);
+      return BSMI_OK;
+    }
     phases[q] = H16Phase{hp.slot, (int32_t)delta, hp.kind ? kH16TileRows : kH16TileRows + (k[1] - 1) * Win + (k[2] - 1), hp.nsteps};
     for (int s = hp.first_step; s < hp.first_step + hp.nsteps; ++s) {
-      const PackEntry& ea = ph.entries[(size_t)kUnitsPerStep * s];
-      const PackEntry& eb = ph.entries[(size_t)kUnitsPerStep * s + 1];
+      const PackEntry& ea = ph_entries[(size_t)kUnitsPerStep * s];
+      const PackEntry& eb = ph_entries[(size_t)kUnitsPerStep * s + 1];
       const int offa = hp.kind ? 0 : ea.dy * Win + ea.dx;
       const int offb = (hp.kind || eb.dummy) ? offa : eb.dy * Win + eb.dx;
       steps[s] = H16Step{offa, offb, 0, 0};
@@ -204,8 +245,8 @@
   a.steps = dsteps;
   a.nphases = (int)phases.size();
   a.nsteps = (int)steps.size();
-  a.w = ph.w;
-  a.w_lo = (const char*)ph.w + ph.lo_image_bytes;
+  a.w = below ? ph.skip_w : ph.w;
+  a.w_lo = (const char*)a.w + (below ? ph.skip_lo_image_bytes : ph.lo_image_bytes);
   a.bias = pc.bias;
   a.out = o.ptr;
   a.Do = o.D; a.Ho = o.H; a.Wo = o.W; a.Co = o.Cpad;
@@ -218,6 +259,50 @@
     hipDeviceProp_t prop;
     if (hipGetDeviceProperties(&prop, h->device) == hipSuccess && prop.multiProcessorCount > 0) n_cus = prop.multiProcessorCount;
     h16_tiling(Q, ph.Npad, rows, max_r, h16_balanced() ? n_cus : 0, &a.ntiles, &a.n_big, &a.r_small);
+  }
+  st.h16_has_blend = false;
+  if (below) {
+    const TDesc& lt = fuse_up->low;
+    const size_t abytes = (size_t)o.D * o.H * o.W * ph.Npad * sizeof(float);
+    float* addend = nullptr;
+    BSMI_HIP(hipMalloc((void**)&addend, abytes));
+    plan->allocs.push_back(addend);
+    plan->bytes += abytes;
+    BSMI_HIP(hipMemsetAsync(addend, 0, abytes, nullptr));
+    H16BlendArgs& b = st.h16_blend;
+    memset(&b, 0, sizeof b);
+    b.addend = addend;
+    b.astride = ph.Npad;
+    b.lD = lt.D; b.lH = lt.H; b.lW = lt.W;
+    b.Do = o.D; b.Ho = o.H; b.Wo = o.W; b.Co = o.Cpad;
+    const double kstep = (double)kUnitsPerStep * sube(prec);
+    st.exec_flops = 2.0 * (double)round_up((int)Q, kH16TileRows) * ph.Npad * ((double)a.nsteps * kstep) * 3.0;
+    int rc, off[3] = {0, 0, 0};
+    void* sums = nullptr;
+    if (ci == 0) {
+      size_t Mbelow = 0;
+      if ((rc = plan_below_gemm(plan, p.prefix, ph.below, *fuse_up, so[1], slots[1].Cpad, o, pc.bias, st.wino_below, &sums, &Mbelow, off))) return rc;
+      st.below_tile = ph.below.tile;
+      st.wino_has_below = true;
+      b.ntaps = 9;
+      b.btap = o.Cpad;
+      b.brow = 9 * o.Cpad;
+      b.oz = 0;
+      st.exec_flops += 2.0 * (double)round_up(st.wino_below.M, 256) * ph.below.Npad * ((double)st.wino_below.nsteps * kstep) * 3.0;
+    } else {
+      if ((rc = plan_residual_low_gemm(plan, p.prefix, ph.res_low, ph.res_low_w, ph.res_low_lo, ph.res_low_Npad, *fuse_up, so, o, pc.bias, st.wino_res_low,
+                                       &sums, off)))
+        return rc;
+      st.wino_has_res_low = true;
+      b.ntaps = 1;
+      b.brow = o.Cpad;
+      b.oz = off[0];
+      st.exec_flops += 2.0 * (double)round_up(st.wino_res_low.M, 256) * ph.res_low_Npad * ((double)st.wino_res_low.nsteps * kstep) * 3.0;
+    }
+    b.y = (const float*)sums;
+    b.oy = off[1]; b.ox = off[2];
+    a.addend = addend;
+    st.h16_has_blend = true;
   }
   st.h16_rows = rows;
   st.use_h16 = true;
@@ -534,6 +619,10 @@
       if ((c == 0 || c == rp.nconv - 1) && (size_t)(sp[0] + 2) * ((sp[1] + wm - 1) / wm) * ((sp[2] + wm - 1) / wm) * rp.wino[c].Cv * 4 >= ((size_t)1 << 31)) fuse = false;
     }
   }
+  if (!dry && !fuse && prec == BSMI_PREC_BF16X3 && f[0] == 1 && f[1] == 2 && f[2] == 2 && g_out.ptr && below_up_h16_takes(h, rp, target)) {
+    fuse = true;
+    uf.h16 = true;
+  }
   if (!dry) {
     PlanStep st;
     st.type = PlanStep::UP;
@@ -546,7 +635,8 @@
     uf.low = g_out;
     for (int d = 0; d < 3; ++d) { uf.f[d] = f[d]; uf.o[d] = (up[d] - target[d]) / 2; }
     fuse_up = &uf;
-    if (getenv("BSMI_PLAN_DEBUG")) fprintf(stderr, "[bsmi plan] %s: upsampling fused into the Winograd stages\n", rp.prefix.c_str());
+    if (getenv("BSMI_PLAN_DEBUG"))
+      fprintf(stderr, "[bsmi plan] %s: upsampling fused into the %s\n", rp.prefix.c_str(), uf.h16 ? "addends of the pass's ends" : "Winograd stages");
   }
   const TDesc ins[2] = {f_left, g_c};
   rc = pass(rp, ins, so, target, f_out);
diff --git a/bootstrapper_amd/csrc/unet_plan_wino.hip b/bootstrapper_amd/csrc/unet_plan_wino.hip
--- a/bootstrapper_amd/csrc/unet_plan_wino.hip
+++ b/bootstrapper_amd/csrc/unet_plan_wino.hip
@@ -17,6 +17,83 @@
   a.nbatch = 0;
   a.a_batch = a.w_batch = 0;
 }
+
+}
+
+int plan_below_gemm(Plan* plan, const std::string& who, const BelowImage& b, const UpFuse& fu, const int so_up[3], int up_cpad, const TDesc& o,
+                    const float* bias, ConvArgs& r, void** Ybuf, size_t* Mbelow, int below_off[3]) {
+  const TDesc& lt = fu.low;
+  for (int d = 0; d < 3; ++d) below_off[d] = so_up[d] + fu.o[d];
+  if (fu.f[1] != 2 || fu.f[2] != 2 || lt.Cpad != up_cpad || below_off[0] < 0 || below_off[0] + o.D + 2 > lt.D || below_off[1] < 0 ||
+      below_off[2] < 0 || below_off[1] + o.H + 2 > 2 * lt.H || below_off[2] + o.W + 2 > 2 * lt.W)
+    BSMI_FAIL(BSMI_ERR_STATE, "%s: the low-resolution tensor does not cover the stage's input", who.c_str());
+  *Mbelow = (size_t)o.D * lt.H * lt.W;
+  const size_t ybytes = 9 * *Mbelow * o.Cpad * sizeof(float);
+  if (*Mbelow * 9 >= ((size_t)1 << 31)) BSMI_FAIL(BSMI_ERR_STATE, "%s: too many rows of sums below the upsampling", who.c_str());
+  BSMI_HIP(hipMalloc(Ybuf, ybytes));
+  plan->allocs.push_back(*Ybuf);
+  plan->bytes += ybytes;
+  memset(&r, 0, sizeof r);
+  set_strides(r, lt.ptr, lt.H, lt.W, lt.Cpad, 4);
+  std::vector<KStep> ks(b.units.size() / kUnitsPerStep);
+  for (size_t s = 0; s < ks.size(); ++s) {
+    KStep k;
+    memset(&k, 0, sizeof k);
+    for (int j = 0; j < kUnitsPerStep; ++j) {
+      const WinoUnit& u = b.units[kUnitsPerStep * s + j];
+      if (!u.dummy) k.delta[j] = (int32_t)(((int64_t)(u.kz + below_off[0]) * lt.H * lt.W * lt.Cpad + u.vc0) * 4);
+    }
+    ks[s] = k;
+  }
+  const int rc = upload_ksteps(plan, ks, r);
+  if (rc) return rc;
+  raw_gemm(r, b.w, b.lo_image_bytes, b.Npad);
+  r.bias = bias;
+  r.out = *Ybuf;
+  r.Do = o.D; r.Ho = lt.H; r.Wo = lt.W;
+  r.Co = b.dense ? 9 * o.Cpad : o.Cpad;
+  r.M = (int)*Mbelow;
+  r.nbatch = b.dense ? 0 : 9;
+  r.w_batch = (int64_t)b.batch_bytes;
+  return BSMI_OK;
+}
+
+int plan_residual_low_gemm(Plan* plan, const std::string& who, const std::vector<PackEntry>& ents, const void* w, size_t lo_image_bytes, int Npad,
+                           const UpFuse& fu, const int (*so)[3], const TDesc& o, const float* bias, ConvArgs& r, void** low, int low_off[3]) {
+  const TDesc& g = fu.low;
+  const size_t Mlow = (size_t)g.D * g.H * g.W;
+  BSMI_HIP(hipMalloc(low, Mlow * o.Cpad * sizeof(float)));
+  plan->allocs.push_back(*low);
+  plan->bytes += Mlow * o.Cpad * sizeof(float);
+  memset(&r, 0, sizeof r);
+  set_strides(r, g.ptr, g.H, g.W, g.Cpad, 4);
+  std::vector<KStep> ks(ents.size() / kUnitsPerStep);
+  int up_slot = -1;
+  for (size_t s = 0; s < ks.size(); ++s) {
+    KStep k;
+    memset(&k, 0, sizeof k);
+    for (int j = 0; j < kUnitsPerStep; ++j) {
+      const PackEntry& e = ents[kUnitsPerStep * s + j];
+      if (e.dummy) continue;
+      k.delta[j] = (int32_t)((int64_t)e.c0 * 4);
+      up_slot = e.slot;
+      low_off[0] = e.dz; low_off[1] = e.dy; low_off[2] = e.dx;
+    }
+    ks[s] = k;
+  }
+  if (up_slot < 0) BSMI_FAIL(BSMI_ERR_STATE, "%s: empty low-resolution residual", who.c_str());
+  for (int d = 0; d < 3; ++d) low_off[d] += so[up_slot][d] + fu.o[d];
+  const int rc = upload_ksteps(plan, ks, r);
+  if (rc) return rc;
+  raw_gemm(r, w, lo_image_bytes, Npad);
+  r.bias = bias;
+  r.out = *low;
+  r.Do = g.D; r.Ho = g.H; r.Wo = g.W; r.Co = o.Cpad;
+  r.M = (int)Mlow;
+  return BSMI_OK;
+}
+
+namespace {
 
 struct WinoStage {
   Plan* plan;
@@ -97,78 +174,17 @@
   }
 
   int below_up() {
-    const TDesc& lt = fuse_up->low;
-    for (int d = 0; d < 3; ++d) below_off[d] = so[1][d] + fuse_up->o[d];
-    if (fuse_up->f[1] != 2 || fuse_up->f[2] != 2 || lt.Cpad != slots[1].Cpad || below_off[0] < 0 || below_off[0] + o.D + 2 > lt.D || below_off[1] < 0 ||
-        below_off[2] < 0 || below_off[1] + o.H + 2 > 2 * lt.H || below_off[2] + o.W + 2 > 2 * lt.W)
-      BSMI_FAIL(BSMI_ERR_STATE, "%s: the low-resolution tensor does not cover the stage's input", p.prefix.c_str());
-    Mbelow = (size_t)o.D * lt.H * lt.W;
-    const size_t ybytes = 9 * Mbelow * o.Cpad * sizeof(float);
-    if (Mbelow * 9 >= ((size_t)1 << 31)) BSMI_FAIL(BSMI_ERR_STATE, "%s: too many rows of sums below the upsampling", p.prefix.c_str());
-    BSMI_HIP(hipMalloc(&Ybuf, ybytes));
-    plan->allocs.push_back(Ybuf);
-    plan->bytes += ybytes;
-    ConvArgs& r = st.wino_below;
-    memset(&r, 0, sizeof r);
-    set_strides(r, lt.ptr, lt.H, lt.W, lt.Cpad, 4);
-    std::vector<KStep> ks(pw.below_units.size() / kUnitsPerStep);
-    for (size_t s = 0; s < ks.size(); ++s) {
-      KStep k;
-      memset(&k, 0, sizeof k);
-      for (int j = 0; j < kUnitsPerStep; ++j) {
-        const WinoUnit& u = pw.below_units[kUnitsPerStep * s + j];
-        if (!u.dummy) k.delta[j] = (int32_t)(((int64_t)(u.kz + below_off[0]) * lt.H * lt.W * lt.Cpad + u.vc0) * 4);
-      }
-      ks[s] = k;
-    }
-    const int rc = upload_ksteps(plan, ks, r);
+    const int rc = plan_below_gemm(plan, p.prefix, pw.below, *fuse_up, so[1], slots[1].Cpad, o, pc.bias, st.wino_below, &Ybuf, &Mbelow, below_off);
     if (rc) return rc;
-    raw_gemm(r, pw.below_w, pw.below_lo_image_bytes, pw.below_Npad);
-    r.bias = pc.bias;
-    r.out = Ybuf;
-    r.Do = o.D; r.Ho = lt.H; r.Wo = lt.W;
-    r.Co = pw.below_dense ? 9 * o.Cpad : o.Cpad;
-    r.M = (int)Mbelow;
-    r.nbatch = pw.below_dense ? 0 : 9;
-    r.w_batch = (int64_t)pw.below_batch_bytes;
-    st.below_tile = pw.below_tile;
+    st.below_tile = pw.below.tile;
     st.wino_has_below = true;
     return BSMI_OK;
   }
 
   int residual_low() {
-    const TDesc& g = fuse_up->low;
-    const size_t Mlow = (size_t)g.D * g.H * g.W;
-    BSMI_HIP(hipMalloc(&low, Mlow * o.Cpad * sizeof(float)));
-    plan->allocs.push_back(low);
-    plan->bytes += Mlow * o.Cpad * sizeof(float);
-    ConvArgs& r = st.wino_res_low;
-    memset(&r, 0, sizeof r);
-    set_strides(r, g.ptr, g.H, g.W, g.Cpad, 4);
-    const std::vector<PackEntry>& ents = pw.res_part[1];
-    std::vector<KStep> ks(ents.size() / kUnitsPerStep);
-    int up_slot = -1;
-    for (size_t s = 0; s < ks.size(); ++s) {
-      KStep k;
-      memset(&k, 0, sizeof k);
-      for (int j = 0; j < kUnitsPerStep; ++j) {
-        const PackEntry& e = ents[kUnitsPerStep * s + j];
-        if (e.dummy) continue;
-        k.delta[j] = (int32_t)((int64_t)e.c0 * 4);
-        up_slot = e.slot;
-        low_off[0] = e.dz; low_off[1] = e.dy; low_off[2] = e.dx;
-      }
-      ks[s] = k;
-    }
-    if (up_slot < 0) BSMI_FAIL(BSMI_ERR_STATE, "%s: empty low-resolution residual", p.prefix.c_str());
-    for (int d = 0; d < 3; ++d) low_off[d] += so[up_slot][d] + fuse_up->o[d];
-    const int rc = upload_ksteps(plan, ks, r);
+    const int rc = plan_residual_low_gemm(plan, p.prefix, pw.res_part[1], pw.res_part_w[1], pw.res_part_lo[1], pw.Npad, *fuse_up, so, o, pc.bias,
+                                          st.wino_res_low, &low, low_off);
     if (rc) return rc;
-    raw_gemm(r, pw.res_part_w[1], pw.res_part_lo[1], pw.Npad);
-    r.bias = pc.bias;
-    r.out = low;
-    r.Do = g.D; r.Ho = g.H; r.Wo = g.W; r.Co = o.Cpad;
-    r.M = (int)Mlow;
     st.wino_has_res_low = true;
     return BSMI_OK;
   }
@@ -215,8 +231,8 @@
     }
     if (below) {
       wo.below = (const float*)Ybuf;
-      wo.btap = pw.below_dense ? (int64_t)o.Cpad : (int64_t)Mbelow * o.Cpad;
-      wo.brow = pw.below_dense ? 9 * o.Cpad : o.Cpad;
+      wo.btap = pw.below.dense ? (int64_t)o.Cpad : (int64_t)Mbelow * o.Cpad;
+      wo.brow = pw.below.dense ? 9 * o.Cpad : o.Cpad;
       wo.boy = below_off[1]; wo.box = below_off[2];
       wo.lD = fuse_up->low.D; wo.lH = fuse_up->low.H; wo.lW = fuse_up->low.W;
       wo.lf = fuse_up->f[1];
@@ -232,7 +248,7 @@
     if (st.wino_has_res) st.exec_flops += 2.0 * (double)round_up(st.wino_res.M, 256) * pw.Npad * ((double)st.wino_res.nsteps * kstep) * 3.0;
     if (st.wino_has_res_low) st.exec_flops += 2.0 * (double)round_up(st.wino_res_low.M, 256) * pw.Npad * ((double)st.wino_res_low.nsteps * kstep) * 3.0;
     if (st.wino_has_below)
-      st.exec_flops += 2.0 * (double)round_up(st.wino_below.M, 256) * pw.below_Npad * (pw.below_dense ? 1 : 9) * ((double)st.wino_below.nsteps * kstep) * 3.0;
+      st.exec_flops += 2.0 * (double)round_up(st.wino_below.M, 256) * pw.below.Npad * (pw.below.dense ? 1 : 9) * ((double)st.wino_below.nsteps * kstep) * 3.0;
   }
 };
 
@@ -241,6 +257,7 @@
 int Planner::plan_wino(PassSite& p, int ci, const PackedConv& pc, const TDesc* slots, const int (*so)[3], int nsl, const TDesc& o, PlanStep& st) {
   st.use_wino = false;
   const PackedWino& pw = p.wino[ci];
+  const UpFuse* const fuse_up = this->fuse_up && !this->fuse_up->h16 ? this->fuse_up : nullptr;
   const bool wants_fused = fuse_up && (ci == 0 || ci == p.nconv - 1);
   if (pw.fused_only && !fuse_up) return BSMI_OK;
   const bool wz = pw.wz;
diff --git a/bootstrapper_amd/csrc/unet_rules.hip b/bootstrapper_amd/csrc/unet_rules.hip
--- a/bootstrapper_amd/csrc/unet_rules.hip
+++ b/bootstrapper_amd/csrc/unet_rules.hip
@@ -109,6 +109,25 @@
   static const int only_npad = [] { const char* e = getenv("BSMI_H16_NPAD"); return e ? atoi(e) : 0; }();
   return only_npad;
 }
+int below_up_h16_mode() {
+  static const int m = [] { const char* e = getenv("BSMI_BELOW_UP_H16"); return e ? atoi(e) : -1; }();
+  return m;
+}
+bool below_up_h16_site(const bsmi_unet* h, const PassSite& p) {
+  if (below_up_h16_mode() == 0 || conv_below_up_mode() == 0 || !fuse_up_enabled() || h16_mode() == 0) return false;
+  if (p.nslots != 2 || p.nconv < 2 || p.cout > 64) return false;
+  if (&p < h->r_conv.data() || &p >= h->r_conv.data() + h->r_conv.size()) return false;
+  const int* f = h->cfg.downsample_factors[&p - h->r_conv.data()];
+  if (f[0] != 1 || f[1] != 2 || f[2] != 2) return false;
+  const int last = p.nconv - 1;
+  for (int ci : {0, last}) {
+    if (p.k[ci][0] != 3 || p.k[ci][1] != 3 || p.k[ci][2] != 3) return false;
+    if (wino_eligible(p, ci) || wino_narrow_last(h, p, ci)) return false;
+  }
+  const int ncol = 9 * round_up(p.cout, kChanPad);
+  return x3_fused_for(ncol <= 160 ? TILE_256x160 : TILE_256x320) && x3_fused_for(choose_tile(p.cout));
+}
+
 bool h16_balanced() {
   static const bool balanced = [] { const char* e = getenv("BSMI_H16_BALANCE"); return !(e && e[0] == '0'); }();
   return balanced;
diff --git a/bootstrapper_amd/csrc/wino.hip b/bootstrapper_amd/csrc/wino.hip
--- a/bootstrapper_amd/csrc/wino.hip
+++ b/bootstrapper_amd/csrc/wino.hip
@@ -3,12 +3,12 @@
 #include <cstdlib>
 #include <cstring>
 
+#include "below_blend.h"
 #include "dev_guard.h"
 
 namespace bsmi {
 
 typedef uint32_t u32x4_t __attribute__((ext_vector_type(4)));
-typedef float f32x4_t __attribute__((ext_vector_type(4)));
 
 namespace {
 
@@ -57,16 +57,6 @@
   }
 }
 
-__device__ __forceinline__ void lin_src(int dst, int f, int n, int& i0, int& i1, float& w0, float& w1) {
-  float src = ((float)dst + 0.5f) * (1.0f / (float)f) - 0.5f;
-  src = src < 0.f ? 0.f : src;
-  i0 = (int)src;
-  i0 = i0 < n - 1 ? i0 : n - 1;
-  i1 = i0 + 1 < n ? i0 + 1 : n - 1;
-  w1 = src - (float)i0;
-  w1 = w1 < 0.f ? 0.f : (w1 > 1.f ? 1.f : w1);
-  w0 = 1.f - w1;
-}
 
 __global__ __launch_bounds__(256) void wino_in_kernel(const WinoInArgs a, int src, size_t total) {
   const unsigned nb = gridDim.x, q = nb >> 3, r = nb & 7, xcd = blockIdx.x & 7, j = blockIdx.x >> 3;
@@ -554,7 +544,6 @@
   }
 }
 
-__device__ __forceinline__ constexpr int up2_rel(int e) { return (e >> 1) + (e & 1); }
 template <bool LOW, bool POOL = false, int BELOW = -1>
 __global__ __launch_bounds__(256) void wino4_out_kernel(const WinoOutArgs a, size_t total) {
   const size_t i = (size_t)blockIdx.x * blockDim.x + threadIdx.x;
@@ -570,67 +559,7 @@
   const size_t m = ((size_t)z * a.Ty + ty) * a.Tx + tx;
   [[maybe_unused]] float bacc[4][4][4];
   if constexpr (BELOW >= 0) {
-    constexpr int PY = BELOW >> 1, PX = BELOW & 1;
-    const int uy = 4 * ty + a.boy, ux = 4 * tx + a.box;
-    const int wy_0 = (uy >> 1) - 1, wx_0 = (ux >> 1) - 1;
-    float wy0[6], wy1[6], wx0[6], wx1[6];
-#pragma unroll
-    for (int s = 0; s < 6; ++s) {
-      int i0, i1;
-      lin_src(uy + s, 2, a.lH, i0, i1, wy0[s], wy1[s]);
-      lin_src(ux + s, 2, a.lW, i0, i1, wx0[s], wx1[s]);
-    }
-    uint32_t roff[5], coff[5];
-#pragma unroll
-    for (int r = 0; r < 5; ++r) {
-      const int y = wy_0 + r, x = wx_0 + r;
-      roff[r] = (uint32_t)(y < 0 ? 0 : (y > a.lH - 1 ? a.lH - 1 : y)) * (uint32_t)(a.lW * a.brow);
-      coff[r] = (uint32_t)(x < 0 ? 0 : (x > a.lW - 1 ? a.lW - 1 : x)) * (uint32_t)a.brow;
-    }
-#pragma unroll
-    for (int p = 0; p < 4; ++p)
-#pragma unroll
-      for (int q = 0; q < 4; ++q)
-#pragma unroll
-        for (int k = 0; k < 4; ++k) bacc[p][q][k] = 0.f;
-    const float* yb = a.below + (size_t)z * a.lH * a.lW * a.brow + 4 * cg;
-#pragma unroll
-    for (int ky = 0; ky < 3; ++ky)
-#pragma unroll
-      for (int kx = 0; kx < 3; ++kx) {
-        const float* yt = yb + (size_t)(3 * ky + kx) * a.btap;
-        const int r_lo = up2_rel(PY + ky), nr = up2_rel(PY + ky + 3) + 2 - r_lo;
-        const int c_lo = up2_rel(PX + kx), nc = up2_rel(PX + kx + 3) + 2 - c_lo;
-        f32x4_t win[4][4];
-#pragma unroll
-        for (int r = 0; r < 4; ++r)
-#pragma unroll
-          for (int c = 0; c < 4; ++c)
-            if (r < nr && c < nc) win[r][c] = *(const f32x4_t*)(yt + (roff[r_lo + r] + coff[c_lo + c]));
-#pragma unroll
-        for (int p = 0; p < 4; ++p) {
-          const int ra = up2_rel(PY + ky + p) - r_lo;
-          float rowb[4][4];
-#pragma unroll
-          for (int c = 0; c < 4; ++c)
-            if (c < nc) {
-#pragma unroll
-              for (int k = 0; k < 4; ++k) rowb[c][k] = wy0[ky + p] * win[ra][c][k] + wy1[ky + p] * win[ra + 1][c][k];
-            }
-#pragma unroll
-          for (int q = 0; q < 4; ++q) {
-            const int ca = up2_rel(PX + kx + q) - c_lo;
-#pragma unroll
-            for (int k = 0; k < 4; ++k) bacc[p][q][k] += wx0[kx + q] * rowb[ca][k] + wx1[kx + q] * rowb[ca + 1][k];
-          }
-        }
-#pragma unroll
-        for (int p = 0; p < 4; ++p)
-#pragma unroll
-          for (int q = 0; q < 4; ++q)
-#pragma unroll
-            for (int k = 0; k < 4; ++k) asm volatile("" : "+v"(bacc[p][q][k]) : : "memory");
-      }
+    below_blend_tile<(BELOW >> 1), (BELOW & 1)>(a.below, a.btap, a.brow, a.lH, a.lW, a.boy, a.box, z, ty, tx, cg, bacc);
   }
   float tp[6][4][4];
 #pragma unroll
@@ -679,19 +608,7 @@
         for (int k = 0; k < 4; ++k) v[k] += r0[k];
       }
       if constexpr (LOW) {
-        int y0, y1, x0, x1;
-        float wy0, wy1, wx0, wx1;
-        lin_src(oy + a.loy, a.lf, a.lH, y0, y1, wy0, wy1);
-        lin_src(ox + a.lox, a.lf, a.lW, x0, x1, wx0, wx1);
-        const float* base = a.low + ((size_t)(z + a.loz) * a.lH * a.lW) * a.Co + 4 * cg;
-        const f32x4_t r00 = *(const f32x4_t*)(base + ((size_t)y0 * a.lW + x0) * a.Co), r01 = *(const f32x4_t*)(base + ((size_t)y0 * a.lW + x1) * a.Co);
-        const f32x4_t r10 = *(const f32x4_t*)(base + ((size_t)y1 * a.lW + x0) * a.Co), r11 = *(const f32x4_t*)(base + ((size_t)y1 * a.lW + x1) * a.Co);
-#pragma unroll
-        for (int k = 0; k < 4; ++k) {
-          const float pa = wx0 * r00[k] + wx1 * r01[k];
-          const float pb = wx0 * r10[k] + wx1 * r11[k];
-          v[k] += wy0 * pa + wy1 * pb;
-        }
+        low_blend4(a.low + ((size_t)(z + a.loz) * a.lH * a.lW) * a.Co + 4 * cg, a.Co, a.lH, a.lW, a.lf, oy + a.loy, ox + a.lox, v);
       }
       if (a.relu) {
 #pragma unroll
diff --git a/bootstrapper_amd/unet.py b/bootstrapper_amd/unet.py
--- a/bootstrapper_amd/unet.py
+++ b/bootstrapper_amd/unet.py
@@ -208,7 +208,8 @@
             if d["type"] == "conv":
                 d.update(prefix=si.prefix.decode(), conv=si.conv_index, form=_lib.CONV_FORMS[si.form],
                          flags=tuple(name for bit, name in _lib.STEP_FLAGS.items() if si.flags & bit), bn=si.bn, ksteps=si.ksteps,
-                         below_up=bool(si.flags & _lib.STEP_BELOW_UP), wino_z=bool(si.flags & _lib.STEP_WINO_Z))
+                         below_up=bool(si.flags & _lib.STEP_BELOW_UP), wino_z=bool(si.flags & _lib.STEP_WINO_Z),
+                         below_up_h16=bool(si.flags & _lib.STEP_BELOW_UP_H16))
             elif d["type"] == "head":
                 d.update(prefix=si.prefix.decode(), head=si.head)
             elif d["type"] in ("pool", "up"):
diff --git a/include/bsmi.h b/include/bsmi.h
--- a/include/bsmi.h
+++ b/include/bsmi.h
@@ -182,7 +182,8 @@
   BSMI_STEP_RES_LOW = 2,
   BSMI_STEP_SPLIT_K = 4,
   BSMI_STEP_BELOW_UP = 8,
-  BSMI_STEP_WINO_Z = 16
+  BSMI_STEP_WINO_Z = 16,
+  BSMI_STEP_BELOW_UP_H16 = 32
 };
 typedef struct {
   int32_t type;
```

Result: no change. 115.4 (-0.7%).
